# darshangm/dynamics-aware-diffusion

Measured on AMD Instinct MI355X. Metric: trajectory plans/sec (H=32, T=100), higher is better.
Workload: dtype f32; 1 GPU; PointMaze umaze-v2 guided policy, H=32 dim=128 mults(1,2,4) T=100 batch=256/GPU; arch=pointmaze, batch_per_gpu=256, global_batch=256, horizon=32, denoise_steps=100, rng=in-kernel philox, conv_arithmetic=fp32 (exact fp32 MFMA), hipgraph=False, loops_in_flight=1

## Files before the change

dynamics_aware_diffusion_amd/_engine.py:

```python
from __future__ import annotations

import ctypes as C
import math
import os
from typing import Dict, Mapping, Optional, Sequence

import torch

_HERE = os.path.dirname(os.path.abspath(__file__))
LIB_PATH = os.environ.get("DAD_LIB") or os.path.join(_HERE, "libdad_hip.so")

DAD_MAX_LEVELS = 8


class DadCfg(C.Structure):
    _fields_ = [
        ("transition_dim", C.c_int32), ("dim", C.c_int32), ("time_dim", C.c_int32),
        ("n_levels", C.c_int32), ("channels", C.c_int32 * DAD_MAX_LEVELS),
        ("kernel_size", C.c_int32), ("horizon", C.c_int32), ("n_timesteps", C.c_int32),
        ("predict_epsilon", C.c_int32), ("clip_denoised", C.c_int32),
    ]


class DadStepArgs(C.Structure):
    _fields_ = [
        ("noise", C.c_void_p), ("seed", C.c_uint64), ("row_offset", C.c_uint64),
        ("draw", C.c_uint64), ("cond0", C.c_void_p), ("cond_per_row", C.c_int32),
        ("guide_grad", C.c_void_p), ("guide_weight", C.c_float),
        ("mean_out", C.c_void_p), ("eps_out", C.c_void_p),
    ]


class DadProjectArgs(C.Structure):
    _fields_ = [
        ("P", C.c_void_p), ("obs_mean", C.c_void_p), ("obs_std", C.c_void_p),
        ("act_mean", C.c_void_p), ("act_std", C.c_void_p),
        ("state_dim", C.c_int32), ("observation_dim", C.c_int32), ("action_dim", C.c_int32),
        ("scratch", C.c_void_p), ("scratch_bytes", C.c_size_t),
    ]


class DadOptimTensor(C.Structure):
    _fields_ = [
        ("param", C.c_void_p), ("grad", C.c_void_p), ("exp_avg", C.c_void_p), ("exp_avg_sq", C.c_void_p),
        ("ema", C.c_void_p), ("numel", C.c_int64), ("group", C.c_int32),
    ]


class DadOptimGroup(C.Structure):
    _fields_ = [
        ("lr", C.c_float), ("beta1", C.c_float), ("beta2", C.c_float), ("eps", C.c_float),
        ("weight_decay", C.c_float), ("step_size", C.c_float), ("bc2_sqrt", C.c_float),
        ("decoupled", C.c_int32), ("one_minus_beta1", C.c_float), ("one_minus_beta2", C.c_float),
    ]


class DadOptimArgs(C.Structure):
    _fields_ = [
        ("groups", C.POINTER(DadOptimGroup)), ("n_groups", C.c_int32), ("max_grad_norm", C.c_float),
        ("ema_decay", C.c_float), ("grad_norm_out", C.c_void_p),
    ]


OPTIM_MAX_GROUPS = 8
OS_HEADER = ("chunk", "chunks", "grid", "partials", "record_ints")
OS_REC_FIELDS = ("tensor", "first", "first_hi", "count", "block")


ABI = {
    "dad_last_error": (C.c_char_p, []),
    "dad_version": (C.c_char_p, []),
    "dad_model_create": (C.c_int, [C.POINTER(DadCfg), C.POINTER(C.c_void_p)]),
    "dad_model_destroy": (None, [C.c_void_p]),
    "dad_model_load_weight": (C.c_int, [C.c_void_p, C.c_char_p, C.c_void_p,
                                        C.POINTER(C.c_int64), C.c_int32]),
    "dad_model_load_schedule": (C.c_int, [C.c_void_p] + [C.c_void_p] * 5),
    "dad_model_load_time_embedding": (C.c_int, [C.c_void_p, C.c_void_p, C.c_int32, C.c_int32]),
    "dad_model_set_precision": (C.c_int, [C.c_void_p, C.c_int32]),
    "dad_model_set_group_channels": (C.c_int, [C.c_void_p, C.POINTER(C.c_int32), C.c_int32]),
    "dad_model_set_horizon": (C.c_int, [C.c_void_p, C.c_int32]),
    "dad_model_finalize": (C.c_int, [C.c_void_p, C.c_void_p]),
    "dad_workspace_bytes": (C.c_int, [C.c_void_p, C.c_int32, C.POINTER(C.c_size_t)]),
    "dad_unet_forward": (C.c_int, [C.c_void_p, C.c_void_p, C.c_int32, C.c_void_p, C.c_int32,
                                   C.c_void_p, C.c_size_t, C.c_void_p]),
    "dad_unet_forward_rows": (C.c_int, [C.c_void_p, C.c_void_p, C.c_void_p, C.c_void_p, C.c_int32,
                                        C.c_void_p, C.c_size_t, C.c_void_p]),
    "dad_projection_violation": (C.c_int, [C.POINTER(DadProjectArgs), C.c_void_p, C.c_void_p, C.c_int32,
                                           C.c_int32, C.c_void_p]),
    "dad_denoise_step": (C.c_int, [C.c_void_p, C.c_void_p, C.c_int32, C.c_int32,
                                   C.POINTER(DadStepArgs), C.c_int32, C.c_void_p, C.c_size_t,
                                   C.c_void_p]),
    "dad_sample_loop": (C.c_int, [C.c_void_p, C.c_void_p, C.c_int32, C.c_int32, C.c_void_p,
                                  C.c_uint64, C.c_uint64, C.c_void_p, C.c_int32,
                                  C.POINTER(DadProjectArgs), C.c_void_p, C.c_int32, C.c_void_p,
                                  C.c_size_t, C.c_void_p]),
    "dad_project": (C.c_int, [C.POINTER(DadProjectArgs), C.c_float, C.c_void_p, C.c_int32,
                              C.c_int32, C.c_void_p]),
    "dad_fill_normal": (C.c_int, [C.c_void_p, C.c_int32, C.c_int32, C.c_uint64, C.c_uint64,
                                  C.c_uint64, C.c_void_p]),
    "dad_debug_set_tile": (C.c_int, [C.c_void_p, C.c_int32]),
    "dad_debug_set_option": (C.c_int, [C.c_void_p, C.c_char_p, C.c_int32]),
    "dad_debug_read_table": (C.c_int, [C.c_void_p, C.c_int32, C.c_int32, C.c_void_p, C.c_int32,
                                       C.POINTER(C.c_int32)]),
    "dad_debug_mish": (C.c_int, [C.c_void_p, C.c_void_p, C.c_int64, C.c_void_p]),
    "dad_debug_kernel_table_consistent": (C.c_int, []),
    "dad_debug_small_batch_plan": (C.c_int, [C.c_void_p, C.c_int32, C.POINTER(C.c_int32),
                                             C.POINTER(C.c_int32)]),
    "dad_debug_backward_plan": (C.c_int, [C.c_void_p, C.c_int32, C.POINTER(C.c_int32), C.c_int32,
                                          C.POINTER(C.c_int32)]),
    "dad_debug_backward_steps": (C.c_int, [C.c_void_p, C.c_int32, C.POINTER(C.c_int32), C.c_int32,
                                           C.POINTER(C.c_int32)]),
    "dad_debug_wgrad_kernel_exists": (C.c_int, [C.c_int32] * 3),
    "dad_model_set_training": (C.c_int, [C.c_void_p, C.c_int32]),
    "dad_model_refresh_weights": (C.c_int, [C.c_void_p, C.c_int32, C.POINTER(C.c_char_p), C.POINTER(C.c_void_p),
                                            C.c_void_p]),
    "dad_train_grad_count": (C.c_int, [C.c_void_p, C.POINTER(C.c_int32), C.POINTER(C.c_int64)]),
    "dad_train_grad_info": (C.c_int, [C.c_void_p, C.c_int32, C.POINTER(C.c_char_p), C.POINTER(C.c_int64),
                                      C.POINTER(C.c_int64)]),
    "dad_train_workspace_bytes": (C.c_int, [C.c_void_p, C.c_int32, C.POINTER(C.c_size_t),
                                            C.POINTER(C.c_size_t)]),
    "dad_unet_forward_train": (C.c_int, [C.c_void_p, C.c_void_p, C.c_void_p, C.c_void_p, C.c_void_p,
                                         C.c_int32, C.c_void_p, C.c_size_t, C.c_void_p]),
    "dad_unet_backward": (C.c_int, [C.c_void_p, C.c_void_p, C.c_void_p, C.c_void_p, C.c_void_p,
                                    C.POINTER(C.c_void_p), C.c_int32,
                                    C.c_int32, C.c_void_p, C.c_size_t, C.c_void_p, C.c_size_t, C.c_void_p]),
    "dad_model_load_train_schedule": (C.c_int, [C.c_void_p, C.c_void_p, C.c_void_p, C.c_int32]),
    "dad_train_time_grad_count": (C.c_int, [C.c_void_p, C.POINTER(C.c_int32), C.POINTER(C.c_int64)]),
    "dad_train_time_grad_info": (C.c_int, [C.c_void_p, C.c_int32, C.POINTER(C.c_char_p), C.POINTER(C.c_int64),
                                           C.POINTER(C.c_int64)]),
    "dad_train_objective_workspace_bytes": (C.c_int, [C.c_void_p, C.c_int32, C.POINTER(C.c_size_t),
                                                      C.POINTER(C.c_size_t)]),
    "dad_train_objective_forward": (C.c_int, [C.c_void_p, C.c_void_p, C.c_void_p, C.c_void_p, C.c_void_p, C.c_int32,
                                              C.c_void_p, C.c_int32, C.c_void_p, C.c_size_t, C.c_void_p]),
    "dad_train_objective_backward": (C.c_int, [C.c_void_p, C.c_void_p, C.c_void_p, C.c_void_p, C.c_int32, C.c_void_p,
                                               C.POINTER(C.c_void_p), C.c_int32, C.POINTER(C.c_void_p), C.c_int32,
                                               C.c_int32, C.c_void_p, C.c_size_t, C.c_void_p, C.c_size_t, C.c_void_p]),
    "dad_debug_objective_offsets": (C.c_int, [C.c_void_p, C.c_int32, C.POINTER(C.c_size_t), C.POINTER(C.c_size_t)]),
    "dad_debug_objective_plan": (C.c_int, [C.c_void_p, C.c_int32, C.POINTER(C.c_int32), C.c_int32,
                                           C.POINTER(C.c_int32)]),
    "dad_debug_forward_plan": (C.c_int, [C.c_void_p, C.c_int32, C.c_int32, C.POINTER(C.c_int32), C.c_int32,
                                         C.POINTER(C.c_int32)]),
    "dad_debug_project_plan": (C.c_int, [C.c_int32] * 5 + [C.c_size_t, C.c_int32, C.POINTER(C.c_int32)]),
    "dad_debug_kernel_registered": (C.c_int, [C.c_int32] * 4),
    "dad_debug_small_kernel_exists": (C.c_int, [C.c_int32] * 8),
    "dad_optim_create": (C.c_int, [C.POINTER(C.c_void_p)]),
    "dad_optim_destroy": (None, [C.c_void_p]),
    "dad_optim_step": (C.c_int, [C.c_void_p, C.POINTER(DadOptimTensor), C.c_int32, C.POINTER(DadOptimArgs), C.c_void_p]),
    "dad_debug_optim_plan": (C.c_int, [C.POINTER(C.c_int64), C.c_int32, C.POINTER(C.c_int32), C.c_int32,
                                       C.POINTER(C.c_int32)]),
    "dad_profile_enable": (C.c_int, [C.c_void_p, C.c_int32]),
    "dad_profile_read": (C.c_int, [C.c_void_p, C.POINTER(C.c_double), C.POINTER(C.c_int64),
                                   C.POINTER(C.c_double)]),
}

_lib = None


def load_library() -> C.CDLL:
    global _lib
    if _lib is not None:
        return _lib
    if not os.path.exists(LIB_PATH):
        raise RuntimeError(
            f"{LIB_PATH} not found: build it with dynamics_aware_diffusion_amd/csrc/build.sh "
            "(or __graft_entry__.build()).  There is no CPU fallback.")
    lib = C.CDLL(LIB_PATH)
    for name, (restype, argtypes) in ABI.items():
        if os.environ.get("DAD_LIB") and not hasattr(lib, name):
            continue
        fn = getattr(lib, name)
        fn.restype = restype
        fn.argtypes = argtypes
    _lib = lib
    return lib


class DadError(RuntimeError):
    def __init__(self, code: int, message: str):
        super().__init__(f"libdad_hip error {code}: {message}")
        self.code = code


def _check(lib, rc: int) -> None:
    if rc != 0:
        raise DadError(rc, lib.dad_last_error().decode("utf-8", "replace"))


def _ptr(t: Optional[torch.Tensor]) -> Optional[int]:
    return None if t is None else t.data_ptr()


def _require_device(t: torch.Tensor, name: str) -> None:
    if not t.is_cuda:
        raise RuntimeError(f"{name} must live on a ROCm device (got {t.device}); the HIP engine "
                           "has no CPU path")
    if t.dtype != torch.float32 or not t.is_contiguous():
        raise RuntimeError(f"{name} must be contiguous float32 (got {t.dtype}, "
                           f"contiguous={t.is_contiguous()})")


PRECISIONS = {"fp32": 0, "f16x3": 1}
LOSS_TYPES = {"l1": 1, "l2": 2}
TABLES = {"sinusoid": 0, "time_mlp": 1, "blocks": 2}
TIME_GEMM_MODES = ("FWD_H1", "FWD_TEMB", "FWD_ROWS", "BWD_DWK", "BWD_DACT", "BWD_DW3", "BWD_DH1", "BWD_DW1", "DTEMB")


FP_REC_FIELDS = ("conv", "sub", "cfg", "taps", "stride", "flags", "kc", "kslices", "gn_npt", "ntiles_n", "mtiles", "part_tile",
                 "family")
FP_FAMILIES = ("gemm", "halo8")
FP_CC_FIELDS = ("conv", "taps", "stride", "wide", "ride", "big", "ride_in", "tile_rows", "windowed", "slice_ch", "kslices",
                "ntiles", "res_kind")
FP_FINAL_KERNELS = (None, "final_posterior_kernel", "final_cc_kernel")
FP_FLAGS = ("x3", "bdir", "ragged", "res", "padded", "windowed")
PP_FIELDS = ("form", "rows_per_block", "gx", "gy", "lds_bytes", "refused")
PP_FORMS = ("row1", "row4", "gemm")


def registered_kernels():
    lib = load_library()
    gemm = {("gemm", cfg, taps, stride, f) for cfg in range(10) for taps in range(1, 8) for stride in (1, 2) for f in range(64)
            if lib.dad_debug_kernel_registered(cfg, taps, stride, f)}
    cc, ccw = set(), set()
    for taps in range(1, 8):
        for stride in (1, 2):
            for ride in (0, 1):
                for rows in (8, 16, 32, 64):
                    for a in (0, 1):
                        for win in (0, 1):
                            if lib.dad_debug_small_kernel_exists(taps, stride, ride, 0, a, 0, rows, win):
                                cc.add(("cc", taps, stride, ride, a, rows, win))
                        if lib.dad_debug_small_kernel_exists(taps, stride, ride, 1, 0, a, rows, 0):
                            ccw.add(("ccw", taps, stride, ride, a, rows))
    return gemm, cc, ccw


BS_KINDS = ("bias", "wgrad", "dgrad", "gn", "resid", "cols")
BS_FIELDS = {
    "bias": ("rows", "C"),
    "wgrad": ("taps", "tile", "windowed", "M", "C0", "C1", "stride", "pad", "Lg", "Lz", "gx", "gy", "ragged", "concat_inside",
              "edge_m", "edge_c", "swapped", "ksplit", "slab_n4", "samples", "spc", "sps", "chunks", "last_chunks"),
    "dgrad": ("conv", "sub", "write"),
    "gn": ("nv", "cpg", "L", "lreal", "cpg_real", "dtemb", "short_pair", "C"),
    "resid": ("write", "n", "to_x"),
    "cols": ("C", "off", "ld", "rows", "write"),
}
BS_WRITES = ("set", "add", "stage")


def wgrad_kernels():
    lib = load_library()
    return {(taps, tile, win) for taps in range(1, 9) for tile in range(4) for win in (0, 1)
            if lib.dad_debug_wgrad_kernel_exists(taps, tile, win)}


def projection_plan(state_dim: int, observation_dim: int, action_dim: int, batch: int, horizon: int, *,
                    scratch_bytes: int = 0, violation: bool = False) -> dict:
    lib = load_library()
    out = (C.c_int32 * len(PP_FIELDS))()
    _check(lib, lib.dad_debug_project_plan(int(state_dim), int(observation_dim), int(action_dim), int(batch), int(horizon),
                                           int(scratch_bytes), int(bool(violation)), out))
    q = dict(zip(PP_FIELDS, out))
    q["form"], q["refused"] = PP_FORMS[q["form"]], bool(q["refused"])
    q["grid"] = (q.pop("gx"), q.pop("gy"))
    return q


def optim_plan(numel: Sequence[int]) -> dict:
    lib = load_library()
    n = len(numel)
    sizes = (C.c_int64 * max(n, 1))(*[int(v) for v in numel])
    needed = C.c_int32()
    _check(lib, lib.dad_debug_optim_plan(sizes, n, None, 0, C.byref(needed)))
    out = (C.c_int32 * needed.value)()
    _check(lib, lib.dad_debug_optim_plan(sizes, n, out, needed.value, C.byref(needed)))
    head = dict(zip(OS_HEADER, out[:len(OS_HEADER)]))
    k = head.pop("record_ints")
    assert k == len(OS_REC_FIELDS)
    recs = []
    for i in range(head["chunks"]):
        r = dict(zip(OS_REC_FIELDS, out[len(OS_HEADER) + i * k:len(OS_HEADER) + (i + 1) * k]))
        r["first"] += r.pop("first_hi") << 31
        recs.append(r)
    head["records"] = recs
    return head


def sinusoid_table(n_timesteps: int, dim: int) -> torch.Tensor:
    half = dim // 2
    scale = math.log(10000) / (half - 1)
    freqs = torch.exp(torch.arange(half) * -scale)
    arg = torch.arange(n_timesteps)[:, None] * freqs[None, :]
    return torch.cat((arg.sin(), arg.cos()), dim=-1).contiguous()

SCHEDULE_KEYS = ("sqrt_recip_alphas_cumprod", "sqrt_recipm1_alphas_cumprod",
                 "posterior_mean_coef1", "posterior_mean_coef2",
                 "posterior_log_variance_clipped")


class HipEngine:

    def __init__(self, *, transition_dim: int, dim: int, channels: Sequence[int], horizon: int,
                 n_timesteps: int, time_dim: Optional[int] = None, kernel_size: int = 5,
                 predict_epsilon: bool = True, clip_denoised: bool = True,
                 device: torch.device | str = "cuda", precision: str = "fp32", training: bool = False):
        if precision not in PRECISIONS:
            raise ValueError(f"precision must be one of {sorted(PRECISIONS)}, got {precision!r}")
        self.precision = precision
        self.lib = load_library()
        self.device = torch.device(device)
        if self.device.type != "cuda":
            raise RuntimeError("HipEngine needs a ROCm device; there is no CPU path")
        from .utils import padding
        self.real_dim, self.real_channels = int(dim), [int(c) for c in channels]
        padded = [padding.padded_width(c) for c in self.real_channels]
        self.padded = padded != self.real_channels
        if self.padded:
            if self.real_channels[0] != self.real_dim:
                raise NotImplementedError("zero-padded widths need dim_mults[0] == 1")
            if transition_dim == self.real_dim:
                raise NotImplementedError(
                    f"transition_dim == dim == {dim} makes the first block's residual the trajectory itself; "
                    "with zero-padded GroupNorm groups that identity has no kernel")
        horizon = int(horizon)
        levels = len(self.real_channels)
        self.padded_horizon = max(1 << max(horizon - 1, 0).bit_length(), 4 << (levels - 1))
        self.rows_padded = self.padded_horizon != horizon
        if self.rows_padded:
            if horizon % (1 << (levels - 1)) != 0:
                raise ValueError(f"horizon {horizon} cannot be halved {levels - 1} times (the reference's U-Net needs "
                                 f"H % 2^(levels-1) == 0, temporal_unet.py:35-54)")
            if transition_dim == self.real_dim:
                raise NotImplementedError("transition_dim == dim with a zero-padded horizon has no kernel")
        self.padded = self.padded or self.rows_padded
        cfg = DadCfg()
        cfg.transition_dim = transition_dim
        cfg.dim = padded[0] if padded != self.real_channels else dim
        cfg.time_dim = time_dim or dim
        cfg.n_levels = len(channels)
        for i, ch in enumerate(padded):
            cfg.channels[i] = int(ch)
        cfg.kernel_size = kernel_size
        cfg.horizon = self.padded_horizon
        cfg.n_timesteps = n_timesteps
        cfg.predict_epsilon = int(predict_epsilon)
        cfg.clip_denoised = int(clip_denoised)
        self.cfg = cfg
        self.horizon = horizon
        self.transition_dim = transition_dim
        self.n_timesteps = n_timesteps
        handle = C.c_void_p()
        _check(self.lib, self.lib.dad_model_create(C.byref(cfg), C.byref(handle)))
        self._h = handle
        _check(self.lib, self.lib.dad_model_set_precision(self._h, PRECISIONS[precision]))
        self.widths_padded = padded != self.real_channels
        if self.widths_padded:
            real = (C.c_int32 * len(self.real_channels))(*self.real_channels)
            _check(self.lib, self.lib.dad_model_set_group_channels(self._h, real, len(self.real_channels)))
        if self.rows_padded:
            _check(self.lib, self.lib.dad_model_set_horizon(self._h, horizon))
        self.training = bool(training)
        if self.training:
            _check(self.lib, self.lib.dad_model_set_training(self._h, 1))
        self._ws: Dict[int, torch.Tensor] = {}
        self._pinned: Dict[tuple, torch.Tensor] = {}
        self.ready = False

    def __del__(self):
        h = getattr(self, "_h", None)
# ... 229 lines not shown
        rows = torch.arange(B, dtype=torch.int32, device=self.device)
        out = torch.empty_like(x)
        with torch.cuda.device(self.device):
            _check(self.lib, self.lib.dad_unet_forward_train(
                self._h, x.data_ptr(), rows.data_ptr(), temb_rows.data_ptr(), out.data_ptr(), B,
                saved.data_ptr(), saved.numel() * 4, self._stream()))
        return out, saved

    def train_backward(self, x: torch.Tensor, d_out: torch.Tensor, saved: torch.Tensor, temb_width: int, shapes):
        B = self._traj(x)
        if self._traj(d_out, "d_out") != B:
            raise RuntimeError("d_out batch mismatch")
        sv, sc = C.c_size_t(), C.c_size_t()
        _check(self.lib, self.lib.dad_train_workspace_bytes(self._h, B, C.byref(sv), C.byref(sc)))
        scratch = torch.empty(max(sc.value, 4) // 4 + 4, dtype=torch.float32, device=self.device)
        layout, total = self.grad_layout()
        if len(shapes) != len(layout):
            raise RuntimeError(f"{len(shapes)} parameter shapes for {len(layout)} gradient tensors")
        real = None
        if self.widths_padded:
            real = self.flat_padding([k for k, _, _ in layout], shapes, [o for _, o, _ in layout], total)
            shapes = real.padded_shapes
            for (key, _, numel), n in zip(layout, real.sizes):
                if n != numel:
                    raise RuntimeError(f"{key}: {n} padded elements, the library expects {numel}")
        flat = torch.empty(total, dtype=torch.float32, device=self.device)
        base = flat.data_ptr()
        spans = [layout[i + 1][1] - layout[i][1] for i in range(len(layout) - 1)] + [total - layout[-1][1]]
        pieces = flat.split_with_sizes(spans)
        grads = [(pc if pc.numel() == numel else pc[:numel]).view(tuple(shape))
                 for pc, (_, _, numel), shape in zip(pieces, layout, shapes)]
        ptrs = (C.c_void_p * len(grads))(*[base + 4 * offset for _, offset, _ in layout])
        d_x = torch.empty_like(x)
        d_temb = torch.empty(B, temb_width, dtype=torch.float32, device=self.device)
        with torch.cuda.device(self.device):
            _check(self.lib, self.lib.dad_unet_backward(
                self._h, x.data_ptr(), d_out.data_ptr(), d_x.data_ptr(), d_temb.data_ptr(), ptrs, len(grads), B,
                saved.data_ptr(), saved.numel() * 4, scratch.data_ptr(), scratch.numel() * 4, self._stream()))
        if real is not None:
            grads = real.gather(flat)
        return d_x, d_temb, grads

    def bind_train_schedule(self, sqrt_ac: torch.Tensor, sqrt_1m_ac: torch.Tensor) -> None:
        sig = (sqrt_ac.data_ptr(), sqrt_ac._version, sqrt_1m_ac.data_ptr(), sqrt_1m_ac._version)
        if getattr(self, "_train_sched_sig", None) == sig:
            return
        a = sqrt_ac.detach().to("cpu", torch.float32).contiguous()
        b = sqrt_1m_ac.detach().to("cpu", torch.float32).contiguous()
        if a.numel() != self.n_timesteps or b.numel() != self.n_timesteps:
            raise ValueError(f"training schedule has {a.numel()} / {b.numel()} entries, expected {self.n_timesteps}")
        with torch.cuda.device(self.device):
            _check(self.lib, self.lib.dad_model_load_train_schedule(self._h, a.data_ptr(), b.data_ptr(), self.n_timesteps))
        self._train_sched_sig = sig

    def time_grad_layout(self):
        cached = getattr(self, "_time_grad_layout", None)
        if cached is not None:
            return cached
        n, total = C.c_int32(), C.c_int64()
        _check(self.lib, self.lib.dad_train_time_grad_count(self._h, C.byref(n), C.byref(total)))
        out = []
        for i in range(n.value):
            key, off, numel = C.c_char_p(), C.c_int64(), C.c_int64()
            _check(self.lib, self.lib.dad_train_time_grad_info(self._h, i, C.byref(key), C.byref(off), C.byref(numel)))
            out.append((key.value.decode(), off.value, numel.value))
        self._time_grad_layout = (out, total.value)
        return self._time_grad_layout

    def _objective_bytes(self, batch: int):
        cache = self.__dict__.setdefault("_objective_sizes", {})
        if batch not in cache:
            sv, sc = C.c_size_t(), C.c_size_t()
            _check(self.lib, self.lib.dad_train_objective_workspace_bytes(self._h, batch, C.byref(sv), C.byref(sc)))
            cache[batch] = (sv.value, sc.value)
        return cache[batch]

    def objective_forward(self, x0: torch.Tensor, t32: torch.Tensor, noise: torch.Tensor,
                          weights: Optional[torch.Tensor], loss_type: int):
        B = self._traj(x0, "x_start")
        for name, ten in (("noise", noise), ("weights", weights)):
            if ten is not None and self._traj(ten, name) != B:
                raise RuntimeError(f"{name} batch mismatch")
        if t32.dtype != torch.int32 or t32.numel() != B or t32.device != x0.device or not t32.is_contiguous():
            raise RuntimeError("t must be (B) contiguous int32 on the trajectory's device")
        sv, _ = self._objective_bytes(B)
        saved = torch.empty(max(sv, 4) // 4 + 4, dtype=torch.float32, device=self.device)
        loss = torch.empty((), dtype=torch.float32, device=self.device)
        with torch.cuda.device(self.device):
            _check(self.lib, self.lib.dad_train_objective_forward(
                self._h, x0.data_ptr(), t32.data_ptr(), noise.data_ptr(), _ptr(weights), int(loss_type),
                loss.data_ptr(), B, saved.data_ptr(), saved.numel() * 4, self._stream()))
        return loss, saved

    def objective_backward(self, x0: torch.Tensor, noise: torch.Tensor, weights: Optional[torch.Tensor],
                           loss_type: int, d_loss: torch.Tensor, saved: torch.Tensor, shapes):
        B = self._traj(x0, "x_start")
        _require_device(d_loss, "d_loss")
        _, sc = self._objective_bytes(B)
        scratch = torch.empty(max(sc, 4) // 4 + 4, dtype=torch.float32, device=self.device)
        conv, conv_total = self.grad_layout()
        time, time_total = self.time_grad_layout()
        layout = list(conv) + [(k, conv_total + o, n) for k, o, n in time]
        total = conv_total + time_total
        if len(shapes) != len(layout):
            raise RuntimeError(f"{len(shapes)} parameter shapes for {len(layout)} gradient tensors")
        real = None
        if self.widths_padded:
            real = self.flat_padding([k for k, _, _ in layout], shapes, [o for _, o, _ in layout], total)
            shapes = real.padded_shapes
            for (key, _, numel), n in zip(layout, real.sizes):
                if n != numel:
                    raise RuntimeError(f"{key}: {n} padded elements, the library expects {numel}")
        flat = torch.empty(total, dtype=torch.float32, device=self.device)
        base = flat.data_ptr()
        ptrs = (C.c_void_p * len(conv))(*[base + 4 * o for _, o, _ in layout[:len(conv)]])
        tptrs = (C.c_void_p * len(time))(*[base + 4 * o for _, o, _ in layout[len(conv):]])
        with torch.cuda.device(self.device):
            _check(self.lib, self.lib.dad_train_objective_backward(
                self._h, x0.data_ptr(), noise.data_ptr(), _ptr(weights), int(loss_type), d_loss.data_ptr(),
                ptrs, len(conv), tptrs, len(time), B, saved.data_ptr(), saved.numel() * 4,
                scratch.data_ptr(), scratch.numel() * 4, self._stream()))
        if real is not None:
            return real.gather(flat)
        spans = [layout[i + 1][1] - layout[i][1] for i in range(len(layout) - 1)] + [total - layout[-1][1]]
        pieces = flat.split_with_sizes(spans)
        return [(pc if pc.numel() == numel else pc[:numel]).view(tuple(shape))
                for pc, (_, _, numel), shape in zip(pieces, layout, shapes)]

    def objective_saved_views(self, saved: torch.Tensor, batch: int):
        a, b = C.c_size_t(), C.c_size_t()
        _check(self.lib, self.lib.dad_debug_objective_offsets(self._h, int(batch), C.byref(a), C.byref(b)))
        n = batch * self.horizon * self.transition_dim
        shape = (batch, self.horizon, self.transition_dim)
        return saved[a.value // 4:a.value // 4 + n].view(shape), saved[b.value // 4:b.value // 4 + n].view(shape)

    def debug_set_tile(self, cfg: int) -> None:
        self.__dict__.pop("_objective_sizes", None)
        with torch.cuda.device(self.device):
            _check(self.lib, self.lib.dad_debug_set_tile(self._h, int(cfg)))

    def debug_set_option(self, name: str, value: int) -> None:
        self.__dict__.pop("_objective_sizes", None)
        with torch.cuda.device(self.device):
            _check(self.lib, self.lib.dad_debug_set_option(self._h, name.encode(), int(value)))

    def read_table(self, which: str, t: int) -> torch.Tensor:
        out = torch.empty(1 << 16, dtype=torch.float32)
        width = C.c_int32()
        with torch.cuda.device(self.device):
            _check(self.lib, self.lib.dad_debug_read_table(self._h, TABLES[which], int(t),
                                                           out.data_ptr(), out.numel(), C.byref(width)))
        return out[:width.value].clone()

    def small_batch_plan(self, batch: int):
        n, w = C.c_int32(), C.c_int32()
        _check(self.lib, self.lib.dad_debug_small_batch_plan(self._h, int(batch), C.byref(n), C.byref(w)))
        return n.value, w.value

    def backward_plan(self, batch: int) -> dict:
        need = C.c_int32()
        _check(self.lib, self.lib.dad_debug_backward_plan(self._h, int(batch), None, 0, C.byref(need)))
        buf = (C.c_int32 * need.value)()
        _check(self.lib, self.lib.dad_debug_backward_plan(self._h, int(batch), buf, need.value, C.byref(need)))
        r = list(buf)
        fields = ("taps", "tile", "windowed", "samples", "spc", "sps", "ksplit", "chunks", "last_chunks")
        assert r[71] == len(fields) and (len(r) - 72) == r[0] * r[71]
        hist = lambda at: {(cfg, bool(s)): r[at + 2 * cfg + s] for cfg in range(10) for s in (0, 1) if r[at + 2 * cfg + s]}
        return {
            "wgrads": r[0], "multi": r[1], "max_chunks": r[2], "max_ksplit": r[3], "part": r[4], "part_multi": r[5],
            "windowed": r[6], "tile": r[7:11],
            "taps_tile": {(taps, tile): r[11 + 4 * i + tile] for i, taps in enumerate((1, 3, 4, 5, 7)) for tile in range(4)
                          if r[11 + 4 * i + tile]},
            "fwd": hist(31), "dgrad": hist(51),
            "launches": [dict(zip(fields, r[at:at + len(fields)])) for at in range(72, len(r), len(fields))],
        }

    def backward_steps(self, batch: int) -> dict:
        need = C.c_int32()
        _check(self.lib, self.lib.dad_debug_backward_steps(self._h, int(batch), None, 0, C.byref(need)))
        buf = (C.c_int32 * need.value)()
        _check(self.lib, self.lib.dad_debug_backward_steps(self._h, int(batch), buf, need.value, C.byref(need)))
        r = list(buf)
        ints = r[1]
        assert ints == 25 and len(r) - 12 == r[0] * ints
        steps = []
        for at in range(12, len(r), ints):
            kind = BS_KINDS[r[at]]
            q = dict(zip(BS_FIELDS[kind], r[at + 1:at + ints]), kind=kind)
            if "write" in q:
                q["write"] = BS_WRITES[q["write"]]
            steps.append(q)
        return {"batch": r[2], "colsums": (r[3], r[4], r[5]), "padcopy": bool(r[6]), "horizon": r[7], "real_horizon": r[8],
                "dx": bool(r[9]), "steps": steps}

    def objective_plan(self, batch: int) -> dict:
        need = C.c_int32()
        _check(self.lib, self.lib.dad_debug_objective_plan(self._h, int(batch), None, 0, C.byref(need)))
        buf = (C.c_int32 * need.value)()
        _check(self.lib, self.lib.dad_debug_objective_plan(self._h, int(batch), buf, need.value, C.byref(need)))
        r = list(buf)
        fields = ("mode", "M", "N", "K", "gx", "gy", "gz", "chunks", "last_chunks", "ktail", "kslice")
        assert r[6] == len(fields) and (len(r) - 8) == r[7] * r[6]
        launches = []
        for at in range(8, len(r), len(fields)):
            q = dict(zip(fields, r[at:at + len(fields)]))
            q["mode"] = TIME_GEMM_MODES[q["mode"]]
            q["grid"] = (q.pop("gx"), q.pop("gy"), q.pop("gz"))
            launches.append(q)
        return {"loss_blocks": r[0], "kslices": r[1], "kslice": r[2], "temb_width": r[3], "blocks": r[4], "n": r[5],
                "launches": launches}

    def forward_plan(self, batch: int, mode: int = 0) -> dict:
        need = C.c_int32()
        _check(self.lib, self.lib.dad_debug_forward_plan(self._h, int(batch), int(mode), None, 0, C.byref(need)))
        buf = (C.c_int32 * need.value)()
        _check(self.lib, self.lib.dad_debug_forward_plan(self._h, int(batch), int(mode), buf, need.value, C.byref(need)))
        r = list(buf)
        small = bool(r[2])
        fields = FP_CC_FIELDS if small else FP_REC_FIELDS
        assert r[4] == len(fields) and len(r) - 8 == r[3] * r[4]
        launches = []
        for at in range(8, len(r), len(fields)):
            q = dict(zip(fields, r[at:at + len(fields)]))
            if not small and FP_FAMILIES[q["family"]] == "halo8":
                q["key"] = ("halo8", q["cfg"], (q["flags"] >> 3) & 1)
            elif not small:
                q["key"] = ("gemm", q["cfg"], q["taps"], q["stride"], q["flags"])
            elif q["wide"]:
                q["key"] = ("ccw", q["taps"], q["stride"], q["ride"], q["ride_in"], q["tile_rows"])
            else:
                q["key"] = ("cc", q["taps"], q["stride"], q["ride"], q["big"], q["tile_rows"], q["windowed"])
            launches.append(q)
        return {"mode": r[0], "batch": r[1], "small": small, "final": (r[5], r[6], FP_FINAL_KERNELS[r[7]]), "launches": launches}

    def mish(self, x: torch.Tensor) -> torch.Tensor:
        _require_device(x, "x")
        out = torch.empty_like(x)
        with torch.cuda.device(self.device):
            _check(self.lib, self.lib.dad_debug_mish(x.data_ptr(), out.data_ptr(), x.numel(),
                                                     self._stream()))
        return out

    def profile_enable(self, on: bool) -> None:
        _check(self.lib, self.lib.dad_profile_enable(self._h, int(on)))

    def profile_read(self):
        ms, n, fl = C.c_double(), C.c_int64(), C.c_double()
        _check(self.lib, self.lib.dad_profile_read(self._h, C.byref(ms), C.byref(n), C.byref(fl)))
        return ms.value, n.value, fl.value


class ProjectionState:

    def __init__(self, P: torch.Tensor, obs_mean, obs_std, act_mean, act_std, state_dim: int,
                 observation_dim: int, action_dim: int, device):
        dev = torch.device(device)
        if dev.type != "cuda":
            raise RuntimeError("projection kernel needs a ROCm device; there is no CPU path")

        def put(v):
            return torch.as_tensor(v, dtype=torch.float32).contiguous().to(dev)

        self.P = put(P)
        self.obs_mean, self.obs_std = put(obs_mean), put(obs_std)
        self.act_mean, self.act_std = put(act_mean), put(act_std)
        a = DadProjectArgs()
        a.P = self.P.data_ptr()
        a.obs_mean, a.obs_std = self.obs_mean.data_ptr(), self.obs_std.data_ptr()
        a.act_mean, a.act_std = self.act_mean.data_ptr(), self.act_std.data_ptr()
        a.state_dim, a.observation_dim, a.action_dim = state_dim, observation_dim, action_dim
        self.args = a
        self.device = dev
        self._scratch = None
        self.gemm = True
        self.D = int(self.P.shape[0])
        if self.P.dim() != 2 or self.P.shape[1] != self.D:
            raise ValueError(f"projection matrix must be square, got {tuple(self.P.shape)}")
        if self.obs_mean.numel() != observation_dim or self.obs_std.numel() != observation_dim \
                or self.act_mean.numel() != action_dim or self.act_std.numel() != action_dim:
            raise ValueError("normaliser statistics do not match observation_dim / action_dim")

    @classmethod
    def host(cls, state_dim: int, observation_dim: int, action_dim: int, gemm: bool = True) -> "ProjectionState":
        self = cls.__new__(cls)
        self.args = DadProjectArgs()
        self.args.state_dim, self.args.observation_dim, self.args.action_dim = state_dim, observation_dim, action_dim
        self.device, self._scratch, self.gemm, self.D = None, None, gemm, None
        return self

    def _check_x(self, x: torch.Tensor) -> None:
        _require_device(x, "x")
        a = self.args
        if x.dim() != 3 or x.shape[2] != a.observation_dim + a.action_dim:
            raise RuntimeError(f"x must be (B, H, {a.observation_dim + a.action_dim}), got {tuple(x.shape)}")
        D = (int(x.shape[1]) + 1) * a.state_dim + int(x.shape[1]) * a.action_dim
        if D != self.D:
            raise RuntimeError(f"mat1 and mat2 shapes cannot be multiplied ({x.shape[0]}x{D} and "
                               f"{self.D}x{self.D}): the projector was built for another horizon")
        if x.device != self.P.device:
            raise RuntimeError(f"x is on {x.device}, the projector on {self.P.device}")
        if self.gemm and (self._scratch is None or self._scratch.numel() < x.numel()):
            self._scratch = torch.empty(x.numel(), dtype=torch.float32, device=self.device)
            self.args.scratch = self._scratch.data_ptr()
            self.args.scratch_bytes = self._scratch.numel() * 4

    def plan(self, batch: int, horizon: int, violation: bool = False) -> dict:
# ... 26 lines not shown
```

dynamics_aware_diffusion_amd/csrc/conv_shapes.hpp:

```cpp
#pragma once
#include <stddef.h>

#if defined(__HIPCC__)
#define DAD_HD __host__ __device__
#else
#define DAD_HD
#endif

namespace dad {

constexpr int kXSwzPad = 64;
constexpr size_t kLdsBytes = 160 * 1024;

DAD_HD inline int conv_xrows(int BN, int Lin, int Lout, int taps) {
    return Lout > BN ? BN * (Lin / Lout) + 2 * (taps / 2) : (BN / Lout) * (Lin + 2 * (taps / 2));
}
DAD_HD inline size_t conv_lds_floats(int BM, int BN, int KC, int taps, int Lin, int Lout, int SK,
                                     bool bdir = false, int wtaps = 0) {
    const size_t kp = KC + 4;
    const size_t wt = wtaps ? wtaps : taps;
    const size_t stage = (size_t)conv_xrows(BN, Lin, Lout, taps) * kp + kXSwzPad +
                         (bdir ? 0 : wt * BM * kp);
    const size_t epi = (size_t)SK * BN * (BM + 4) + 64;
    const size_t k = 2 * stage;
    return k > epi ? k : epi;
}

DAD_HD inline int halo8_sample(int i) { return ((i >> 1) & 1) * 4 + (i >> 2); }
DAD_HD inline int halo8_pos(int i, int q) { return 2 * q + (i & 1); }
DAD_HD inline int halo8_block(int tn, int nb) { return tn ? 3 - nb : nb; }
DAD_HD inline int halo8_tap(int tn, int t) { return tn ? 4 - t : t; }

constexpr int WG_THREADS = 512;
constexpr int WG_ROWS = 64;
constexpr int WG_MAX_GROWS = 128, WG_MAX_ZROWS = 160;

constexpr int COLS_MAX = 120;

DAD_HD inline int wgrad_segz(int Lz, int taps, int pad) { return Lz + pad + (taps - 1 - pad); }
DAD_HD inline int wgrad_round64(int v) { return (v + 63) / 64 * 64; }
DAD_HD inline size_t wgrad_lds_floats(int spc, int Lg, int Lz, int taps, int pad, int tm, int tn) {
    const size_t stage = 2 * ((size_t)wgrad_round64(spc * Lg * 8 * tm) * 4 + (size_t)wgrad_round64(spc * wgrad_segz(Lz, taps, pad) * 8 * tn) * 4);
    const size_t red = (size_t)4 * taps * 16 * 64;
    return stage > red ? stage : red;
}

DAD_HD inline int cc_xrows(int taps, int Lin, int Lout, int nr) {
    return Lout > nr ? nr + 2 * (taps / 2) : (nr / Lout) * (Lin + 2 * (taps / 2));
}

constexpr int CC_THREADS = 512;
constexpr int CC_MAX_SLABS = 8;
DAD_HD inline size_t cc_lds_floats(int slice_ch, int taps, int wtaps, int Lin, int Lout, int nr) {
    const size_t xs = slice_ch + 4;
    const size_t k = (size_t)cc_xrows(taps, Lin, Lout, nr) * xs + (size_t)wtaps * 32 * xs;
    const size_t e = (size_t)2 * 8 * nr * 36;
    return k > e ? k : e;
}
DAD_HD inline size_t final_cc_lds_floats(int td, int dim, int H) {
    return (size_t)td * dim + ((td + 3) & ~3) + (size_t)H * (dim + 4);
}

constexpr int FINAL_COLS = 32;
DAD_HD inline int final_rows_local(int td, int gy) {
    constexpr int JG = 256 / FINAL_COLS;
    const int col_groups = (td + JG - 1) / JG;
    return (col_groups + gy - 1) / gy * JG;
}
DAD_HD inline size_t final_lds_floats(int td, int dim, int gy) {
    return (size_t)final_rows_local(td, gy) * dim + ((td + 3) & ~3) + (size_t)FINAL_COLS * (dim + 4);
}

constexpr int GNP_THREADS = 256;
constexpr int kGnPassMaxNpt = 32;

constexpr int kCcwMaxPairs = 64;
DAD_HD inline size_t ccw_lds_floats(int slice_ch, int taps, int Lin, int Lout, int nr) {
    const int spt = nr / Lout;
    const size_t xs = slice_ch + 4;
    const size_t k = (size_t)spt * (Lin + 2 * (taps / 2)) * xs + (size_t)spt * Lin * xs + 2 * (size_t)slice_ch +
                     2 * kCcwMaxPairs;
    const size_t e = (size_t)2 * 8 * nr * 36;
    return k > e ? k : e;
}

constexpr int PROJ_KP = 16;
DAD_HD inline size_t project_row_lds_bytes(int D) { return (size_t)(1 + PROJ_KP) * D * sizeof(float); }
constexpr int PG_THREADS = 256;
constexpr int PG_KC = 64;
constexpr int PG_AS = 33;
DAD_HD inline size_t project_gemm_lds_floats() { return (size_t)4 * PG_KC * PG_AS + 64; }

}
```

dynamics_aware_diffusion_amd/csrc/dad_lib.hip:

```cpp
#include <hip/hip_runtime.h>

#include <algorithm>
#include <cmath>
#include <cstdarg>
#include <cstdio>
#include <cstring>
#include <cstdlib>
#include <functional>
#include <map>
#include <memory>
#include <string>
#include <vector>

#include <mutex>
#include <set>
#include <tuple>
#include <utility>

#include "../../include/dad.h"
#include "host_plan.hpp"
#include "conv_gemm.hpp"
#include "conv_halo8.hpp"
#include "conv_gn_pass.hpp"
#include "pointwise.hpp"
#include "conv_cc.hpp"
#include "conv_ccw.hpp"
#include "train_bwd.hpp"
#include "train_objective.hpp"
#include "optim_step.hpp"

using namespace dadhost;

namespace {

#ifdef DAD_STAMPS
unsigned long long* g_stamps = nullptr;
#endif

#define HIP_TRY(expr)                                                                   \
    do {                                                                                \
        hipError_t e_ = (expr);                                                         \
        if (e_ != hipSuccess)                                                           \
            return fail(DAD_E_HIP, "%s failed: %s (%s:%d)", #expr, hipGetErrorString(e_), \
                        __FILE__, __LINE__);                                            \
    } while (0)

struct GraphKey {
    const void* x; const void* noise; const void* cond; const void* ws;
    const void* P; const void* obs_mean; const void* obs_std; const void* act_mean; const void* act_std;
    const void* proj_scratch;
    int n_steps, batch, cond_per_row, state_dim, observation_dim, action_dim;
    int force_tile, flags;
    uint64_t row_offset;
    uint64_t alpha_hash;
    bool operator<(const GraphKey& o) const {
        return std::memcmp(this, &o, sizeof(GraphKey)) < 0;
    }
};

}

struct dad_model : HostModel {
    bool finalized = false;
    int device = -1;
    std::vector<float> sched[5];
    bool have_sched = false;
    std::vector<float> emb_override;
    float* d_emb = nullptr;
    float* d_temb = nullptr;
    float* d_temb_table = nullptr;
    float* d_final_w = nullptr;
    float* d_final_b = nullptr;
    uint64_t* d_rng = nullptr;
    unsigned* d_counters = nullptr;
    float* d_zero = nullptr;
    std::map<std::string, float*> d_time;
    std::vector<WeightEntry> weights;
    float* d_h1 = nullptr;
    std::vector<float> train_sched[2];
    float* d_train_sched = nullptr;
    std::vector<void*> owned;
    void* d_repack = nullptr;
    size_t repack_cap = 0;
    std::vector<char> repack_host;
    bool tables_stale = false;
    char* arena = nullptr;
    size_t arena_cap = 0, arena_used = 0;
    bool profile = false;
    std::vector<std::pair<hipEvent_t, hipEvent_t>> ev_pool;
    size_t ev_used = 0;
    double prof_flops = 0;
    int64_t prof_launches = 0;
    std::map<GraphKey, hipGraphExec_t> graphs;
    hipStream_t cap_stream = nullptr;
};

namespace {

using dad::ConvParams;

int arena_alloc(dad_model* m, size_t bytes, void** out) {
    const size_t aligned = (bytes + 255) / 256 * 256;
    if (m->arena_used + aligned > m->arena_cap)
        return fail(DAD_E_STATE, "parameter arena exhausted (%zu + %zu > %zu)", m->arena_used, aligned,
                    m->arena_cap);
    *out = m->arena + m->arena_used;
    m->arena_used += aligned;
    return DAD_OK;
}

int upload(dad_model* m, const std::vector<float>& host, float** dev) {
    void* p = nullptr;
    const int rc = arena_alloc(m, std::max<size_t>(host.size(), 1) * sizeof(float), &p);
    if (rc != DAD_OK) return rc;
    HIP_TRY(hipMemcpy(p, host.data(), host.size() * sizeof(float), hipMemcpyHostToDevice));
    *dev = (float*)p;
    return DAD_OK;
}

float*& weight_ptr(dad_model* m, const WeightEntry& e) {
    switch (e.to) {
        case WT_W: return m->plan.convs[e.conv].d_w;
        case WT_BIAS: return m->plan.convs[e.conv].d_bias;
        case WT_RBIAS: return m->plan.convs[e.conv].d_rbias;
        case WT_GAMMA: return m->plan.convs[e.conv].d_gamma;
        case WT_BETA: return m->plan.convs[e.conv].d_beta;
        case WT_BWD_W: return m->bconvs[e.conv].op[e.sub].d_w;
        case WT_BFINAL_W: return m->bfinal.d_w;
        case WT_FINAL_W: return m->d_final_w;
        case WT_FINAL_B: return m->d_final_b;
        case WT_TIME: break;
    }
    return m->d_time[e.key];
}

void free_device(dad_model* m) {
    for (auto& kv : m->graphs) (void)hipGraphExecDestroy(kv.second);
    m->graphs.clear();
    for (void* p : m->owned) (void)hipFree(p);
    m->owned.clear();
    m->d_repack = nullptr; m->repack_cap = 0; m->repack_host.clear(); m->tables_stale = false;
    m->arena = nullptr;
    m->arena_cap = m->arena_used = 0;
    m->d_emb = m->d_temb = m->d_temb_table = nullptr;
    m->d_final_w = m->d_final_b = nullptr;
    m->d_rng = nullptr;
    m->d_counters = nullptr;
    m->d_zero = nullptr;
    m->d_train_sched = nullptr;
    m->weights.clear(); m->d_time.clear();
    for (Plan* plan : {&m->plan, &m->tplan})
        for (auto& op : plan->convs) op.d_w = op.d_bias = op.d_gamma = op.d_beta = op.d_rbias = nullptr;
    for (auto& b : m->bconvs) for (int k = 0; k < b.n; ++k) b.op[k].d_w = b.op[k].d_bias = nullptr;
    m->bfinal.d_w = m->bfinal.d_bias = nullptr;
}

using KernFn = void (*)(const ConvParams);
using KernKey = std::tuple<int, int, int, bool, bool, bool, bool, bool, bool>;
using KernTable = std::map<KernKey, KernFn>;

template <int CFG, int TAPS, int STRIDE, int F>
void reg_kernel(KernTable& t) {
    if constexpr (kernel_registered_f(CFG, TAPS, STRIDE, F)) {
        constexpr TileCfg T = kTiles[CFG];
        constexpr bool X3 = F & 1, BDIR = F & 2, RAGGED = F & 4, RES = F & 8, PADDED = F & 16, WIN = F & 32;
        t[KernKey(CFG, TAPS, STRIDE, X3, BDIR, RAGGED, RES, PADDED, WIN)] =
            dad::conv_gemm_f32<T.BM, T.BN, T.SK, tile_kc(CFG, TAPS, X3, BDIR), TAPS, STRIDE, RAGGED, X3, BDIR, RES, PADDED, WIN>;
    }
}
template <int CFG, int TAPS, size_t... F>
void reg_flags(KernTable& t, std::index_sequence<F...>) {
    (reg_kernel<CFG, TAPS, 1, (int)F>(t), ...);
    (reg_kernel<CFG, TAPS, 2, (int)F>(t), ...);
}
template <int CFG, size_t... TAPS>
void reg_taps(KernTable& t, std::index_sequence<TAPS...>) {
    (reg_flags<CFG, (int)TAPS + 1>(t, std::make_index_sequence<(1 << kRegFlags)>()), ...);
}
template <size_t... CFG>
void reg_tiles(KernTable& t, std::index_sequence<CFG...>) {
    (reg_taps<(int)CFG>(t, std::make_index_sequence<kRegMaxTaps>()), ...);
}
const KernTable& kernel_table() {
    static const KernTable table = [] {
        KernTable t;
        reg_tiles(t, std::make_index_sequence<kNumTiles>());
        return t;
    }();
    return table;
}

struct FamilyKernel { int key[5]; const void* fn; };
using FamilyList = std::vector<FamilyKernel>;
const void* find_kernel(const FamilyList& list, int k0, int k1, int k2, int k3 = 0, int k4 = 0) {
    for (const FamilyKernel& k : list)
        if (k.key[0] == k0 && k.key[1] == k1 && k.key[2] == k2 && k.key[3] == k3 && k.key[4] == k4) return k.fn;
    return nullptr;
}

template <bool BIG, int NR>
void add_cc(FamilyList& v) {
    v.push_back({{5, 0, BIG, NR, 0}, (const void*)dad::conv_cc<5, 1, false, BIG, NR>});
    v.push_back({{5, 1, BIG, NR, 0}, (const void*)dad::conv_cc<5, 1, true, BIG, NR>});
    v.push_back({{3, 0, BIG, NR, 0}, (const void*)dad::conv_cc<3, 2, false, BIG, NR>});
    v.push_back({{2, 0, BIG, NR, 0}, (const void*)dad::conv_cc<2, 1, false, BIG, NR>});
}
const FamilyList& cc_kernels() {
    static const FamilyList list = [] {
        FamilyList v;
        add_cc<false, 16>(v); add_cc<false, 32>(v); add_cc<true, 16>(v); add_cc<true, 32>(v);
        v.push_back({{5, 0, 0, 32, 1}, (const void*)dad::conv_cc<5, 1, false, false, 32, 6, true>});
        v.push_back({{5, 1, 0, 32, 1}, (const void*)dad::conv_cc<5, 1, true, false, 32, 6, true>});
        return v;
    }();
    return list;
}
const void* cc_kernel(int taps, bool ride, bool big, int rows, bool windowed) {
    return find_kernel(cc_kernels(), taps, ride, big, rows, windowed);
}

template <bool RIDE, int NR>
void add_ccw(FamilyList& v) {
    v.push_back({{5, 0, RIDE, NR}, (const void*)dad::conv_ccw<5, 1, false, RIDE, NR>});
    v.push_back({{5, 1, RIDE, NR}, (const void*)dad::conv_ccw<5, 1, true, RIDE, NR>});
    v.push_back({{3, 0, RIDE, NR}, (const void*)dad::conv_ccw<3, 2, false, RIDE, NR>});
    v.push_back({{2, 0, RIDE, NR}, (const void*)dad::conv_ccw<2, 1, false, RIDE, NR>});
    v.push_back({{1, 0, RIDE, NR}, (const void*)dad::conv_ccw<1, 1, false, RIDE, NR>});
}
const FamilyList& ccw_kernels() {
    static const FamilyList list = [] {
        FamilyList v;
        add_ccw<false, 16>(v); add_ccw<false, 32>(v); add_ccw<true, 16>(v); add_ccw<true, 32>(v);
        return v;
    }();
    return list;
}
const void* ccw_kernel(int taps, bool res, bool ride_in, int rows) {
    return find_kernel(ccw_kernels(), taps, res, ride_in, rows);
}

const FamilyList& halo8_kernels() {
    static const FamilyList list = [] {
        FamilyList v;
        static_assert(kTiles[0].BM == 32 && kTiles[0].SK == 4 && kTiles[1].BM == 64 && kTiles[1].SK == 2 && halo8_kernel_exists(0) &&
                      halo8_kernel_exists(1) && !halo8_kernel_exists(2), "conv_halo8_f32 covers tiles 0 and 1");
        v.push_back({{0, 0}, (const void*)dad::conv_halo8_f32<32, 4, false>});
        v.push_back({{0, 1}, (const void*)dad::conv_halo8_f32<32, 4, true>});
        v.push_back({{1, 0}, (const void*)dad::conv_halo8_f32<64, 2, false>});
        v.push_back({{1, 1}, (const void*)dad::conv_halo8_f32<64, 2, true>});
        return v;
    }();
    return list;
}
const void* halo8_kernel(int cfg, bool res) { return find_kernel(halo8_kernels(), cfg, res, 0); }

template <int TAPS, bool WIN>
void add_wgrad(FamilyList& v) {
    v.push_back({{TAPS, 0, WIN}, (const void*)dad::conv_wgrad<TAPS, 2, 2, true, WIN>});
    v.push_back({{TAPS, 1, WIN}, (const void*)dad::conv_wgrad<TAPS, 2, 1, true, WIN>});
    v.push_back({{TAPS, 2, WIN}, (const void*)dad::conv_wgrad<TAPS, 1, 1, true, WIN>});
    v.push_back({{TAPS, 3, WIN}, (const void*)dad::conv_wgrad<TAPS, 1, 1, false, WIN>});
}
template <size_t... I>
void add_wgrad_taps(FamilyList& v, std::index_sequence<I...>) {
    ((add_wgrad<kWgradTaps[I], false>(v), add_wgrad<kWgradTaps[I], true>(v)), ...);
}
const FamilyList& wgrad_kernels() {
    static const FamilyList list = [] {
        FamilyList v;
        add_wgrad_taps(v, std::make_index_sequence<std::size(kWgradTaps)>());
        return v;
    }();
    return list;
}
const void* wgrad_kernel(int taps, int tile, bool win) { return find_kernel(wgrad_kernels(), taps, tile, win); }

int configure_kernels() {
    static std::mutex lock;
    static std::set<int> done;
    int dev = -1;
    HIP_TRY(hipGetDevice(&dev));
    std::lock_guard<std::mutex> hold(lock);
    if (done.count(dev)) return DAD_OK;
    std::vector<const void*> fns = {(const void*)dad::final_posterior_kernel, (const void*)dad::final_cc_kernel,
                                    (const void*)dad::project_kernel<4, 16>, (const void*)dad::project_kernel<1, 16>};
    for (const auto& kv : kernel_table()) fns.push_back((const void*)kv.second);
    for (const FamilyList* list : {&cc_kernels(), &ccw_kernels(), &wgrad_kernels(), &halo8_kernels()})
        for (const FamilyKernel& k : *list) fns.push_back(k.fn);
    for (const void* fn : fns)
        HIP_TRY(hipFuncSetAttribute(fn, hipFuncAttributeMaxDynamicSharedMemorySize, (int)dad::kLdsBytes));
    done.insert(dev);
    return DAD_OK;
}

struct ConvIO {
    const float* src0 = nullptr; const float* src1 = nullptr;
    float* dst = nullptr; const float* res = nullptr; float* rdst = nullptr;
    const float* temb = nullptr; const int32_t* trow = nullptr;
    float* pre = nullptr; float* stats = nullptr;
    float* slab = nullptr;
};
int launch_conv(dad_model* m, const ConvOp& op, const LaunchGeom& g, int batch, const ConvIO& io, hipStream_t st);

int run_conv(dad_model* m, const FwdPlan& f, const FwdLaunch& l, const float* xext, float* ws, int t, hipStream_t st,
             const int32_t* trow, const float* temb_rows) {
    const Plan& plan = f.train ? m->tplan : m->plan;
    const ConvOp& op = plan.convs[l.conv];
    const int batch = f.batch;
    auto buf = [&](int id) -> float* {
        return id >= 0 ? ws + plan.bufs[id].offset * (long)batch : nullptr;
    };
    if (op.cat0 >= 0) {
        const long rows = (long)batch * op.Lout;
        const long n4 = rows * ((op.cat_c0 + op.cat_c1) / 4);
        hipLaunchKernelGGL(dad::concat_rows_kernel, dim3((unsigned)((n4 + 255) / 256)), dim3(256), 0, st,
                           buf(op.res), buf(op.cat0), buf(op.cat1), rows, op.cat_c0, op.cat_c1);
        HIP_TRY(hipGetLastError());
    }
    ConvIO io;
    io.src0 = op.src0 == -2 ? xext : buf(op.src0);
    io.src1 = buf(op.src1);
    if (op.temb_off >= 0)
        io.temb = temb_rows != nullptr ? temb_rows + op.temb_off
                                       : m->d_temb_table + (trow ? 0L : (long)t * m->plan.temb_width) + op.temb_off;
    io.trow = io.temb != nullptr ? trow : nullptr;
    io.res = op.res == -2 ? xext : buf(op.res);
    io.dst = buf(op.dst);
    io.rdst = buf(op.rdst);
    io.pre = buf(op.pre); io.stats = buf(op.stats);
    io.slab = ws + plan.floats_per_sample * (long)batch;
    return launch_conv(m, op, l.g, batch, io, st);
}

int launch_gn_pass(dad_model* m, const ConvOp& op, int npt, int batch, const ConvIO& io, hipStream_t st) {
    dad::GnPassParams q{};
    q.src = io.pre != nullptr ? io.pre : io.dst;
    q.dst = io.dst;
    q.gamma = op.d_gamma; q.beta = op.d_beta;
    q.temb = io.temb; q.trow = io.trow; q.temb_stride = m->plan.temb_width;
    q.res = io.res; q.stats = io.stats;
    q.C = op.cout; q.L = op.Lout; q.cpg = op.cout / 8; q.lreal = op.lreal; q.cpg_real = op.gn_real;
    const dim3 grid(8, (unsigned)batch), block(dad::GNP_THREADS);
    static_assert(dad::kGnPassMaxNpt == 32, "one case per power of two up to kGnPassMaxNpt");
    switch (npt) {
        case 1: hipLaunchKernelGGL(dad::gn_pass_kernel<1>, grid, block, 0, st, q); break;
        case 2: hipLaunchKernelGGL(dad::gn_pass_kernel<2>, grid, block, 0, st, q); break;
        case 4: hipLaunchKernelGGL(dad::gn_pass_kernel<4>, grid, block, 0, st, q); break;
        case 8: hipLaunchKernelGGL(dad::gn_pass_kernel<8>, grid, block, 0, st, q); break;
        case 16: hipLaunchKernelGGL(dad::gn_pass_kernel<16>, grid, block, 0, st, q); break;
        default: hipLaunchKernelGGL(dad::gn_pass_kernel<32>, grid, block, 0, st, q);
    }
    HIP_TRY(hipGetLastError());
    return DAD_OK;
}

int launch_conv(dad_model* m, const ConvOp& op, const LaunchGeom& g, int batch, const ConvIO& io, hipStream_t st) {
    const bool gn_pass = g.gn_npt > 0;
    ConvParams p{};
    p.src0 = io.src0;
    p.src1 = io.src1;
    p.w = op.d_w; p.bias = op.d_bias; p.gamma = op.d_gamma; p.beta = op.d_beta;
    p.temb = io.temb;
    p.trow = io.trow; p.temb_stride = m->plan.temb_width;
    p.res = io.res;
    p.dst = io.dst;
    p.pre = io.pre; p.stats = io.stats;
    if (gn_pass) {
        p.gamma = p.beta = p.temb = p.res = nullptr;
        p.trow = nullptr;
        p.pre = nullptr; p.stats = nullptr;
        if (io.pre != nullptr) p.dst = io.pre;
    }
    p.cin0 = op.cin0; p.cin1 = op.cin1; p.cin_pad = op.cin_pad;
    p.M = op.M; p.cpg = op.norm.empty() ? 0 : op.cout / 8; p.cpg_real = op.gn_real;
    p.lreal = op.lreal; p.src_len = op.src_len;
    p.B = batch; p.Lin = op.Lin; p.Lout = op.Lout; p.lshift = ilog2(op.Lout);
    p.lshift_in = ilog2(op.Lin);
    p.interleave = op.kind == CONV_UP;
    p.ntiles_n = g.ntiles_n;
    p.xcd_gn = g.xcd_gn; p.xcd_mts = g.xcd_mts; p.xcd_ntn = g.xcd_ntn;
    p.kslices = g.split.kslices;
    p.chunks_per_slice = g.split.chunks_per_slice;
    p.slab = io.slab;
    p.counters = m->d_counters;
    p.c1 = op.c1; p.c2 = op.c2;
    p.xswz = g.xswz;
    p.wtaps = op.wtaps();
    p.rbias = g.fused ? op.d_rbias : nullptr;
    p.rdst = g.fused ? io.rdst : nullptr;
    if (g.split.kslices > 1 && io.slab == nullptr)
        return fail(DAD_E_WORKSPACE, "%s: split-K launch without scratch", op.name.c_str());
    static const bool trace = getenv("DAD_TRACE_TILES") != nullptr;
    if (trace)
        fprintf(stderr, "[dad] %-34s B=%d M=%d K=%dx%d L=%d tile=%d (%dx%d SK%d) kslices=%d%s\n", op.name.c_str(),
                batch, op.M, op.taps, op.cin0 + op.cin1, op.Lout, g.cfg, kTiles[g.cfg].BM, kTiles[g.cfg].BN,
                kTiles[g.cfg].SK, g.split.kslices, g.fused ? " +res1x1" : "");
#ifdef DAD_STAMPS
    p.stamps = (g_stamps && &op >= &m->plan.convs[0] && &op < &m->plan.convs[0] + m->plan.convs.size())
                   ? g_stamps + (size_t)(&op - &m->plan.convs[0]) * 4096 * 8 : nullptr;
#endif
    if (g.halo8) {
        const void* fn = halo8_kernel(g.cfg, g.fused);
        if (fn == nullptr || gn_pass || p.pre != nullptr || p.stats != nullptr || p.kslices != 1)
            return fail(DAD_E_INVALID, "no halo-skipping kernel for %s (tile %d res=%d)", op.name.c_str(), g.cfg, (int)g.fused);
        p.xswz = g.xswz8;
        void* hargs[] = {&p};
        HIP_TRY(hipLaunchKernel(fn, dim3(g.gx, g.gy, g.gz), dim3(g.threads), hargs, g.lds_bytes, st));
        return DAD_OK;
    }
    const auto& table = kernel_table();
    const auto it = table.find(KernKey(g.cfg, op.taps, op.stride, op.x3, op.bdir, g.ragged, g.fused, g.padded, g.windowed));
    if (it == table.end())
        return fail(DAD_E_INVALID, "no kernel for %s (tile %d taps=%d stride=%d x3=%d bdir=%d ragged=%d res=%d)",
                    op.name.c_str(), g.cfg, op.taps, op.stride, (int)op.x3, (int)op.bdir, (int)g.ragged, (int)g.fused);
    void* args[] = {&p};
    HIP_TRY(hipLaunchKernel((const void*)it->second, dim3(g.gx, g.gy, g.gz), dim3(g.threads), args,
                            g.lds_bytes, st));
    if (gn_pass) return launch_gn_pass(m, op, g.gn_npt, batch, io, st);
    return DAD_OK;
}

int build_time_tables(dad_model* m, hipStream_t st);
int upload_train_schedule(dad_model* m) {
    const size_t T = m->train_sched[0].size();
    if (m->d_train_sched != nullptr) HIP_TRY(hipDeviceSynchronize());
    if (m->d_train_sched == nullptr) {
        void* a = nullptr;
        HIP_TRY(hipMalloc(&a, 2 * T * sizeof(float)));
        m->owned.push_back(a);
        m->d_train_sched = (float*)a;
    }
    HIP_TRY(hipMemcpy(m->d_train_sched, m->train_sched[0].data(), T * sizeof(float), hipMemcpyHostToDevice));
    HIP_TRY(hipMemcpy(m->d_train_sched + T, m->train_sched[1].data(), T * sizeof(float), hipMemcpyHostToDevice));
    return DAD_OK;
}
int ensure_tables(dad_model* m, hipStream_t st) {
    if (!m->tables_stale) return DAD_OK;
    const int rc = build_time_tables(m, st);
    if (rc == DAD_OK) m->tables_stale = false;
    return rc;
}

int check_ready(const dad_model* m, int batch, int t, size_t ws_bytes, bool small_ok, FwdPlan& f) {
    if (!m) return fail(DAD_E_INVALID, "null model");
    if (!m->finalized) return fail(DAD_E_STATE, "dad_model_finalize has not been called");
    if (batch <= 0) return fail(DAD_E_INVALID, "batch must be positive (got %d)", batch);
    if (t < 0 || t >= m->cfg.n_timesteps)
        return fail(DAD_E_RANGE, "index %d is out of bounds for the schedule of size %d", t,
                    m->cfg.n_timesteps);
    const int rc = plan_forward(*m, false, batch, small_ok, f);
    if (ws_bytes < f.bytes)
        return fail(DAD_E_WORKSPACE, "workspace has %zu bytes, batch %d needs %zu", ws_bytes, batch,
                    f.bytes);
    return rc;
}

dad::CcSrc cc_source(dad_model* m, const CcPlan& cc, const CcInput& in, int channels, const float* xext,
                     float* ws, int batch, int t) {
    dad::CcSrc s{};
    auto buf = [&](int id) -> float* { return ws + m->plan.bufs[id].offset * (long)batch; };
    float* slabs = ws + m->plan.floats_per_sample * (long)batch;
    s.C = channels;
    if (in.kind == 1) { s.data = xext; s.rows = batch * m->cfg.horizon; return s; }
    if (in.kind == 2) { s.data = buf(in.buf); return s; }
    const ConvOp& q = m->plan.convs[in.producer];
    const CcOp& qo = cc.ops[in.producer];
    s.data = slabs + qo.oslab;
    s.nsl = qo.kslices;
    s.C = qo.out_cols;
    s.rows = qo.out_rows;
    s.bias = q.d_bias;
    if (!q.norm.empty()) { s.gamma = q.d_gamma; s.beta = q.d_beta; s.cpg = q.cout / 8; }
    if (q.temb_off >= 0) s.temb = m->d_temb_table + (long)t * m->plan.temb_width + q.temb_off;
    if (qo.res_kind == 1) s.res = xext;
    else if (qo.res_kind == 2) s.res = buf(qo.res_buf);
    else if (qo.res_kind == 3) {
        const CcOp& r = cc.ops[qo.res_ride];
        s.rslab = slabs + r.orslab; s.nrs = r.kslices; s.rbias = m->plan.convs[qo.res_ride].d_rbias;
    } else if (qo.res_kind == 4) {
        const CcOp& r = cc.ops[qo.res_ride];
        s.rslab = slabs + r.oslab; s.nrs = r.kslices; s.rbias = m->plan.convs[qo.res_ride].d_bias;
    }
    s.mat = buf(in.buf);
    return s;
}

int run_conv_cc(dad_model* m, const CcPlan& cc, int i, const float* xext, float* ws, int batch, int t,
                hipStream_t st) {
    const ConvOp& op = m->plan.convs[i];
    const CcOp& o = cc.ops[i];
    dad::CcParams p{};
    p.src0 = cc_source(m, cc, o.in0, op.cin0, xext, ws, batch, t);
    if (o.in1.kind != 0) p.src1 = cc_source(m, cc, o.in1, op.cin1, xext, ws, batch, t);
    p.w = op.d_w; p.wtaps = op.wtaps();
    p.cin0 = op.cin0; p.cin1 = op.cin1; p.M = op.M;
    p.B = batch; p.Lin = op.Lin; p.Lout = op.Lout;
    p.lshift = ilog2(op.Lout); p.lshift_in = ilog2(op.Lin);
    p.interleave = op.kind == CONV_UP;
    p.slice_ch = o.slice_ch;
    float* slabs = ws + m->plan.floats_per_sample * (long)batch;
    p.oslab = slabs + o.oslab;
    p.orslab = o.orslab >= 0 ? slabs + o.orslab : nullptr;
    p.out_rows = o.out_rows;
    const void* kern = o.wide ? ccw_kernel(op.taps, op.ride, o.ride_in, o.tile_rows)
                              : cc_kernel(op.taps, op.ride, o.big, o.tile_rows, op.Lout > 32);
    if (!kern) return fail(DAD_E_INVALID, "no small-batch kernel for %s (taps=%d stride=%d)", op.name.c_str(), op.taps, op.stride);
    static const bool trace = getenv("DAD_TRACE_TILES") != nullptr;
    if (trace)
        fprintf(stderr, "[dad] %-34s B=%d M=%d K=%dx%d L=%d cc slice=%d kslices=%d ntiles=%d%s\n", op.name.c_str(), batch,
                op.M, op.taps, op.cin0 + op.cin1, op.Lout, o.slice_ch, o.kslices, o.ntiles, op.ride ? " +res1x1" : "");
    if (trace && o.wide) fprintf(stderr, "[dad]   (wide: %d-row tiles, %zu B LDS)\n", o.tile_rows, o.lds_bytes);
#ifdef DAD_STAMPS
    p.stamps = g_stamps ? g_stamps + (size_t)i * 16 : nullptr;
#endif
    void* args[] = {&p};
    HIP_TRY(hipLaunchKernel(kern, dim3(o.kslices, op.M / 32, o.ntiles), dim3(dad::CC_THREADS), args, o.lds_bytes, st));
    return DAD_OK;
}

int run_unet(dad_model* m, const FwdPlan& f, const float* x, int t, float* ws, hipStream_t st,
             const int32_t* trow = nullptr, const float* temb_rows = nullptr) {
    hipEvent_t e0 = nullptr, e1 = nullptr;
    if (m->profile) {
        if (m->ev_used == m->ev_pool.size()) {
            hipEvent_t a, b;
            HIP_TRY(hipEventCreate(&a));
            HIP_TRY(hipEventCreate(&b));
            m->ev_pool.push_back({a, b});
        }
        e0 = m->ev_pool[m->ev_used].first;
        e1 = m->ev_pool[m->ev_used].second;
        ++m->ev_used;
        HIP_TRY(hipEventRecord(e0, st));
    }
    for (size_t i = 0; f.cc.ok && i < f.cc.ops.size(); ++i) {
        if (!f.cc.ops[i].launched) continue;
        const int rc = run_conv_cc(m, f.cc, (int)i, x, ws, f.batch, t, st);
        if (rc != DAD_OK) return rc;
    }
    for (const FwdLaunch& l : f.launches) {
        const int rc = run_conv(m, f, l, x, ws, t, st, trow, temb_rows);
        if (rc != DAD_OK) return rc;
    }
    if (m->profile) {
        for (const ConvOp& op : m->plan.convs) m->prof_flops += op.flops_per_sample * f.batch;
        for (const CcOp& o : f.cc.ops) m->prof_launches += o.launched;
        m->prof_launches += (int64_t)f.launches.size();
        HIP_TRY(hipEventRecord(e1, st));
    }
    return DAD_OK;
}

int run_final(dad_model* m, const FwdPlan& f, float* x, const float* x_ro, int t, const dad_step_args* a,
              int x_out_disabled, float* eps_only, float* ws, hipStream_t st, bool seed_from_device = false) {
    const dad_cfg& c = m->cfg;
    const int batch = f.batch;
    dad::FinalParams p{};
    const Plan& plan = f.train ? m->tplan : m->plan;
    p.act = ws + plan.bufs[plan.final_act].offset * (long)batch;
    p.w = m->d_final_w; p.bias = m->d_final_b;
    p.dim = c.dim; p.td = c.transition_dim; p.B = batch; p.H = traj_horizon(*m); p.Hact = c.horizon;
    p.predict_epsilon = c.predict_epsilon; p.clip_denoised = c.clip_denoised;
    if (eps_only) {
        p.x = const_cast<float*>(x_ro);
        p.eps_out = eps_only;
        p.x_out_disabled = 1;
    } else {
        p.x = x;
        p.noise = a->noise; p.cond0 = a->cond0; p.cond_per_row = a->cond_per_row;
        p.guide = (a->guide_grad && a->guide_weight > 0.0f) ? a->guide_grad : nullptr;
        p.mean_out = a->mean_out; p.eps_out = a->eps_out;
        p.x_out_disabled = x_out_disabled;
        const float lv = m->sched[4][t];
        p.c_recip = m->sched[0][t]; p.c_recipm1 = m->sched[1][t];
        p.coef1 = m->sched[2][t]; p.coef2 = m->sched[3][t];
        p.sigma = t == 0 ? 0.0f : expf(0.5f * lv);
        p.guide_scale = a->guide_weight * expf(lv);
        p.seed = a->seed;
        p.elem_offset = a->row_offset * (uint64_t)traj_horizon(*m) * (uint64_t)c.transition_dim;
        p.draw = a->draw;
        p.seed_dev = seed_from_device ? (const unsigned long long*)m->d_rng : nullptr;
    }
    const dim3 grid(f.final_gx, f.final_gy);
    if (f.cc.ok) {
        dad::FinalCcParams fp{};
        CcInput in; in.kind = 3; in.producer = f.cc.final_producer; in.buf = m->plan.final_act;
        fp.src = cc_source(m, f.cc, in, c.dim, x_ro ? x_ro : x, ws, batch, t);
        fp.src.mat = nullptr;
        fp.f = p;
        hipLaunchKernelGGL(dad::final_cc_kernel, grid, dim3(dad::CC_THREADS), f.final_lds, st, fp);
    } else {
        hipLaunchKernelGGL(dad::final_posterior_kernel, grid, dim3(256), f.final_lds, st, p);
    }
    HIP_TRY(hipGetLastError());
    return DAD_OK;
}

int run_project(const dad_project_args* pa, float alpha, float* x, int batch, int horizon,
                hipStream_t st, float* violation = nullptr) {
    if (!pa || !pa->P) return fail(DAD_E_INVALID, "projection arguments missing");
    if (alpha <= 0.0f && !violation) return DAD_OK;
    {
        const int rc0 = configure_kernels();
        if (rc0 != DAD_OK) return rc0;
    }
    dad::ProjParams p{};
    p.P = pa->P; p.obs_mean = pa->obs_mean; p.obs_std = pa->obs_std;
    p.act_mean = pa->act_mean; p.act_std = pa->act_std;
    p.x = x; p.B = batch; p.H = horizon; p.n = pa->state_dim; p.od = pa->observation_dim;
    p.m = pa->action_dim;
    p.D = (horizon + 1) * p.n + horizon * p.m;
    p.alpha = alpha;
    p.one_minus_alpha = (float)(1.0 - (double)alpha);
    p.violation = violation;
    const size_t x_bytes = (size_t)batch * horizon * (pa->observation_dim + pa->action_dim) * sizeof(float);
    const ProjectPlan q = plan_project(p.D, batch, x_bytes, pa->scratch ? pa->scratch_bytes : 0, violation != nullptr);
    if (q.refused)
        return fail(DAD_E_INVALID, "projection dimension D=%d: one trajectory's partial sums exceed LDS; pass "
                    "dad_project_args.scratch and a batch of at least 32 for the GEMM form", p.D);
    const dim3 grid(q.gx, q.gy);
    if (q.form == DAD_PP_GEMM) {
        p.xout = pa->scratch;
        hipLaunchKernelGGL(dad::project_gemm_kernel, grid, dim3(dad::PG_THREADS), q.lds_bytes, st, p);
        HIP_TRY(hipGetLastError());
        HIP_TRY(hipMemcpyAsync(x, pa->scratch, x_bytes, hipMemcpyDeviceToDevice, st));
        return DAD_OK;
    }
    p.xout = x;
    if (q.form == DAD_PP_ROW1)
        hipLaunchKernelGGL((dad::project_kernel<1, dad::PROJ_KP>), grid, dim3(64 * dad::PROJ_KP), q.lds_bytes, st, p);
    else
        hipLaunchKernelGGL((dad::project_kernel<4, dad::PROJ_KP>), grid, dim3(64 * dad::PROJ_KP), q.lds_bytes, st, p);
    HIP_TRY(hipGetLastError());
    return DAD_OK;
}

int build_time_tables(dad_model* m, hipStream_t st) {
    const dad_cfg& c = m->cfg;
    const int T = c.n_timesteps, dim = c.dim, tdm = c.time_dim;
    auto linear = [&](const float* in, const std::string& key, float* out, int K, int M, int stride, int mish_in) -> int {
        auto w = m->d_time.find(key + ".weight"), b = m->d_time.find(key + ".bias");
        if (w == m->d_time.end() || b == m->d_time.end()) return fail(DAD_E_KEY, "missing key '%s'", key.c_str());
        const long total = (long)T * M;
        hipLaunchKernelGGL(dad::table_linear_kernel, dim3((unsigned)((total + 255) / 256)), dim3(256),
                           0, st, in, w->second, b->second, out, T, K, M, stride, mish_in);
        HIP_TRY(hipGetLastError());
        return DAD_OK;
    };
    int rc;
    if ((rc = linear(m->d_emb, "time_mlp.1", m->d_h1, dim, 4 * tdm, 4 * tdm, 0)) != DAD_OK) return rc;
    if ((rc = linear(m->d_h1, "time_mlp.3", m->d_temb, 4 * tdm, tdm, tdm, 1)) != DAD_OK) return rc;
    for (const ConvOp& op : m->plan.convs) {
        if (op.temb_off < 0) continue;
        std::string base = op.name.substr(0, op.name.size() - std::strlen(".blocks.0.block.0"));
        if ((rc = linear(m->d_temb, base + ".time_mlp.1", m->d_temb_table + op.temb_off, tdm, op.cout,
                         m->plan.temb_width, 1)) != DAD_OK) return rc;
    }
    return DAD_OK;
}

}

extern "C" {

const char* dad_last_error(void) { return g_err; }
const char* dad_version(void) { return "dad-hip 0.1 (gfx950, fp32 MFMA)"; }

int dad_model_create(const dad_cfg* cfg, dad_model** out) {
    if (!cfg || !out) return fail(DAD_E_INVALID, "null argument");
    int rc = check_cfg(cfg);
    if (rc != DAD_OK) return rc;
    std::unique_ptr<dad_model> m(new dad_model());
    m->cfg = *cfg;
    m->xswz_enabled = getenv("DAD_NO_XSWZ") == nullptr;
    m->xcd_order = getenv("DAD_NO_XCD_ORDER") == nullptr;
    m->fuse_residual = getenv("DAD_NO_FUSE_RES") == nullptr;
    if (const char* v = getenv("DAD_SPLIT_TARGET")) m->split_target = std::max(1, atoi(v));
    m->cc_enabled = getenv("DAD_NO_CC") == nullptr;
    if (const char* v = getenv("DAD_CC_MAX_ROWS")) m->cc_max_rows = std::max(0, atoi(v));
    if (const char* v = getenv("DAD_WGRAD_BLOCKS")) m->wgrad_blocks = std::max(1, atoi(v));
    if ((rc = build_plan(m.get())) != DAD_OK) return rc;
    *out = m.release();
    return DAD_OK;
}

void dad_model_destroy(dad_model* m) {
    if (!m) return;
    free_device(m);
    if (m->cap_stream) (void)hipStreamDestroy(m->cap_stream);
    for (auto& e : m->ev_pool) { (void)hipEventDestroy(e.first); (void)hipEventDestroy(e.second); }
    delete m;
}

int dad_model_load_weight(dad_model* m, const char* key, const float* data, const int64_t* shape,
                          int32_t ndim) {
    if (!m || !key || !data || !shape) return fail(DAD_E_INVALID, "null argument");
    auto it = m->expected.find(key);
    if (it == m->expected.end()) return fail(DAD_E_KEY, "unexpected key '%s'", key);
    if ((int)it->second.size() != ndim) return fail(DAD_E_KEY, "'%s': rank %d, expected %zu", key, ndim, it->second.size());
    size_t n = 1;
    for (int i = 0; i < ndim; ++i) {
        if (shape[i] != it->second[i])
            return fail(DAD_E_KEY, "'%s': size mismatch at dim %d (%lld vs %lld)", key, i,
                        (long long)shape[i], (long long)it->second[i]);
        n *= (size_t)shape[i];
    }
    HostTensor& t = m->raw[key];
    t.shape.assign(shape, shape + ndim);
    t.data.assign(data, data + n);
    m->finalized = false;
    return DAD_OK;
}

int dad_model_load_schedule(dad_model* m, const float* a, const float* b, const float* c1,
                            const float* c2, const float* lv) {
    if (!m || !a || !b || !c1 || !c2 || !lv) return fail(DAD_E_INVALID, "null argument");
    const float* src[5] = {a, b, c1, c2, lv};
    for (int i = 0; i < 5; ++i) m->sched[i].assign(src[i], src[i] + m->cfg.n_timesteps);
    m->have_sched = true;
    return DAD_OK;
}

int dad_model_load_train_schedule(dad_model* m, const float* sqrt_ac, const float* sqrt_1m_ac, int32_t n) {
    if (!m || !sqrt_ac || !sqrt_1m_ac) return fail(DAD_E_INVALID, "null argument");
    if (n != m->cfg.n_timesteps)
        return fail(DAD_E_INVALID, "training schedule has %d entries, the model %d timesteps", n, m->cfg.n_timesteps);
    m->train_sched[0].assign(sqrt_ac, sqrt_ac + n);
    m->train_sched[1].assign(sqrt_1m_ac, sqrt_1m_ac + n);
    return m->finalized ? upload_train_schedule(m) : DAD_OK;
}

int dad_model_load_time_embedding(dad_model* m, const float* emb, int32_t n_timesteps, int32_t dim) {
    if (!m || !emb) return fail(DAD_E_INVALID, "null argument");
    if (n_timesteps != m->cfg.n_timesteps || dim != m->cfg.dim)
// ... 39 lines not shown
    for (int i = 0; i < DAD_MAX_LEVELS; ++i) m->real_channels[i] = i < n_levels ? real_channels[i] : 0;
    const int rc = build_plan(m);
    if (rc != DAD_OK) return rc;
    m->finalized = false;
    if (m->training) if (const char* why = training_refusal(*m)) return fail(DAD_E_INVALID, "training: %s", why);
    return DAD_OK;
}

int dad_model_finalize(dad_model* m, dad_stream_t stream) {
    if (!m) return fail(DAD_E_INVALID, "null model");
    if (!m->have_sched) return fail(DAD_E_STATE, "schedule not loaded");
    for (auto& kv : m->expected)
        if (!m->raw.count(kv.first)) return fail(DAD_E_KEY, "missing key '%s'", kv.first.c_str());
    hipStream_t st = (hipStream_t)stream;
    HIP_TRY(hipStreamSynchronize(st));
    {
        const int rc0 = configure_kernels();
        if (rc0 != DAD_OK) return rc0;
    }
    free_device(m);
    const dad_cfg& c = m->cfg;
    if (m->training) if (const char* why = training_refusal(*m)) return fail(DAD_E_INVALID, "training: %s", why);
    m->weights = weight_table(*m);
    {
        void* a = nullptr;
        m->arena_cap = arena_bytes_needed(*m, m->weights);
        HIP_TRY(hipMalloc(&a, m->arena_cap));
        m->owned.push_back(a);
        m->arena = (char*)a;
        m->arena_used = 0;
    }

    HIP_TRY(hipGetDevice(&m->device));
    int rc;
    std::vector<float> host;
    for (WeightEntry& e : m->weights) {
        if ((rc = pack_entry(m, e, host)) != DAD_OK) return rc;
        if ((rc = upload(m, host, &e.dev)) != DAD_OK) return rc;
        weight_ptr(m, e) = e.dev;
    }
    for (size_t i = 0; i < m->plan.convs.size(); ++i) {
        const ConvOp& a = m->plan.convs[i];
        ConvOp& b = m->tplan.convs[i];
        b.d_w = a.d_w; b.d_bias = a.d_bias; b.d_gamma = a.d_gamma; b.d_beta = a.d_beta; b.d_rbias = a.d_rbias;
        b.c1 = a.c1; b.c2 = a.c2;
    }
    if (m->training) {
        std::vector<float> zeros((size_t)std::max(m->max_bwd_m, 2 * m->max_cout) + 64, 0.0f);
        if ((rc = upload(m, zeros, &m->d_zero)) != DAD_OK) return rc;
        for (HostModel::BwdConv& b : m->bconvs)
            for (int k = 0; k < b.n; ++k) b.op[k].d_bias = m->d_zero;
        m->bfinal.d_bias = m->d_zero;
    }

    const int T = c.n_timesteps, dim = c.dim, tdm = c.time_dim;
    const std::vector<float> emb = m->emb_override.size() == (size_t)T * dim ? m->emb_override
                                                                            : sinusoid_table(T, dim);
    float *d_emb, *d_h1, *d_temb;
    (void)c; (void)dim;
    if ((rc = upload(m, emb, &d_emb)) != DAD_OK) return rc;
    std::vector<float> zeros((size_t)T * 4 * tdm, 0.0f);
    if ((rc = upload(m, zeros, &d_h1)) != DAD_OK) return rc;
    zeros.resize((size_t)T * tdm);
    if ((rc = upload(m, zeros, &d_temb)) != DAD_OK) return rc;
    zeros.assign((size_t)T * std::max(1, m->plan.temb_width), 0.0f);
    if ((rc = upload(m, zeros, &m->d_temb_table)) != DAD_OK) return rc;
    m->d_emb = d_emb; m->d_temb = d_temb; m->d_h1 = d_h1;
    if ((rc = build_time_tables(m, st)) != DAD_OK) return rc;
    void* rng = nullptr;
    if ((rc = arena_alloc(m, 64, &rng)) != DAD_OK) return rc;
    m->d_rng = (uint64_t*)rng;
    void* cnt = nullptr;
    if ((rc = arena_alloc(m, kMaxSplitTiles * sizeof(unsigned), &cnt)) != DAD_OK) return rc;
    HIP_TRY(hipMemsetAsync(cnt, 0, kMaxSplitTiles * sizeof(unsigned), st));
    m->d_counters = (unsigned*)cnt;
    HIP_TRY(hipStreamSynchronize(st));
    if (!m->train_sched[0].empty() && (rc = upload_train_schedule(m)) != DAD_OK) return rc;
    m->raw.clear();
    m->finalized = true;
    return DAD_OK;
}

int dad_workspace_bytes(const dad_model* m, int32_t batch, size_t* bytes) {
    if (!m || !bytes || batch <= 0) return fail(DAD_E_INVALID, "bad argument");
    *bytes = workspace_bytes(*m, batch);
    return DAD_OK;
}

int dad_unet_forward(dad_model* m, const float* x, int32_t t, float* out, int32_t batch,
                     void* workspace, size_t workspace_bytes, dad_stream_t stream) {
    FwdPlan f;
    int rc = check_ready(m, batch, t, workspace_bytes, true, f);
    if (rc != DAD_OK) return rc;
    if (!x || !out || !workspace) return fail(DAD_E_INVALID, "null pointer");
    hipStream_t st = (hipStream_t)stream;
    if ((rc = ensure_tables(m, st)) != DAD_OK) return rc;
    if ((rc = run_unet(m, f, x, t, (float*)workspace, st)) != DAD_OK) return rc;
    return run_final(m, f, nullptr, x, t, nullptr, 1, out, (float*)workspace, st);
}

int dad_unet_forward_rows(dad_model* m, const float* x, const int32_t* t_rows, float* out, int32_t batch,
                          void* workspace, size_t workspace_bytes, dad_stream_t stream) {
    FwdPlan f;
    int rc = check_ready(m, batch, 0, workspace_bytes, false, f);
    if (rc != DAD_OK) return rc;
    if (!x || !out || !workspace || !t_rows) return fail(DAD_E_INVALID, "null pointer");
    hipStream_t st = (hipStream_t)stream;
    if ((rc = ensure_tables(m, st)) != DAD_OK) return rc;
    if ((rc = run_unet(m, f, x, 0, (float*)workspace, st, t_rows)) != DAD_OK) return rc;
    return run_final(m, f, nullptr, x, 0, nullptr, 1, out, (float*)workspace, st);
}

int dad_denoise_step(dad_model* m, float* x, int32_t t, int32_t batch, const dad_step_args* args,
                     int32_t x_out_disabled, void* workspace, size_t workspace_bytes,
                     dad_stream_t stream) {
    FwdPlan f;
    int rc = check_ready(m, batch, t, workspace_bytes, true, f);
    if (rc != DAD_OK) return rc;
    if (!x || !args || !workspace) return fail(DAD_E_INVALID, "null pointer");
    hipStream_t st = (hipStream_t)stream;
    if ((rc = ensure_tables(m, st)) != DAD_OK) return rc;
    if ((rc = run_unet(m, f, x, t, (float*)workspace, st)) != DAD_OK) return rc;
    return run_final(m, f, x, nullptr, t, args, x_out_disabled, nullptr, (float*)workspace, st);
}

int dad_project(const dad_project_args* p, float alpha, float* x, int32_t batch, int32_t horizon,
                dad_stream_t stream) {
    if (!x || batch <= 0 || horizon <= 0) return fail(DAD_E_INVALID, "bad argument");
    return run_project(p, alpha, x, batch, horizon, (hipStream_t)stream);
}

int dad_projection_violation(const dad_project_args* p, const float* x, float* violation, int32_t batch,
                             int32_t horizon, dad_stream_t stream) {
    if (!x || !violation || batch <= 0 || horizon <= 0) return fail(DAD_E_INVALID, "bad argument");
    return run_project(p, 1.0f, const_cast<float*>(x), batch, horizon, (hipStream_t)stream, violation);
}

int dad_sample_loop(dad_model* m, float* x, int32_t n_steps, int32_t batch,
                    const float* noise_stack, uint64_t seed, uint64_t row_offset,
                    const float* cond0, int32_t cond_per_row, const dad_project_args* proj,
                    const float* proj_alphas_host, int32_t use_graph, void* workspace,
                    size_t workspace_bytes, dad_stream_t stream) {
    if (n_steps < 1) return fail(DAD_E_INVALID, "n_steps must be positive");
    FwdPlan f;
    int rc = check_ready(m, batch, n_steps - 1, workspace_bytes, true, f);
    if (rc != DAD_OK) return rc;
    if (!x || !workspace) return fail(DAD_E_INVALID, "null pointer");
    if (proj && !proj_alphas_host) return fail(DAD_E_INVALID, "projection needs per-step alphas");
    hipStream_t st = (hipStream_t)stream;
    if ((rc = ensure_tables(m, st)) != DAD_OK) return rc;
    const long step_elems = (long)batch * traj_horizon(*m) * m->cfg.transition_dim;

    const bool seed_dev = use_graph && !m->profile && noise_stack == nullptr;
    auto enqueue_all = [&](hipStream_t st) -> int {
        for (int j = 0; j < n_steps; ++j) {
            const int t = n_steps - 1 - j;
            dad_step_args a{};
            a.noise = noise_stack ? noise_stack + (long)j * step_elems : nullptr;
            a.seed = seed; a.row_offset = row_offset; a.draw = (uint64_t)(j + 1);
            a.cond0 = cond0; a.cond_per_row = cond_per_row;
            int r = run_unet(m, f, x, t, (float*)workspace, st);
            if (r != DAD_OK) return r;
            if ((r = run_final(m, f, x, nullptr, t, &a, 0, nullptr, (float*)workspace, st, seed_dev)) != DAD_OK) return r;
            if (proj && (r = run_project(proj, proj_alphas_host[t], x, batch, traj_horizon(*m), st)) != DAD_OK)
                return r;
        }
        return DAD_OK;
    };

    if (!use_graph || m->profile) return enqueue_all(st);

    if (seed_dev) {
        hipLaunchKernelGGL(dad::set_u64_kernel, dim3(1), dim3(1), 0, st,
                           (unsigned long long*)m->d_rng, (unsigned long long)seed);
        HIP_TRY(hipGetLastError());
    }
    GraphKey key{};
    key.x = x; key.noise = noise_stack; key.cond = cond0; key.ws = workspace;
    if (proj) {
        key.P = proj->P; key.obs_mean = proj->obs_mean; key.obs_std = proj->obs_std;
        key.act_mean = proj->act_mean; key.act_std = proj->act_std;
        key.proj_scratch = proj->scratch;
        key.state_dim = proj->state_dim; key.observation_dim = proj->observation_dim;
        key.action_dim = proj->action_dim;
    }
    key.n_steps = n_steps; key.batch = batch; key.cond_per_row = cond_per_row;
    key.force_tile = m->force_tile;
    key.flags = (m->split_enabled ? 1 : 0) | (m->fuse_residual ? 2 : 0) | (m->xswz_enabled ? 4 : 0) |
                (m->xcd_order ? 8 : 0) | (f.cc.ok ? 16 : 0) | (m->split_target << 8);
    key.row_offset = row_offset;
    if (proj) {
        uint64_t hsh = 1469598103934665603ull;
        for (int i = 0; i < n_steps; ++i) {
            uint32_t bits;
            std::memcpy(&bits, &proj_alphas_host[i], 4);
            hsh = (hsh ^ bits) * 1099511628211ull;
        }
        key.alpha_hash = hsh;
    }
    auto it = m->graphs.find(key);
    if (it == m->graphs.end()) {
        if (m->graphs.size() >= 16) {
            HIP_TRY(hipDeviceSynchronize());
            for (auto& kv : m->graphs) (void)hipGraphExecDestroy(kv.second);
            m->graphs.clear();
        }
        if (!m->cap_stream) HIP_TRY(hipStreamCreateWithFlags(&m->cap_stream, hipStreamNonBlocking));
        hipGraph_t graph = nullptr;
        HIP_TRY(hipStreamBeginCapture(m->cap_stream, hipStreamCaptureModeRelaxed));
        rc = enqueue_all(m->cap_stream);
        hipError_t e = hipStreamEndCapture(m->cap_stream, &graph);
        if (rc != DAD_OK) { if (graph) (void)hipGraphDestroy(graph); return rc; }
        if (e != hipSuccess) return fail(DAD_E_HIP, "hipStreamEndCapture: %s", hipGetErrorString(e));
        hipGraphExec_t exec = nullptr;
        e = hipGraphInstantiate(&exec, graph, nullptr, nullptr, 0);
        (void)hipGraphDestroy(graph);
        if (e != hipSuccess) return fail(DAD_E_HIP, "hipGraphInstantiate: %s", hipGetErrorString(e));
        it = m->graphs.emplace(key, exec).first;
    }
    HIP_TRY(hipGraphLaunch(it->second, st));
    return DAD_OK;
}

int dad_model_set_training(dad_model* m, int32_t on) {
    if (!m) return fail(DAD_E_INVALID, "null model");
    if (on) if (const char* why = training_refusal(*m)) return fail(DAD_E_INVALID, "training: %s", why);
    if ((on != 0) != m->training) m->finalized = false;
    m->training = on != 0;
    return DAD_OK;
}

int dad_model_refresh_weights(dad_model* m, int32_t n, const char* const* keys, const float* const* tensors,
                              dad_stream_t stream) {
    if (!m || n < 0 || (n > 0 && (!keys || !tensors))) return fail(DAD_E_INVALID, "bad argument");
    if (!m->finalized) return fail(DAD_E_STATE, "dad_model_finalize has not been called");
    if (m->precision != DAD_PREC_FP32)
        return fail(DAD_E_STATE, "the split-f16 images are scaled per layer on the host: load the weights and finalize again");
    hipStream_t st = (hipStream_t)stream;
    std::vector<dad::ImageDesc> reps;
    std::vector<std::tuple<float*, const float*, size_t>> copies;
    std::map<std::string, const float*> given;
    for (int i = 0; i < n; ++i) {
        if (!keys[i] || !tensors[i]) return fail(DAD_E_INVALID, "null key or tensor at index %d", i);
        if (!m->expected.count(keys[i])) return fail(DAD_E_KEY, "unexpected key '%s'", keys[i]);
        given[keys[i]] = tensors[i];
    }
    auto has = [&](const std::string& k) -> const float* { auto it = given.find(k); return it == given.end() ? nullptr : it->second; };
    bool tables_dirty = false;
    for (const WeightEntry& e : m->weights) {
        const float* w = has(e.key);
        if (e.img.n == 0) {
            if (!w) continue;
            if ((size_t)e.floats >= (1u << 31)) return fail(DAD_E_INVALID, "refresh: a tensor of %zu floats", (size_t)e.floats);
            for (int r = 0; r < e.reps; ++r) copies.emplace_back(e.dev + r * e.floats, w, (size_t)e.floats);
            tables_dirty = tables_dirty || e.to == WT_TIME;
            continue;
        }
        const float* ride = e.key2.empty() ? nullptr : has(e.key2);
        if (!e.key2.empty() && (!w) != (!ride))
            return fail(DAD_E_KEY, "'%s' and '%s' share one packed image: refresh them together", e.key.c_str(), e.key2.c_str());
        if (!w) continue;
        dad::ImageDesc p = e.img;
        p.dst = e.dev; p.w = w; p.ride = ride;
        reps.push_back(p);
    }
    for (size_t at = 0; at < copies.size(); at += dad::COPY_MAX) {
        dad::CopyMany cm{};
        const int k = (int)std::min<size_t>(dad::COPY_MAX, copies.size() - at);
        size_t widest = 1;
        for (int i = 0; i < k; ++i) {
            cm.dst[i] = std::get<0>(copies[at + i]); cm.src[i] = std::get<1>(copies[at + i]);
            cm.n[i] = (int32_t)std::get<2>(copies[at + i]);
            widest = std::max(widest, std::get<2>(copies[at + i]));
        }
        const unsigned gx = (unsigned)std::min<size_t>(64, (widest + 1023) / 1024);
        hipLaunchKernelGGL(dad::copy_many_kernel, dim3(gx, (unsigned)k), dim3(256), 0, st, cm);
        HIP_TRY(hipGetLastError());
    }
    if (!reps.empty()) {
        std::vector<int> first(reps.size() + 1, 0);
        for (size_t i = 0; i < reps.size(); ++i) {
            const long blocks = (reps[i].n + 255) / 256;
            if (first[i] + blocks >= (1L << 31)) return fail(DAD_E_INVALID, "refresh: too many image elements for one launch");
            first[i + 1] = first[i] + (int)blocks;
        }
        const size_t desc_bytes = reps.size() * sizeof(dad::ImageDesc), first_bytes = first.size() * sizeof(int);
        const bool same = m->repack_host.size() == desc_bytes && std::memcmp(m->repack_host.data(), reps.data(), desc_bytes) == 0;
        if (!same) {
            if (m->repack_cap < desc_bytes + first_bytes) {
                void* a = nullptr;
                HIP_TRY(hipMalloc(&a, desc_bytes + first_bytes));
                m->owned.push_back(a);
                m->d_repack = a; m->repack_cap = desc_bytes + first_bytes;
            }
            HIP_TRY(hipStreamSynchronize(st));
            HIP_TRY(hipMemcpy(m->d_repack, reps.data(), desc_bytes, hipMemcpyHostToDevice));
            HIP_TRY(hipMemcpy((char*)m->d_repack + desc_bytes, first.data(), first_bytes, hipMemcpyHostToDevice));
            m->repack_host.assign((const char*)reps.data(), (const char*)reps.data() + desc_bytes);
        }
        hipLaunchKernelGGL(dad::repack_many_kernel, dim3((unsigned)first.back()), dim3(256), 0, st,
                           (const dad::ImageDesc*)m->d_repack, (const int*)((const char*)m->d_repack + desc_bytes), (int)reps.size());
        HIP_TRY(hipGetLastError());
    }
    if (tables_dirty) m->tables_stale = true;
    return DAD_OK;
}

int dad_train_grad_count(const dad_model* m, int32_t* count, int64_t* total_floats) {
    if (!m) return fail(DAD_E_INVALID, "null model");
    if (count) *count = (int32_t)m->grad_slots.size();
    if (total_floats) *total_floats = m->grad_numel;
    return DAD_OK;
}

int dad_train_grad_info(const dad_model* m, int32_t i, const char** key, int64_t* offset, int64_t* numel) {
    if (!m || i < 0 || i >= (int32_t)m->grad_slots.size()) return fail(DAD_E_INVALID, "gradient slot %d out of range", i);
    if (key) *key = m->grad_slots[i].key.c_str();
    if (offset) *offset = m->grad_slots[i].offset;
    if (numel) *numel = m->grad_slots[i].numel;
    return DAD_OK;
}

}

namespace {

int launch_wgrad(const dad_model* m, const BwdStep& s, const TrainScratch::Wgrad& w, const float* G, const float* Z0,
                 const float* Z1, float* out, float* wslab, hipStream_t st) {
    const WgradGeom& g = w.g;
    dad::WgradParams p{};
    p.G = G; p.ldg = s.M; p.M = s.M;
    p.Z0 = Z0; p.ldz0 = s.C0; p.C0 = s.C0; p.Z1 = Z1; p.ldz1 = s.C1; p.C1 = s.C1;
    p.out_numel = (long)s.M * (s.C0 + s.C1) * s.taps;
    p.out = g.ksplit > 1 ? wslab : out;
    p.B = w.sh.B; p.Lg = w.sh.Lg; p.Lz = w.sh.Lz; p.lg_shift = ilog2(w.sh.Lg); p.stride = s.stride; p.pad = s.pad;
    p.wshift = w.sh.wshift;
    p.ksplit = g.ksplit; p.samples_per_split = g.sps; p.spc = g.spc;
    p.zero = m->d_zero;
    void* args[] = {&p};
    HIP_TRY(hipLaunchKernel(wgrad_kernel(s.taps, g.tile, w.sh.wshift > 0), dim3(g.gx, g.gy, (unsigned)g.ksplit),
                            dim3(dad::WG_THREADS), args, g.lds, st));
    if (g.ksplit > 1) {
// ... 319 lines not shown
    if (rc != DAD_OK) return rc;
    if (saved_bytes < o.saved_bytes)
        return fail(DAD_E_WORKSPACE, "saved buffer has %zu bytes, the objective at batch %d needs %zu", saved_bytes, batch, o.saved_bytes);
    const dad_cfg& c = m->cfg;
    const int tdm = c.time_dim;
    const std::vector<TimeLaunch>& tl = plan.time;
    const float *w1 = time_tensor(m, "time_mlp.1.weight"), *b1 = time_tensor(m, "time_mlp.1.bias");
    const float *w3 = time_tensor(m, "time_mlp.3.weight"), *b3 = time_tensor(m, "time_mlp.3.bias");
    if (!w1 || !b1 || !w3 || !b3) return fail(DAD_E_KEY, "missing key 'time_mlp'");
    dad::TimeGemmParams g{};
    if ((rc = fill_time_blocks(m, g.tb, nullptr)) != DAD_OK) return rc;

    hipStream_t st = (hipStream_t)stream;
    float* const sv = (float*)((char*)saved + o.saved_base);
    dad::ObjectiveParams q = objective_params(m, o, sv, batch, loss_type, x0, noise, weights);
    q.t_in = t_rows; q.loss = loss_out;
    hipLaunchKernelGGL(dad::objective_xt_kernel, dim3((unsigned)((std::max<long>(q.n, batch) + 255) / 256)), dim3(dad::OBJ_THREADS), 0, st, q);
    HIP_TRY(hipGetLastError());
    g.emb = m->d_emb; g.t_rows = q.t_rows;
    g.w = w1; g.ldw = c.dim; g.bias = b1; g.out = sv + o.h1;
    if ((rc = launch_time_gemm<dad::TG_FWD_H1>(g, tl[0], st)) != DAD_OK) return rc;
    g.a = sv + o.h1; g.lda = 4 * tdm; g.w = w3; g.ldw = 4 * tdm; g.bias = b3; g.out = sv + o.temb; g.out2 = sv + o.act;
    if ((rc = launch_time_gemm<dad::TG_FWD_TEMB>(g, tl[1], st)) != DAD_OK) return rc;
    g.a = sv + o.act; g.lda = tdm; g.out = sv + o.rows; g.out2 = nullptr;
    if ((rc = launch_time_gemm<dad::TG_FWD_ROWS>(g, tl[2], st)) != DAD_OK) return rc;
    if ((rc = run_unet(m, f, q.xt, 0, (float*)saved, st, q.row_index, sv + o.rows)) != DAD_OK) return rc;
    if ((rc = run_final(m, f, nullptr, q.xt, 0, nullptr, 1, sv + o.out, (float*)saved, st)) != DAD_OK) return rc;
    hipLaunchKernelGGL(dad::objective_loss_partial_kernel, dim3((unsigned)q.nblocks), dim3(dad::OBJ_THREADS), 0, st, q);
    hipLaunchKernelGGL(dad::objective_loss_final_kernel, dim3(1), dim3(dad::OBJ_THREADS), 0, st, q);
    HIP_TRY(hipGetLastError());
    return DAD_OK;
}

int dad_train_objective_backward(dad_model* m, const float* x0, const float* noise, const float* weights, int32_t loss_type,
                                 const float* d_loss, float* const* grad_tensors, int32_t n_grad_tensors,
                                 float* const* time_grad_tensors, int32_t n_time_grad_tensors, int32_t batch, void* saved,
                                 size_t saved_bytes, void* scratch, size_t scratch_bytes, dad_stream_t stream) {
    if (!m) return fail(DAD_E_INVALID, "null model");
    if (!x0 || !noise || !d_loss || !grad_tensors || !time_grad_tensors || !saved || !scratch) return fail(DAD_E_INVALID, "null pointer");
    ObjectivePlan plan;
    int rc = check_objective(m, batch, loss_type, true, plan);
    const ObjectiveLayout& o = plan.o;
    if (rc != DAD_OK) return rc;
    if (n_grad_tensors != (int32_t)m->grad_slots.size())
        return fail(DAD_E_INVALID, "%d gradient tensors passed, the model has %zu (dad_train_grad_count)", n_grad_tensors, m->grad_slots.size());
    if (n_time_grad_tensors != (int32_t)m->time_grad_slots.size())
        return fail(DAD_E_INVALID, "%d time gradient tensors passed, the model has %zu (dad_train_time_grad_count)", n_time_grad_tensors,
                    m->time_grad_slots.size());
    for (int32_t i = 0; i < n_time_grad_tensors; ++i)
        if (!time_grad_tensors[i]) return fail(DAD_E_INVALID, "time gradient tensor %d ('%s') is null", i, m->time_grad_slots[i].key.c_str());
    if (saved_bytes < o.saved_bytes || scratch_bytes < o.scratch_bytes)
        return fail(DAD_E_WORKSPACE, "objective workspaces too small (saved %zu / %zu, scratch %zu / %zu bytes)", saved_bytes, o.saved_bytes,
                    scratch_bytes, o.scratch_bytes);
    float* const sv = (float*)((char*)saved + o.saved_base);
    float* const sc = (float*)((char*)scratch + o.scratch_base);
    const int tdm = m->cfg.time_dim, W = m->tplan.temb_width;
    const std::vector<TimeLaunch>& tl = plan.time;
    const float* w3 = time_tensor(m, "time_mlp.3.weight");
    if (!w3) return fail(DAD_E_KEY, "missing key 'time_mlp.3.weight'");
    dad::TimeGemmParams g{};
    if ((rc = fill_time_blocks(m, g.tb, time_grad_tensors)) != DAD_OK) return rc;

    hipStream_t st = (hipStream_t)stream;
    dad::ObjectiveParams q = objective_params(m, o, sv, batch, loss_type, x0, noise, weights);
    q.d_loss = d_loss; q.d_out = sc + o.d_out;
    const std::function<int()> head = [&]() -> int {
        hipLaunchKernelGGL(dad::objective_dout_kernel, dim3((unsigned)((q.n + 255) / 256)), dim3(dad::OBJ_THREADS), 0, st, q);
        HIP_TRY(hipGetLastError());
        return DAD_OK;
    };
    if ((rc = unet_backward(m, sv + o.xt, sc + o.d_out, nullptr, sc + o.d_rows, grad_tensors, n_grad_tensors, batch, saved, saved_bytes,
                            scratch, scratch_bytes, stream, &plan, &head)) != DAD_OK) return rc;
    g.emb = m->d_emb; g.t_rows = q.t_rows;
    g.a = sc + o.d_rows; g.lda = W; g.w = sv + o.act; g.ldw = tdm;
    if ((rc = launch_time_gemm<dad::TG_BWD_DWK>(g, tl[3], st)) != DAD_OK) return rc;
    g.out = sc + o.dact_slab;
    if ((rc = launch_time_gemm<dad::TG_BWD_DACT>(g, tl[4], st)) != DAD_OK) return rc;
    {
        const TimeLaunch& l = tl[5];
        if (l.mode != DAD_OP_TG_DTEMB) return fail(DAD_E_STATE, "time chain: launch %d planned where the slab sum runs", l.mode);
        hipLaunchKernelGGL(dad::time_dtemb_kernel, dim3(l.gx(), l.gy(), l.gz()), dim3(256), 0, st, sc + o.dtemb,
                           sc + o.dact_slab, sv + o.temb, (long)l.M * l.N, l.K);
        HIP_TRY(hipGetLastError());
    }
    g.a = sc + o.dtemb; g.lda = tdm; g.w = sv + o.h1; g.ldw = 4 * tdm; g.out = time_grad_tensors[2]; g.out2 = time_grad_tensors[3];
    if ((rc = launch_time_gemm<dad::TG_BWD_DW3>(g, tl[6], st)) != DAD_OK) return rc;
    g.w = w3; g.ldw = 4 * tdm; g.h1 = sv + o.h1; g.out = sc + o.dh1; g.out2 = nullptr;
    if ((rc = launch_time_gemm<dad::TG_BWD_DH1>(g, tl[7], st)) != DAD_OK) return rc;
    g.a = sc + o.dh1; g.lda = 4 * tdm; g.out = time_grad_tensors[0]; g.out2 = time_grad_tensors[1];
    return launch_time_gemm<dad::TG_BWD_DW1>(g, tl[8], st);
}

int dad_fill_normal(float* x, int32_t batch, int32_t row_elems, uint64_t seed, uint64_t row_offset,
                    uint64_t draw, dad_stream_t stream) {
    if (!x || batch <= 0 || row_elems <= 0) return fail(DAD_E_INVALID, "bad argument");
    const long n = (long)batch * row_elems;
    hipLaunchKernelGGL(dad::fill_normal_kernel, dim3((unsigned)((n + 255) / 256)), dim3(256), 0,
                       (hipStream_t)stream, x, n, row_offset * (uint64_t)row_elems, draw, seed);
    HIP_TRY(hipGetLastError());
    return DAD_OK;
}

#ifdef DAD_STAMPS
int dad_debug_stamps(void* buf) { g_stamps = (unsigned long long*)buf; return DAD_OK; }
#endif
int dad_debug_kernel_table_consistent(void) {
    const KernTable& t = kernel_table();
    size_t hits = 0;
    for (int cfg = 0; cfg < kNumTiles; ++cfg)
        for (int taps = 1; taps <= kRegMaxTaps; ++taps)
            for (int stride = 1; stride <= 2; ++stride)
                for (int f = 0; f < (1 << kRegFlags); ++f) {
                    const bool x3 = f & 1, bdir = f & 2, ragged = f & 4, res = f & 8, padded = f & 16, win = f & 32;
                    const bool have = t.count(KernKey(cfg, taps, stride, x3, bdir, ragged, res, padded, win)) != 0;
                    if (have != kernel_registered_f(cfg, taps, stride, f)) {
                        fail(DAD_E_INVALID, "kernel table mismatch at tile %d taps=%d stride=%d x3=%d bdir=%d ragged=%d res=%d padded=%d windowed=%d (registry %d)",
                             cfg, taps, stride, (int)x3, (int)bdir, (int)ragged, (int)res, (int)padded, (int)win, (int)have);
                        return 0;
                    }
                    hits += have;
                }
    return hits == t.size() ? 1 : 0;
}

#ifdef DAD_WG_STAMPS
extern "C" int dad_debug_wgrad_stamps(unsigned long long* host32) {
    HIP_TRY(hipDeviceSynchronize());
    HIP_TRY(hipMemcpyFromSymbol(host32, HIP_SYMBOL(dad::g_wg_stamps), 32 * sizeof(unsigned long long)));
    return DAD_OK;
}
#endif

int dad_debug_set_tile(dad_model* m, int32_t cfg) {
    if (!m) return fail(DAD_E_INVALID, "null model");
    m->split_enabled = cfg < 99;
    m->force_tile = cfg >= 99 ? cfg - 100 : cfg;
    return DAD_OK;
}

int dad_debug_set_option(dad_model* m, const char* name, int32_t value) {
    if (!m || !name) return fail(DAD_E_INVALID, "null argument");
    const std::string key(name);
    if (key == "fuse_residual") m->fuse_residual = value != 0;
    else if (key == "xswz") m->xswz_enabled = value != 0;
    else if (key == "xcd_order") m->xcd_order = value != 0;
    else if (key == "split_target") m->split_target = std::max(1, (int)value);
    else if (key == "cc") m->cc_enabled = value != 0;
    else if (key == "cc_max_rows") m->cc_max_rows = std::max(0, (int)value);
    else if (key == "ccw_max_rows") m->ccw_max_rows = std::max(0, (int)value);
    else if (key == "ccw_min_blocks") m->ccw_min_blocks = std::max(1, (int)value);
    else if (key == "ccw_prefer16") m->ccw_prefer16 = value != 0;
    else if (key == "wgrad_blocks") m->wgrad_blocks = std::max(1, (int)value);
    else if (key == "halo8") m->halo8_enabled = value != 0;
    else return fail(DAD_E_INVALID, "unknown option '%s'", name);
    if (!m->graphs.empty()) {
        HIP_TRY(hipDeviceSynchronize());
        for (auto& kv : m->graphs) (void)hipGraphExecDestroy(kv.second);
        m->graphs.clear();
    }
    return DAD_OK;
}

int dad_debug_read_table(dad_model* m, int32_t which, int32_t t, float* host_out, int32_t capacity,
                         int32_t* width_out) {
    if (!m || !host_out) return fail(DAD_E_INVALID, "null argument");
    if (!m->finalized) return fail(DAD_E_STATE, "dad_model_finalize has not been called");
    if (t < 0 || t >= m->cfg.n_timesteps)
        return fail(DAD_E_RANGE, "index %d is out of bounds for the schedule of size %d", t, m->cfg.n_timesteps);
    { const int rc = ensure_tables(m, nullptr); if (rc != DAD_OK) return rc; }
    const float* base = nullptr;
    int width = 0;
    switch (which) {
        case DAD_TABLE_SINUSOID: base = m->d_emb; width = m->cfg.dim; break;
        case DAD_TABLE_TIME_MLP: base = m->d_temb; width = m->cfg.time_dim; break;
        case DAD_TABLE_BLOCKS: base = m->d_temb_table; width = m->plan.temb_width; break;
        default: return fail(DAD_E_INVALID, "unknown table %d", which);
    }
    if (width_out) *width_out = width;
    if (capacity < width)
        return fail(DAD_E_INVALID, "table %d has rows of %d floats, the buffer holds %d", which, width, capacity);
    HIP_TRY(hipDeviceSynchronize());
    HIP_TRY(hipMemcpy(host_out, base + (size_t)t * width, (size_t)width * sizeof(float), hipMemcpyDeviceToHost));
    return DAD_OK;
}

int dad_debug_mish(const float* in, float* out, int64_t n, dad_stream_t stream) {
    if (!in || !out || n <= 0) return fail(DAD_E_INVALID, "bad argument");
    hipLaunchKernelGGL(dad::mish_probe_kernel, dim3((unsigned)((n + 255) / 256)), dim3(256), 0,
                       (hipStream_t)stream, in, out, (long)n);
    HIP_TRY(hipGetLastError());
    return DAD_OK;
}

int dad_debug_small_batch_plan(dad_model* m, int32_t batch, int32_t* launches_out, int32_t* wide_out) {
    if (!m || batch <= 0) return fail(DAD_E_INVALID, "bad argument");
    const CcPlan cc = cc_plan(*m, batch);
    int launches = 0, wide = 0;
    if (cc.ok)
        for (const CcOp& o : cc.ops) {
            launches += o.launched;
            wide += o.launched && o.wide;
        }
    static const bool trace = getenv("DAD_TRACE_TILES") != nullptr;
    if (trace && !cc.ok) fprintf(stderr, "[dad] batch %d: no small-batch plan (%s)\n", batch, cc.why.c_str());
    if (launches_out) *launches_out = launches;
    if (wide_out) *wide_out = wide;
    return DAD_OK;
}

int dad_debug_backward_plan(dad_model* m, int32_t batch, int32_t* out, int32_t capacity, int32_t* needed_out) {
    if (!m || batch <= 0 || capacity < 0 || (capacity > 0 && !out)) return fail(DAD_E_INVALID, "bad argument");
    if (!m->training) return fail(DAD_E_STATE, "dad_model_set_training(m, 1) has not been called");
    if (m->bwd_rc != DAD_OK) return fail(m->bwd_rc, "%s", m->bwd_err.c_str());
    std::vector<int32_t> r;
    const int rc = backward_plan_report(*m, batch, r);
    if (rc != DAD_OK) return rc;
    if (needed_out) *needed_out = (int32_t)r.size();
    std::copy(r.begin(), r.begin() + std::min<size_t>(r.size(), (size_t)capacity), out);
    return DAD_OK;
}

int dad_debug_backward_steps(dad_model* m, int32_t batch, int32_t* out, int32_t capacity, int32_t* needed_out) {
    if (!m || batch <= 0 || capacity < 0 || (capacity > 0 && !out)) return fail(DAD_E_INVALID, "bad argument");
    if (!m->training) return fail(DAD_E_STATE, "dad_model_set_training(m, 1) has not been called");
    if (m->bwd_rc != DAD_OK) return fail(m->bwd_rc, "%s", m->bwd_err.c_str());
    std::vector<int32_t> r;
    const int rc = backward_steps_report(*m, batch, r);
    if (rc != DAD_OK) return rc;
    if (needed_out) *needed_out = (int32_t)r.size();
    std::copy(r.begin(), r.begin() + std::min<size_t>(r.size(), (size_t)capacity), out);
    return DAD_OK;
}

int dad_debug_wgrad_kernel_exists(int32_t taps, int32_t tile, int32_t windowed) {
    return wgrad_kernel(taps, tile, windowed != 0) != nullptr ? 1 : 0;
}

int dad_debug_objective_plan(dad_model* m, int32_t batch, int32_t* out, int32_t capacity, int32_t* needed_out) {
    if (!m || batch <= 0 || capacity < 0 || (capacity > 0 && !out)) return fail(DAD_E_INVALID, "bad argument");
    if (!m->training) return fail(DAD_E_STATE, "dad_model_set_training(m, 1) has not been called");
    if (m->bwd_rc != DAD_OK) return fail(m->bwd_rc, "%s", m->bwd_err.c_str());
    std::vector<int32_t> r;
    const int rc = objective_plan_report(*m, batch, r);
    if (rc != DAD_OK) return rc;
    if (needed_out) *needed_out = (int32_t)r.size();
    std::copy(r.begin(), r.begin() + std::min<size_t>(r.size(), (size_t)capacity), out);
    return DAD_OK;
}

int dad_debug_forward_plan(dad_model* m, int32_t batch, int32_t mode, int32_t* out, int32_t capacity, int32_t* needed_out) {
    if (!m || batch <= 0 || mode < 0 || mode > 3 || capacity < 0 || (capacity > 0 && !out)) return fail(DAD_E_INVALID, "bad argument");
    if (mode >= 2 && !m->training) return fail(DAD_E_STATE, "dad_model_set_training(m, 1) has not been called");
    if (mode == 3 && m->bwd_rc != DAD_OK) return fail(m->bwd_rc, "%s", m->bwd_err.c_str());
    std::vector<int32_t> r;
    const int rc = forward_plan_report(*m, batch, mode, r);
    if (rc != DAD_OK) return rc;
    if (needed_out) *needed_out = (int32_t)r.size();
    std::copy(r.begin(), r.begin() + std::min<size_t>(r.size(), (size_t)capacity), out);
    return DAD_OK;
}

int dad_debug_project_plan(int32_t state_dim, int32_t observation_dim, int32_t action_dim, int32_t batch, int32_t horizon,
                           size_t scratch_bytes, int32_t violation, int32_t* out) {
    if (!out || state_dim <= 0 || observation_dim < state_dim || action_dim <= 0 || batch <= 0 || horizon <= 0)
        return fail(DAD_E_INVALID, "bad argument");
    const long D = (long)(horizon + 1) * state_dim + (long)horizon * action_dim;
    if (D > INT32_MAX / 64) return fail(DAD_E_INVALID, "projection dimension D=%ld too large", D);
    const size_t x_bytes = (size_t)batch * horizon * (observation_dim + action_dim) * sizeof(float);
    const ProjectPlan q = plan_project((int)D, batch, x_bytes, scratch_bytes, violation != 0);
    out[DAD_PP_FORM] = q.form;
    out[DAD_PP_ROWS_PER_BLOCK] = q.rows_per_block;
    out[DAD_PP_GX] = (int32_t)q.gx;
    out[DAD_PP_GY] = (int32_t)q.gy;
    out[DAD_PP_LDS_BYTES] = (int32_t)std::min<size_t>(q.lds_bytes, INT32_MAX);
    out[DAD_PP_REFUSED] = q.refused;
    return DAD_OK;
}

int dad_debug_kernel_registered(int32_t cfg, int32_t taps, int32_t stride, int32_t flags) {
    if (taps < 1 || taps > kRegMaxTaps || stride < 1 || stride > 2 || flags < 0 || flags >= (1 << kRegFlags)) return 0;
    return kernel_registered_f(cfg, taps, stride, flags) ? 1 : 0;
}

int dad_debug_small_kernel_exists(int32_t taps, int32_t stride, int32_t ride, int32_t wide, int32_t big, int32_t ride_in,
                                  int32_t rows, int32_t windowed) {
    return small_kernel_exists(taps, stride, ride != 0, wide != 0, big != 0, ride_in != 0, rows, windowed != 0) ? 1 : 0;
}

int dad_profile_enable(dad_model* m, int32_t on) {
    if (!m) return fail(DAD_E_INVALID, "null model");
    m->profile = on != 0;
    m->ev_used = 0;
    m->prof_flops = 0;
    m->prof_launches = 0;
    return DAD_OK;
}

int dad_profile_read(dad_model* m, double* conv_ms, int64_t* conv_launches, double* conv_flops) {
    if (!m) return fail(DAD_E_INVALID, "null model");
    double ms = 0;
    for (size_t i = 0; i < m->ev_used; ++i) {
        HIP_TRY(hipEventSynchronize(m->ev_pool[i].second));
        float d = 0;
        HIP_TRY(hipEventElapsedTime(&d, m->ev_pool[i].first, m->ev_pool[i].second));
        ms += d;
    }
    if (conv_ms) *conv_ms = ms;
    if (conv_launches) *conv_launches = m->prof_launches;
    if (conv_flops) *conv_flops = m->prof_flops;
    m->ev_used = 0;
    m->prof_flops = 0;
    m->prof_launches = 0;
    return DAD_OK;
}

}

struct dad_optim {
    struct Stage { void* host; size_t cap; hipEvent_t done; };
    std::vector<Stage> stages;
    std::vector<void*> owned;
    void* d_table = nullptr;
    size_t table_cap = 0;
    double* d_partials = nullptr;
    std::vector<char> image;
    std::vector<int64_t> numel;
    OptimPlan plan;
};

namespace {

int optim_upload(dad_optim* o, const std::vector<char>& image, hipStream_t st) {
    const size_t bytes = image.size();
    if (o->table_cap < bytes) {
        void* a = nullptr;
        HIP_TRY(hipMalloc(&a, bytes * 2));
        o->owned.push_back(a);
        o->d_table = a;
        o->table_cap = bytes * 2;
    }
    dad_optim::Stage* use = nullptr;
    for (auto& sg : o->stages) {
        if (sg.cap < bytes) continue;
        const hipError_t q = hipEventQuery(sg.done);
        if (q == hipSuccess) { use = &sg; break; }
        if (q != hipErrorNotReady) return fail(DAD_E_HIP, "hipEventQuery failed: %s", hipGetErrorString(q));
        (void)hipGetLastError();
    }
    if (!use) {
        dad_optim::Stage sg{nullptr, bytes * 2, nullptr};
        HIP_TRY(hipHostMalloc(&sg.host, sg.cap, hipHostMallocDefault));
        const hipError_t e = hipEventCreateWithFlags(&sg.done, hipEventDisableTiming);
        if (e != hipSuccess) {
            (void)hipHostFree(sg.host);
            return fail(DAD_E_HIP, "hipEventCreateWithFlags failed: %s", hipGetErrorString(e));
        }
        o->stages.push_back(sg);
        use = &o->stages.back();
    }
    std::memcpy(use->host, image.data(), bytes);
    HIP_TRY(hipMemcpyAsync(o->d_table, use->host, bytes, hipMemcpyHostToDevice, st));
    HIP_TRY(hipEventRecord(use->done, st));
    return DAD_OK;
}

}

extern "C" {

int dad_optim_create(dad_optim** out) {
    if (!out) return fail(DAD_E_INVALID, "null out");
    *out = new dad_optim();
    return DAD_OK;
}

void dad_optim_destroy(dad_optim* o) {
    if (!o) return;
    for (auto& sg : o->stages) { (void)hipEventDestroy(sg.done); (void)hipHostFree(sg.host); }
    for (void* p : o->owned) (void)hipFree(p);
    delete o;
}

int dad_optim_step(dad_optim* o, const dad_optim_tensor* tensors, int32_t n, const dad_optim_args* a, dad_stream_t s) {
    if (!o || !tensors || !a) return fail(DAD_E_INVALID, "optimiser step: null %s", !o ? "dad_optim" : !tensors ? "tensor list" : "arguments");
    if (n <= 0) return fail(DAD_E_INVALID, "optimiser step: n = %d tensors", n);
    if (!a->groups) return fail(DAD_E_INVALID, "optimiser step: null groups");
    if (a->n_groups <= 0 || a->n_groups > kOptimMaxGroups)
        return fail(DAD_E_INVALID, "optimiser step: %d groups (1 .. %d)", a->n_groups, kOptimMaxGroups);
    bool any_grad = false, same_numel = o->numel.size() == (size_t)n;
    for (int i = 0; i < n; ++i) {
        const dad_optim_tensor& t = tensors[i];
        if (!t.param) return fail(DAD_E_INVALID, "optimiser step: tensor %d has a null param", i);
        if (t.numel <= 0) return fail(DAD_E_INVALID, "optimiser step: tensor %d has numel %lld", i, (long long)t.numel);
        if (t.group < 0 || t.group >= a->n_groups)
            return fail(DAD_E_INVALID, "optimiser step: tensor %d is in group %d of %d", i, t.group, a->n_groups);
        if (t.grad && (!t.exp_avg || !t.exp_avg_sq))
            return fail(DAD_E_INVALID, "optimiser step: tensor %d has a grad but no %s", i, !t.exp_avg ? "exp_avg" : "exp_avg_sq");
        if (!t.grad && !t.ema) return fail(DAD_E_INVALID, "optimiser step: tensor %d has neither grad nor ema: nothing to do", i);
        any_grad = any_grad || t.grad;
        same_numel = same_numel && o->numel[(size_t)i] == t.numel;
    }
    if (!same_numel) {
        std::vector<int64_t> numel((size_t)n);
        for (int i = 0; i < n; ++i) numel[(size_t)i] = tensors[i].numel;
        OptimPlan p;
        const int rc = optim_plan(numel.data(), n, p);
        if (rc != DAD_OK) return rc;
        o->plan = std::move(p);
        o->numel = std::move(numel);
    }
    hipStream_t st = (hipStream_t)s;
    const size_t desc_bytes = (size_t)n * sizeof(dad::OptimDesc), first_bytes = o->plan.first.size() * sizeof(int32_t);
    std::vector<char> image(desc_bytes + first_bytes, 0);
    for (int i = 0; i < n; ++i) {
        const dad_optim_tensor& t = tensors[i];
        dad::OptimDesc d{};
        d.p = t.param; d.g = t.grad; d.m = t.exp_avg; d.v = t.exp_avg_sq; d.ema = t.ema;
        d.numel = t.numel; d.group = t.group;
        const uintptr_t bits = (uintptr_t)t.param | (uintptr_t)t.grad | (uintptr_t)t.exp_avg | (uintptr_t)t.exp_avg_sq | (uintptr_t)t.ema;
        d.vec = (bits & 15) == 0;
        std::memcpy(image.data() + (size_t)i * sizeof(dad::OptimDesc), &d, sizeof(d));
    }
    std::memcpy(image.data() + desc_bytes, o->plan.first.data(), first_bytes);
    if (image != o->image) {
        const int rc = optim_upload(o, image, st);
        if (rc != DAD_OK) { o->image.clear(); return rc; }
        o->image.swap(image);
    }
    if (!o->d_partials) {
        void* p = nullptr;
// ... 35 lines not shown
```

dynamics_aware_diffusion_amd/csrc/host_plan.hpp:

```cpp
#pragma once
#include <algorithm>
#include <array>
#include <cmath>
#include <cstdarg>
#include <cstdint>
#include <cstdio>
#include <cstdlib>
#include <cstring>
#include <functional>
#include <iterator>
#include <map>
#include <string>
#include <vector>

#include "../../include/dad.h"
#include "conv_shapes.hpp"
#include "weight_image.hpp"

namespace dadhost {

inline thread_local char g_err[1024] = "";

inline int fail(int code, const char* fmt, ...) {
    va_list ap;
    va_start(ap, fmt);
    vsnprintf(g_err, sizeof(g_err), fmt, ap);
    va_end(ap);
    return code;
}

struct HostTensor {
    std::vector<float> data;
    std::vector<int64_t> shape;
};

enum ConvKind { CONV_K5 = 0, CONV_1X1 = 1, CONV_DOWN = 2, CONV_UP = 3 };

struct ConvOp {
    std::string name;
    std::string norm;
    ConvKind kind;
    int taps, stride;
    int cin0, cin1, cin_pad;
    int cout;
    int M;
    int Lin, Lout;
    int src0, src1, dst, res;
    int temb_off;
    int kc = 16;
    bool x3 = false;
    bool bdir = false;
    int cat0 = -1, cat1 = -1, cat_c0 = 0, cat_c1 = 0;
    std::string rname;
    int rdst = -1;
    bool ride = false;
    int rider_of = -1;
    float c1 = 1.0f, c2 = 0.0f;
    int pre = -1, stats = -1;
    bool net_padded = false;
    int gn_real = 0;
    int lreal = 0;
    int src_len = 0;
    int real_in = 0, real_out = 0;
    float* d_w = nullptr;
    float* d_bias = nullptr;
    float* d_gamma = nullptr;
    float* d_beta = nullptr;
    float* d_rbias = nullptr;
    double flops_per_sample = 0;
    int wtaps() const { return taps + (ride ? 1 : 0); }
    bool padded() const { return gn_real > 0 || lreal > 0 || src_len > 0; }
};

struct Buf {
    long per_sample;
    long offset;
};

struct Plan {
    std::vector<ConvOp> convs;
    std::vector<Buf> bufs;
    long floats_per_sample = 0;
    int final_act = -1;
    int temb_width = 0;
};

constexpr int kMaxSplitTiles = 4096;
struct TileCfg { int BM, BN, SK, KC; };
constexpr int kNumTiles = 10;
constexpr TileCfg kTiles[kNumTiles] = {
    {32, 64, 4, 32},
    {64, 64, 2, 32},
    {128, 64, 1, 16},
    {256, 32, 1, 8},
    {64, 64, 1, 16},
    {32, 64, 2, 16},
    {32, 64, 1, 16},
    {64, 64, 2, 16},
    {32, 128, 2, 32},
    {64, 128, 1, 16},
};
constexpr int kMaxTileBN = 128;
constexpr bool kWinTiles[kNumTiles] = {true, true, true, false, false, false, false, false, false, false};
constexpr bool kPaddedTiles[kNumTiles] = {true, true, true, true, true, false, false, false, true, true};
constexpr int kGnPassMaxPair = dad::GNP_THREADS * 4 * dad::kGnPassMaxNpt;
inline bool windowed_layer(const ConvOp& op) { return op.Lout > kMaxTileBN; }
inline long tiles_n(const ConvOp& op, int BN, int batch) {
    if (op.Lout > BN) return (long)batch * (op.Lout / BN);
    const int spt = BN / op.Lout;
    return (batch + spt - 1) / spt;
}

constexpr int eff_kc(int cfg_kc, int bm, int taps, int sk = 1, bool x3 = false, bool bd = false, int bn = 64) {
    return bd                          ? 32
           : (taps == 1 && cfg_kc >= 16) ? (bn >= 128 ? 32 : bm >= 128 ? 64 : 128)
           : (x3 && cfg_kc < 16 * sk)  ? 16 * sk
                                       : cfg_kc;
}
constexpr int tile_kc(int cfg, int taps, bool x3, bool bdir) {
    return eff_kc(kTiles[cfg].KC, kTiles[cfg].BM, taps, kTiles[cfg].SK, x3, bdir, kTiles[cfg].BN);
}

enum BwdSpace : int8_t { BSP_NONE, BSP_ACT, BSP_GRAD, BSP_X, BSP_DOUT, BSP_DX };
struct BwdRef { BwdSpace sp = BSP_NONE; int buf = -1; };
enum BwdKind : int8_t {
    BK_BIAS,
    BK_WGRAD,
    BK_DGRAD,
    BK_GN,
    BK_RESID,
    BK_COLS,
};
enum BwdWrite : int8_t { BW_SET, BW_ADD, BW_STAGE };
struct BwdStep {
    BwdKind kind;
    BwdWrite write = BW_SET;
    int conv = -1;
    int sub = 0;
    BwdRef in, out;
    BwdRef z0, z1;
    int slot = -1;
    long part = 0;
    long n = 0;
    int rows = 0, C = 0;
    int off = 0, ld = 0;
    int M = 0, C0 = 0, C1 = 0, taps = 0, stride = 0, pad = 0, Lg = 0, Lz = 0;
    int nv = 0;
};
struct BwdSum { int slot; long part; int C; };

struct HostModel {
    dad_cfg cfg{};
    std::map<std::string, HostTensor> raw;
    std::map<std::string, std::vector<int64_t>> expected;
    Plan plan;
    Plan tplan;
    int precision = DAD_PREC_FP32;
    int force_tile = -1;
    bool split_enabled = true;
    bool fuse_residual = true;
    bool xswz_enabled = true;
    bool xcd_order = true;
    int split_target = 256;
    bool cc_enabled = true;
    int cc_max_rows = 512;
    int ccw_max_rows = 128;
    int ccw_min_blocks = 256;
    int real_channels[DAD_MAX_LEVELS] = {0};
    int real_horizon = 0;
    int wgrad_blocks = 256;
    bool ccw_prefer16 = true;
    mutable std::map<std::array<int, 5>, uint64_t> xswz_cache;
    bool halo8_enabled = true;
    mutable std::map<std::array<int, 3>, uint64_t> xswz8_cache;
    bool training = false;
    struct BwdConv {
        int n = 0;
        ConvOp op[2];
        int c_lo[2] = {0, 0};
        int c_n[2] = {0, 0};
    };
    std::vector<BwdConv> bconvs;
    ConvOp bfinal;
    struct GradSlot { std::string key; long offset, numel; };
    std::vector<GradSlot> grad_slots;
    long grad_numel = 0;
    std::vector<GradSlot> time_grad_slots;
    long time_grad_numel = 0;
    std::vector<BwdStep> bsteps;
    std::vector<BwdSum> bsums;
    long bpart = 0;
    bool bdx = false;
    int bwd_rc = DAD_OK;
    std::string bwd_err;
    int max_cout = 0;
    int max_bwd_m = 0;
};

inline int ilog2(int v) { int s = 0; while ((1 << s) < v) ++s; return s; }
inline bool is_pow2(int v) { return v > 0 && (v & (v - 1)) == 0; }

inline int check_cfg(const dad_cfg* cfg) {
    if (!cfg) return fail(DAD_E_INVALID, "null argument");
    if (cfg->kernel_size != 3 && cfg->kernel_size != 5 && cfg->kernel_size != 7)
        return fail(DAD_E_INVALID, "kernel_size %d unsupported (3, 5 or 7)", cfg->kernel_size);
    if (cfg->n_levels < 1 || cfg->n_levels > DAD_MAX_LEVELS)
        return fail(DAD_E_INVALID, "n_levels %d out of range", cfg->n_levels);
    if (cfg->transition_dim < 1 || cfg->dim < 4 || (cfg->dim & 1) || cfg->time_dim < 1)
        return fail(DAD_E_INVALID, "bad transition_dim/dim/time_dim");
    if (!is_pow2(cfg->horizon) || (cfg->horizon >> (cfg->n_levels - 1)) < 4)
        return fail(DAD_E_INVALID, "horizon %d must be a power of two with horizon / 2^(levels-1) >= 4",
                    cfg->horizon);
    if (cfg->n_timesteps < 1) return fail(DAD_E_INVALID, "n_timesteps must be positive");
    for (int i = 0; i < cfg->n_levels; ++i) {
        const int ch = cfg->channels[i];
        if (ch < 32 || ch % 32 != 0 || !is_pow2(ch / 8))
            return fail(DAD_E_INVALID, "level %d has %d channels: need a multiple of 32 with C/8 a power of two",
                        i, ch);
    }
    if (cfg->dim % 32 != 0) return fail(DAD_E_INVALID, "dim %d must be a multiple of 32", cfg->dim);
    return DAD_OK;
}

struct Allocator {
    std::vector<Buf>& bufs;
    std::vector<bool> in_use;
    bool retain;
    explicit Allocator(std::vector<Buf>& b, bool keep = false) : bufs(b), retain(keep) {}
    int get(long per_sample) {
        int best = -1;
        for (size_t i = 0; i < bufs.size() && !retain; ++i)
            if (!in_use[i] && bufs[i].per_sample >= per_sample &&
                (best < 0 || bufs[i].per_sample < bufs[best].per_sample))
                best = (int)i;
        if (best < 0) {
            bufs.push_back({per_sample, 0});
            in_use.push_back(false);
            best = (int)bufs.size() - 1;
        }
        in_use[best] = true;
        return best;
    }
    void put(int id) { if (id >= 0) in_use[id] = false; }
};

inline void expect(HostModel* m, const std::string& key, std::vector<int64_t> shape) {
    m->expected[key] = std::move(shape);
}

inline void decide_kernel_families(HostModel* m) {
    bool padded_net = m->real_horizon > 0 && m->real_horizon != m->cfg.horizon;
    for (int i = 0; i < m->cfg.n_levels; ++i) padded_net = padded_net || (m->real_channels[i] > 0 && m->real_channels[i] != m->cfg.channels[i]);
    for (Plan* plan : {&m->plan, &m->tplan})
    for (ConvOp& op : plan->convs) {
        const int cin_all = op.cin0 + op.cin1;
        op.bdir = op.kc == 8 && op.kind == CONV_K5 &&
                  (op.cin0 % 32) == 0 && (cin_all % 32) == 0 && op.cin_pad == cin_all;
        const bool win = windowed_layer(op);
        op.ride = !op.rname.empty() && !op.bdir && m->precision == DAD_PREC_FP32 && !padded_net && !win;
        op.x3 = !padded_net && !win && ((op.bdir && m->precision == DAD_PREC_F16X3) ||
                (m->precision == DAD_PREC_F16X3 && op.kc == 16 &&
                 ((op.kind == CONV_K5 && op.taps == 5) || op.kind == CONV_1X1 ||
                  ((op.kind == CONV_DOWN || op.kind == CONV_UP) && (op.cin0 & 63) == 0 && (cin_all & 63) == 0))));
        op.net_padded = padded_net;
    }
}

inline int build_plan_into(HostModel* m, Plan& P, bool retain) {
    const dad_cfg& c = m->cfg;
    P = Plan();
    Allocator A(P.bufs, retain);
    const int k = c.kernel_size;
    const int tdm = c.time_dim;
    int temb_off = 0;

    int level_now = 0;
    const bool rows_padded = m->real_horizon > 0 && m->real_horizon != c.horizon;
    int Lr_now = rows_padded ? m->real_horizon : c.horizon;
    auto conv = [&](const std::string& name, const std::string& norm, ConvKind kind, int src0,
                    int src1, int cin0, int cin1, int cout, int Lin, int dst, int res,
                    int toff) {
        ConvOp op;
        op.name = name; op.norm = norm; op.kind = kind;
        const int real = m->real_channels[level_now];
        if (!norm.empty() && real > 0 && real != cout) op.gn_real = real / 8;
        if (rows_padded) {
            const int lr_out = kind == CONV_DOWN ? Lr_now / 2 : Lr_now;
            const int lp_out = kind == CONV_DOWN ? Lin / 2 : Lin;
            if (lr_out != lp_out) op.lreal = lr_out;
            if (src0 == -2) op.src_len = Lr_now;
            op.real_in = Lr_now;
            op.real_out = kind == CONV_DOWN ? Lr_now / 2 : kind == CONV_UP ? 2 * Lr_now : Lr_now;
        }
        op.cin0 = cin0; op.cin1 = cin1;
        op.kc = (!norm.empty() && cout / 8 >= 256) ? 8 : 16;
        const int padto = op.kc == 8 ? 8 : (kind == CONV_1X1 ? 128 : 64);
        op.cin_pad = (cin0 + cin1 + padto - 1) / padto * padto;
        op.cout = cout; op.src0 = src0; op.src1 = src1; op.dst = dst; op.res = res;
        op.temb_off = toff; op.Lin = Lin;
        const int cin = cin0 + cin1;
        switch (kind) {
            case CONV_K5: op.taps = k; op.stride = 1; op.M = cout; op.Lout = Lin;
                expect(m, name + ".weight", {cout, cin, k});
                op.flops_per_sample = 2.0 * cout * cin * k * Lin; break;
            case CONV_1X1: op.taps = 1; op.stride = 1; op.M = cout; op.Lout = Lin;
                expect(m, name + ".weight", {cout, cin, 1});
                op.flops_per_sample = 2.0 * cout * cin * Lin; break;
            case CONV_DOWN: op.taps = 3; op.stride = 2; op.M = cout; op.Lout = Lin / 2;
                expect(m, name + ".weight", {cout, cin, 3});
                op.flops_per_sample = 2.0 * cout * cin * 3 * (Lin / 2); break;
            case CONV_UP: op.taps = 2; op.stride = 1; op.M = 2 * cout; op.Lout = Lin;
                expect(m, name + ".weight", {cin, cout, 4});
                op.flops_per_sample = 2.0 * cout * cin * 4 * Lin; break;
        }
        expect(m, name + ".bias", {cout});
        if (!norm.empty()) {
            expect(m, norm + ".weight", {cout});
            expect(m, norm + ".bias", {cout});
            if (retain) { op.pre = A.get((long)cout * op.Lout); op.stats = A.get(16); }
        }
        P.convs.push_back(op);
    };

    auto realw = [&](int level) { return m->real_channels[level] > 0 ? m->real_channels[level] : c.channels[level]; };
    bool padded_net = false;
    for (int i = 0; i < c.n_levels; ++i) padded_net = padded_net || realw(i) != c.channels[i];
    const char* plan_error = nullptr;
// ... 881 lines not shown
            if (slice % 32 != 0) return refuse(P, "K slice not a multiple of 32 channels");
            o.tile_rows = 32;
            if (op.Lout <= 16) {
                const int ks = (cin + slice - 1) / slice;
                const long blocks16 = (long)((batch + 16 / op.Lout - 1) / (16 / op.Lout)) * (op.M / 32) * ks;
                if (blocks16 <= 256) o.tile_rows = 16;
            }
        } else {
            if (op.src0 == -2 || (op.cin0 & 3) || (op.cin1 & 3) || max_slabs_in > kCcwMaxSlabs ||
                max_pair > kCcwMaxPair)
                return refuse(P, "wide layer: ragged channels, more than 8 slabs to add, or a GroupNorm pair above 8192 elements");
            auto try_rows = [&](int rows) -> int {
                auto fits = [&](int sl) {
                    return dad::ccw_lds_floats(sl, op.taps, op.Lin, op.Lout, rows) * sizeof(float) <= dad::kLdsBytes;
                };
                const int spt_r = rows / op.Lout;
                const long nt = (batch + spt_r - 1) / spt_r;
                int sl = need;
                while (sl % 32 != 0) sl += need;
                while ((cin + sl - 1) / sl > kCcwMaxSlabs) sl *= 2;
                while ((long)((cin + 2 * sl - 1) / (2 * sl)) * (op.M / 32) * nt >= m.ccw_min_blocks && 2 * sl <= cin && fits(2 * sl) &&
                       (op.cin1 == 0 || op.cin0 % (2 * sl) == 0))
                    sl *= 2;
                return fits(sl) ? sl : 0;
            };
            o.tile_rows = 32;
            if (op.Lout <= 16 && (batch + 16 / op.Lout - 1) / (16 / op.Lout) == (batch + 32 / op.Lout - 1) / (32 / op.Lout))
                o.tile_rows = 16;
            slice = try_rows(o.tile_rows);
            if (o.tile_rows == 32 && op.Lout <= 16 && m.ccw_prefer16) {
                const int s16 = try_rows(16);
                if (slice == 0 || s16 >= 2 * slice) { o.tile_rows = 16; slice = s16; }
            }
            if (slice == 0) return refuse(P, "wide layer: no K slice of at most 8 slabs fits LDS");
            const int spt_w = o.tile_rows / op.Lout;
            int min_cpg = slice;
            for (const CcInput* in : {&o.in0, &o.in1})
                if (in->kind == 3 && !convs[in->producer].norm.empty())
                    min_cpg = std::min(min_cpg, convs[in->producer].cout / 8);
            if ((long)spt_w * (slice / min_cpg) > kCcwMaxPairs) return refuse(P, "wide layer: more than 64 (sample, group) pairs per block");
        }
        if (op.cin1 > 0 && op.cin0 % slice != 0) return refuse(P, "a K slice would straddle the concat");
        o.slice_ch = slice;
        o.kslices = (cin + slice - 1) / slice;
        if ((long)o.kslices * slice > op.cin_pad) return refuse(P, "weight image too short for whole K slices");
        if (!op.norm.empty() && (long)(op.cout / 8) * op.Lout > kCcwMaxPair) return refuse(P, "GroupNorm pair above 8192 elements");
        const int spt = windowed ? 1 : o.tile_rows / op.Lout;
        o.ntiles = windowed ? batch * (op.Lout / 32) : (batch + spt - 1) / spt;
        o.out_rows = op.kind == CONV_UP ? batch * 2 * op.Lout : batch * op.Lout;
        o.out_cols = op.kind == CONV_UP ? op.M / 2 : op.M;
        o.oslab = off;
        off += (long)o.kslices * o.out_rows * o.out_cols;
        if (op.ride) { o.orslab = off; off += (long)o.kslices * o.out_rows * o.out_cols; }
        o.lds_bytes = (o.wide ? dad::ccw_lds_floats(slice, op.taps, op.Lin, op.Lout, o.tile_rows)
                              : dad::cc_lds_floats(slice, op.taps, op.wtaps(), op.Lin, op.Lout, o.tile_rows)) * sizeof(float);
        if (o.lds_bytes > dad::kLdsBytes) return refuse(P, "a launch does not fit LDS");
        o.big = max_slabs_in > dad::CC_MAX_SLABS;
        if (!cc_kernel_exists(op.taps, op.stride, op.ride, o.wide, o.big, o.tile_rows, windowed)) return refuse(P, "a launch no small-batch kernel exists for");
        if (op.res == -2) o.res_kind = 1;
        else if (op.res >= 0) {
            const int q = owner[op.res];
            if (q <= -2) { o.res_kind = 3; o.res_ride = -2 - q; }
            else if (q >= 0 && materialised[q]) { o.res_kind = 2; o.res_buf = op.res; }
            else if (q >= 0 && convs[q].kind == CONV_1X1 && convs[q].norm.empty() && P.ops[q].launched) {
                o.res_kind = 4; o.res_ride = q;
            } else return refuse(P, "residual tensor neither finished nor a 1x1 conv in pieces");
        }
        owner[op.dst] = (int)i;
    }
    P.final_producer = owner[m.plan.final_act];
    if (P.final_producer < 0 || materialised[P.final_producer]) return refuse(P, "final conv input already finished");
    for (const CcOp& o : P.ops)
        if (o.launched && o.wide && (long)batch * c.horizon > m.ccw_max_rows) return refuse(P, "wide layers and more than ccw_max_rows rows");
    {
        const ConvOp& f = convs[P.final_producer];
        if ((long)(f.cout / 8) * f.Lout > 1024) return refuse(P, "final conv: GroupNorm pair above 1024 elements");
        if (P.ops[P.final_producer].kslices > 8) return refuse(P, "final conv: more than 8 partial slabs");
    }
    P.slab_floats = off;
    P.ok = true;
    return P;
}

struct FirstRefusal {
    int rc = DAD_OK;
    std::string why;
    void note(int r) { if (r != DAD_OK && rc == DAD_OK) { rc = r; why = g_err; } }
    int done() const { return rc == DAD_OK ? DAD_OK : fail(rc, "%s", why.c_str()); }
};
inline int traj_horizon(const HostModel& m) { return m.real_horizon > 0 ? m.real_horizon : m.cfg.horizon; }

struct FwdLaunch {
    int conv;
    bool ok;
    LaunchGeom g;
};
struct FwdPlan {
    bool train = false;
    int batch = 0;
    CcPlan cc;
    std::vector<FwdLaunch> launches;
    unsigned final_gx = 1, final_gy = 1;
    size_t final_lds = 0;
    size_t bytes = 0;
};
inline int plan_forward(const HostModel& m, bool train, int batch, bool small_ok, FwdPlan& f) {
    const Plan& plan = train ? m.tplan : m.plan;
    const dad_cfg& c = m.cfg;
    FirstRefusal first;
    f = FwdPlan();
    f.train = train; f.batch = batch;
    long scratch = 0;
    if (!train) {
        CcPlan cc = cc_plan(m, batch);
        if (cc.ok) scratch = cc.slab_floats;
        if (cc.ok && small_ok) f.cc = std::move(cc);
    }
    std::vector<char> carries(plan.convs.size(), 0);
    for (size_t i = 0; i < plan.convs.size(); ++i) {
        const ConvOp& op = plan.convs[i];
        FwdLaunch l{(int)i, true, LaunchGeom()};
        const bool listed = !f.cc.ok && !(op.rider_of >= 0 && carries[op.rider_of]);
        if (listed) { const int rc = plan_launch(m, op, batch, l.g); l.ok = rc == DAD_OK; first.note(rc); }
        else choose_launch(m, op, batch, l.g);
        if (listed && l.ok && !train) choose_halo8(m, op, l.g);
        carries[i] = l.g.fused;
        scratch = std::max(scratch, l.g.split.slab_floats);
        if (listed) f.launches.push_back(l);
    }
    f.bytes = ((size_t)plan.floats_per_sample * (size_t)batch + (size_t)scratch) * sizeof(float);
    if (f.cc.ok) {
        const int want = (c.horizon * c.transition_dim + dad::CC_THREADS - 1) / dad::CC_THREADS;
        f.final_gx = (unsigned)batch;
        f.final_gy = (unsigned)std::max(1, std::min({want, c.transition_dim, 256 / std::max(batch, 1)}));
        f.final_lds = dad::final_cc_lds_floats(c.transition_dim, c.dim, c.horizon) * sizeof(float);
    } else {
        const long row_tiles = ((long)batch * traj_horizon(m) + dad::FINAL_COLS - 1) / dad::FINAL_COLS;
        const long col_groups = (c.transition_dim + 256 / dad::FINAL_COLS - 1) / (256 / dad::FINAL_COLS);
        long gy = std::max(1L, std::min(col_groups, 512 / row_tiles));
        while (gy < col_groups && dad::final_lds_floats(c.transition_dim, c.dim, (int)gy) * sizeof(float) > dad::kLdsBytes) ++gy;
        f.final_gx = (unsigned)row_tiles; f.final_gy = (unsigned)gy;
        f.final_lds = dad::final_lds_floats(c.transition_dim, c.dim, (int)gy) * sizeof(float);
    }
    if (f.final_lds > dad::kLdsBytes)
        first.note(fail(DAD_E_INVALID, "final 1x1 conv does not fit LDS (td=%d, dim=%d)", c.transition_dim, c.dim));
    return first.done();
}
inline size_t workspace_bytes(const HostModel& m, int batch) {
    FwdPlan f;
    plan_forward(m, false, batch, true, f);
    return f.bytes;
}

struct ProjectPlan {
    int form = DAD_PP_ROW1;
    int rows_per_block = 1;
    unsigned gx = 1, gy = 1;
    size_t lds_bytes = 0;
    bool refused = false;
};
inline ProjectPlan plan_project(int D, int batch, size_t x_bytes, size_t scratch_bytes, bool violation) {
    ProjectPlan q;
    const size_t row_lds = dad::project_row_lds_bytes(D);
    const bool gemm_pays = D >= 512 || row_lds > dad::kLdsBytes;
    if (!violation && gemm_pays && batch >= 32 && scratch_bytes > 0 && scratch_bytes >= x_bytes) {
        q.form = DAD_PP_GEMM;
        q.rows_per_block = 32;
        q.gx = (unsigned)((batch + 31) / 32); q.gy = (unsigned)((D + 31) / 32);
        q.lds_bytes = dad::project_gemm_lds_floats() * sizeof(float);
        return q;
    }
    const int rb = (batch > 512 && 4 * row_lds <= dad::kLdsBytes) ? 4 : 1;
    q.form = rb == 4 ? DAD_PP_ROW4 : DAD_PP_ROW1;
    q.rows_per_block = rb;
    q.gx = (unsigned)((batch + rb - 1) / rb);
    q.lds_bytes = rb * row_lds;
    q.refused = q.lds_bytes > dad::kLdsBytes;
    return q;
}

constexpr int kWgradTaps[] = {1, 3, 4, 5, 7};
struct WgradGeom { int spc, ksplit, sps, tile, tm, tn; unsigned gx, gy; size_t lds; };
constexpr int kWgradWindow = 64;
struct WgradShape { int B, Lg, Lz, wshift; };
inline WgradShape wgrad_shape(int B, int Lg, int Lz) {
    if (Lg <= 128 && Lz <= 128) return {B, Lg, Lz, 0};
    const int nw = Lg / kWgradWindow;
    return {B * nw, kWgradWindow, Lz / nw, ilog2(nw)};
}
inline WgradGeom wgrad_geom(int M, int Ctot, int B, int Lg, int Lz, int taps, int pad, int target, bool ragged) {
    WgradGeom g{};
    g.spc = std::max(1, dad::WG_ROWS / Lg);
    while (g.spc > 1 && g.spc * dad::wgrad_segz(Lz, taps, pad) > dad::WG_MAX_ZROWS) g.spc /= 2;
    static const int tms[3] = {2, 2, 1}, tns[3] = {2, 1, 1};
    long tiles = 0;
    for (g.tile = ragged ? 2 : 0; g.tile < 3; ++g.tile) {
        g.tm = tms[g.tile]; g.tn = tns[g.tile];
        g.gx = (unsigned)((M + 32 * g.tm - 1) / (32 * g.tm));
        g.gy = (unsigned)((Ctot + 32 * g.tn - 1) / (32 * g.tn));
        tiles = (long)g.gx * g.gy;
        const int kgroups = 8 / (g.tm * g.tn);
        if ((tiles >= 32 && (g.spc * Lg) % (4 * kgroups) == 0) || g.tile == 2) break;
    }
    const int chunks = (B + g.spc - 1) / g.spc;
    int want = (int)std::max(1L, target / tiles);
    want = std::min(want, chunks);
    g.sps = (chunks + want - 1) / want * g.spc;
    g.ksplit = (B + g.sps - 1) / g.sps;
    g.lds = dad::wgrad_lds_floats(g.spc, Lg, Lz, taps, pad, g.tm, g.tn) * sizeof(float);
    if (ragged) g.tile = 3;
    return g;
}

struct TrainScratch {
    long mirror = 0, part = 0, wslab = 0, dxpad = 0, tmp = 0, bslab = 0, total = 0;
    struct Wgrad { WgradShape sh; WgradGeom g; };
    struct Dgrad { bool ok; LaunchGeom g; };
    std::vector<Wgrad> wgrads;
    std::vector<Dgrad> dgrads;
};
inline const ConvOp& bwd_op(const HostModel& m, const BwdStep& s) { return s.conv < 0 ? m.bfinal : m.bconvs[s.conv].op[s.sub]; }
inline int train_scratch(const HostModel& m, int B, TrainScratch& t) {
    const int H = m.cfg.horizon, td = m.cfg.transition_dim;
    FirstRefusal first;
    t = TrainScratch();
    t.mirror = m.tplan.floats_per_sample * (long)B;
    for (const ConvOp& f : m.tplan.convs) t.part += (f.norm.empty() ? 1L : 3L) * B * round_up(f.cout, 4);
    t.part += (long)B * round_up(td, 4);
    for (const BwdStep& s : m.bsteps) {
        if (s.kind == BK_WGRAD) {
            const WgradShape sh = wgrad_shape(B, s.Lg, s.Lz);
            const bool ragged = ((s.M | s.C0 | s.C1) & 3) != 0;
            const WgradGeom g = wgrad_geom(s.M, s.C0 + s.C1, sh.B, sh.Lg, sh.Lz, s.taps, s.pad, m.wgrad_blocks, ragged);
            const long numel = (long)s.M * (s.C0 + s.C1) * s.taps;
            const int kgroups = 8 / (g.tm * g.tn);
            if (g.lds > dad::kLdsBytes || g.spc * sh.Lg > dad::WG_MAX_GROWS ||
                g.spc * dad::wgrad_segz(sh.Lz, s.taps, s.pad) > dad::WG_MAX_ZROWS || (g.spc * sh.Lg) % (4 * kgroups) != 0)
                first.note(fail(DAD_E_INVALID, "wgrad: a chunk of %d samples x %d rows does not fit the kernel's staging", g.spc, sh.Lz));
            if (std::find(std::begin(kWgradTaps), std::end(kWgradTaps), s.taps) == std::end(kWgradTaps))
                first.note(fail(DAD_E_INVALID, "wgrad: %d taps", s.taps));
            if (g.ksplit > 1 && numel % 4 != 0)
                first.note(fail(DAD_E_INVALID, "wgrad: %ld gradient elements (not a multiple of 4)", numel));
            if (g.ksplit > 1) t.wslab = std::max(t.wslab, (long)g.ksplit * numel);
            t.wgrads.push_back({sh, g});
        } else if (s.kind == BK_DGRAD) {
            const ConvOp& op = bwd_op(m, s);
            TrainScratch::Dgrad d{};
            const int rc = plan_launch(m, op, B, d.g);
            d.ok = rc == DAD_OK;
            first.note(rc);
            t.bslab = std::max(t.bslab, d.g.split.slab_floats);
            t.dgrads.push_back(d);
            if (op.kind == CONV_UP) t.tmp = std::max(t.tmp, (long)B * s.n);
        }
    }
    t.dxpad = (long)B * H * round_up(td, 32);
    if (m.real_horizon > 0 && m.real_horizon != H) t.dxpad += 2L * B * H * round_up(td, 4);
    auto al = [](long v) { return (v + 63) / 64 * 64; };
    t.mirror = al(t.mirror); t.part = al(t.part); t.wslab = al(t.wslab); t.dxpad = al(t.dxpad);
    t.tmp = al(t.tmp); t.bslab = al(t.bslab);
    t.total = t.mirror + t.part + t.wslab + t.dxpad + t.tmp + t.bslab;
    if (m.bpart * B > t.part)
        first.note(fail(DAD_E_WORKSPACE, "backward: partial sums overran their region (%ld > %ld floats)", m.bpart * B, t.part));
    return first.done();
}

struct ObjectiveLayout {
    long xt = 0, out = 0, t_rows = 0, row_index = 0, h1 = 0, temb = 0, act = 0, rows = 0, partial = 0, saved_floats = 0;
    long d_out = 0, d_rows = 0, dact_slab = 0, dtemb = 0, dh1 = 0, scratch_floats = 0;
    int loss_blocks = 1;
    int kslices = 1;
    int kslice = 0;
    size_t saved_base = 0, scratch_base = 0;
    size_t saved_bytes = 0, scratch_bytes = 0;
};
constexpr int kObjectiveMaxLossBlocks = 1024;
struct TimeLaunch {
    int mode, M, N, K, kslice, kslices;
    unsigned gx() const { return mode == DAD_OP_TG_DTEMB ? (unsigned)(((long)M * N + 255) / 256) : (unsigned)((M + 31) / 32); }
    unsigned gy() const { return mode == DAD_OP_TG_DTEMB ? 1u : (unsigned)((N + 31) / 32); }
    unsigned gz() const { return mode == DAD_OP_TG_DTEMB ? 1u : (unsigned)kslices; }
};
constexpr int kObjectiveForwardLaunches = 3, kObjectiveTimeLaunches = 9;
struct ObjectivePlan { ObjectiveLayout o; FwdPlan fwd; TrainScratch ts; std::vector<TimeLaunch> time; };
inline int objective_plan(const HostModel& m, int B, bool backward, ObjectivePlan& p) {
    ObjectiveLayout& o = p.o;
    FwdPlan& f = p.fwd;
    TrainScratch& ts = p.ts;
    o = ObjectiveLayout();
    FirstRefusal first;
    first.note(plan_forward(m, true, B, false, f));
    ts = TrainScratch();
    if (backward) first.note(train_scratch(m, B, ts));
    const long tdm = m.cfg.time_dim, W = std::max(1, m.tplan.temb_width);
    const long n = (long)B * traj_horizon(m) * m.cfg.transition_dim;
    auto al = [](long v) { return (v + 63) / 64 * 64; };
    o.loss_blocks = (int)std::max(1L, std::min((long)kObjectiveMaxLossBlocks, (n + 1023) / 1024));
    const long tiles = (long)((B + 31) / 32) * ((tdm + 31) / 32);
    const long want = std::max(1L, std::min(256 / tiles, (W + 127) / 128));
    o.kslice = (int)(((W + want - 1) / want + 127) / 128 * 128);
    o.kslices = (int)((W + o.kslice - 1) / o.kslice);
    long at = 0;
    auto take = [&](long floats) { const long q = at; at += al(floats); return q; };
    o.xt = take(n); o.out = take(n); o.t_rows = take(B); o.row_index = take(B);
    o.h1 = take(B * 4 * tdm); o.temb = take(B * tdm); o.act = take(B * tdm); o.rows = take(B * W);
    o.partial = take(o.loss_blocks);
// ... 309 lines not shown
```

include/dad.h:

```cpp
#ifndef DAD_H
#define DAD_H

#include <stddef.h>
#include <stdint.h>

#ifdef __cplusplus
extern "C" {
#endif

#define DAD_OK 0
#define DAD_E_INVALID (-1)
#define DAD_E_STATE (-2)
#define DAD_E_KEY (-3)
#define DAD_E_HIP (-4)
#define DAD_E_RANGE (-5)
#define DAD_E_WORKSPACE (-6)

#define DAD_MAX_LEVELS 8

#define DAD_PREC_FP32 0
#define DAD_PREC_F16X3 1

typedef struct dad_model dad_model;
typedef void* dad_stream_t;
// ... 160 lines not shown
#define DAD_BS_RECORD_INTS 1
#define DAD_BS_BATCH 2
#define DAD_BS_COLSUMS_LAUNCHES 3
#define DAD_BS_COLSUMS_ENTRIES 4
#define DAD_BS_COLSUMS_WIDEST 5
#define DAD_BS_PADCOPY 6
#define DAD_BS_HORIZON 7
#define DAD_BS_REAL_HORIZON 8
#define DAD_BS_DX 9
#define DAD_BS_HEADER 12
#define DAD_BS_K_BIAS 0
#define DAD_BS_K_WGRAD 1
#define DAD_BS_K_DGRAD 2
#define DAD_BS_K_GN 3
#define DAD_BS_K_RESID 4
#define DAD_BS_K_COLS 5
#define DAD_BS_KIND 0
#define DAD_BS_BIAS_ROWS 1
#define DAD_BS_BIAS_C 2
#define DAD_BS_WG_TAPS 1
#define DAD_BS_WG_TILE 2
#define DAD_BS_WG_WINDOWED 3
#define DAD_BS_WG_M 4
#define DAD_BS_WG_C0 5
#define DAD_BS_WG_C1 6
#define DAD_BS_WG_STRIDE 7
#define DAD_BS_WG_PAD 8
#define DAD_BS_WG_LG 9
#define DAD_BS_WG_LZ 10
#define DAD_BS_WG_GX 11
#define DAD_BS_WG_GY 12
#define DAD_BS_WG_RAGGED 13
#define DAD_BS_WG_CONCAT_INSIDE 14
#define DAD_BS_WG_EDGE_M 15
#define DAD_BS_WG_EDGE_C 16
#define DAD_BS_WG_SWAPPED 17
#define DAD_BS_WG_KSPLIT 18
#define DAD_BS_WG_SLAB_N4 19
#define DAD_BS_WG_SAMPLES 20
#define DAD_BS_WG_SPC 21
#define DAD_BS_WG_SPS 22
#define DAD_BS_WG_CHUNKS 23
#define DAD_BS_WG_LAST_CHUNKS 24
#define DAD_BS_DG_CONV 1
#define DAD_BS_DG_SUB 2
#define DAD_BS_DG_WRITE 3
#define DAD_BS_GN_NV 1
#define DAD_BS_GN_CPG 2
#define DAD_BS_GN_L 3
#define DAD_BS_GN_LREAL 4
#define DAD_BS_GN_CPG_REAL 5
#define DAD_BS_GN_DTEMB 6
#define DAD_BS_GN_SHORT_PAIR 7
#define DAD_BS_GN_C 8
#define DAD_BS_RS_WRITE 1
#define DAD_BS_RS_N 2
#define DAD_BS_RS_TO_X 3
#define DAD_BS_CL_C 1
#define DAD_BS_CL_OFF 2
#define DAD_BS_CL_LD 3
#define DAD_BS_CL_ROWS 4
#define DAD_BS_CL_WRITE 5
#define DAD_BS_REC_INTS 25
int dad_debug_backward_steps(dad_model* m, int32_t batch, int32_t* out, int32_t capacity, int32_t* needed_out);
int dad_debug_wgrad_kernel_exists(int32_t taps, int32_t tile, int32_t windowed);

#define DAD_OP_LOSS_BLOCKS 0
#define DAD_OP_KSLICES 1
#define DAD_OP_KSLICE 2
#define DAD_OP_TEMB_WIDTH 3
#define DAD_OP_BLOCKS 4
#define DAD_OP_N 5
#define DAD_OP_RECORD_INTS 6
#define DAD_OP_LAUNCHES 7
#define DAD_OP_HEADER 8
#define DAD_OP_REC_MODE 0
#define DAD_OP_REC_M 1
#define DAD_OP_REC_N 2
#define DAD_OP_REC_K 3
#define DAD_OP_REC_GRID_X 4
#define DAD_OP_REC_GRID_Y 5
#define DAD_OP_REC_GRID_Z 6
#define DAD_OP_REC_CHUNKS 7
#define DAD_OP_REC_LAST_CHUNKS 8
#define DAD_OP_REC_KTAIL 9
#define DAD_OP_REC_KSLICE 10
#define DAD_OP_REC_INTS 11
#define DAD_OP_TG_FWD_H1 0
#define DAD_OP_TG_FWD_TEMB 1
#define DAD_OP_TG_FWD_ROWS 2
#define DAD_OP_TG_BWD_DWK 3
#define DAD_OP_TG_BWD_DACT 4
#define DAD_OP_TG_BWD_DW3 5
#define DAD_OP_TG_BWD_DH1 6
#define DAD_OP_TG_BWD_DW1 7
#define DAD_OP_TG_DTEMB 8
int dad_debug_objective_plan(dad_model* m, int32_t batch, int32_t* out, int32_t capacity, int32_t* needed_out);

#define DAD_FP_MODE 0
#define DAD_FP_BATCH 1
#define DAD_FP_SMALL 2
#define DAD_FP_RECORDS 3
#define DAD_FP_RECORD_INTS 4
#define DAD_FP_FINAL_GX 5
#define DAD_FP_FINAL_GY 6
#define DAD_FP_FINAL_KERNEL 7
#define DAD_FP_HEADER 8
#define DAD_FP_FINAL_NONE 0
#define DAD_FP_FINAL_POSTERIOR 1
#define DAD_FP_FINAL_CC 2
#define DAD_FP_REC_CONV 0
#define DAD_FP_REC_SUB 1
#define DAD_FP_REC_CFG 2
#define DAD_FP_REC_TAPS 3
#define DAD_FP_REC_STRIDE 4
#define DAD_FP_REC_FLAGS 5
#define DAD_FP_REC_KC 6
#define DAD_FP_REC_KSLICES 7
#define DAD_FP_REC_GN_NPT 8
#define DAD_FP_REC_NTILES_N 9
#define DAD_FP_REC_MTILES 10
#define DAD_FP_REC_PART_TILE 11
#define DAD_FP_REC_FAMILY 12
#define DAD_FP_REC_INTS 13
#define DAD_FP_FAMILY_GEMM 0
#define DAD_FP_FAMILY_HALO8 1
#define DAD_FP_CC_CONV 0
#define DAD_FP_CC_TAPS 1
#define DAD_FP_CC_STRIDE 2
#define DAD_FP_CC_WIDE 3
#define DAD_FP_CC_RIDE 4
#define DAD_FP_CC_BIG 5
#define DAD_FP_CC_RIDE_IN 6
#define DAD_FP_CC_TILE_ROWS 7
#define DAD_FP_CC_WINDOWED 8
#define DAD_FP_CC_SLICE_CH 9
#define DAD_FP_CC_KSLICES 10
#define DAD_FP_CC_NTILES 11
#define DAD_FP_CC_RES_KIND 12
#define DAD_FP_CC_INTS 13
int dad_debug_forward_plan(dad_model* m, int32_t batch, int32_t mode, int32_t* out, int32_t capacity, int32_t* needed_out);
#define DAD_PP_FORM 0
#define DAD_PP_ROWS_PER_BLOCK 1
#define DAD_PP_GX 2
#define DAD_PP_GY 3
#define DAD_PP_LDS_BYTES 4
#define DAD_PP_REFUSED 5
#define DAD_PP_INTS 6
#define DAD_PP_ROW1 0
#define DAD_PP_ROW4 1
#define DAD_PP_GEMM 2
int dad_debug_project_plan(int32_t state_dim, int32_t observation_dim, int32_t action_dim, int32_t batch, int32_t horizon,
                           size_t scratch_bytes, int32_t violation, int32_t* out);
int dad_debug_kernel_registered(int32_t cfg, int32_t taps, int32_t stride, int32_t flags);
int dad_debug_small_kernel_exists(int32_t taps, int32_t stride, int32_t ride, int32_t wide, int32_t big, int32_t ride_in,
                                  int32_t rows, int32_t windowed);

typedef struct dad_optim dad_optim;
typedef struct dad_optim_tensor {
    float* param;
    const float* grad;
    float* exp_avg;
    float* exp_avg_sq;
    float* ema;
    int64_t numel;
    int32_t group;
} dad_optim_tensor;
typedef struct dad_optim_group {
    float lr, beta1, beta2, eps, weight_decay, step_size, bc2_sqrt;
    int32_t decoupled;
    float one_minus_beta1, one_minus_beta2;
} dad_optim_group;
typedef struct dad_optim_args {
    const dad_optim_group* groups;
    int32_t n_groups;
    float max_grad_norm;
    float ema_decay;
    float* grad_norm_out;
} dad_optim_args;
int dad_optim_create(dad_optim** out);
void dad_optim_destroy(dad_optim* o);
int dad_optim_step(dad_optim* o, const dad_optim_tensor* tensors, int32_t n, const dad_optim_args* a, dad_stream_t s);
#define DAD_OS_CHUNK 0
#define DAD_OS_CHUNKS 1
#define DAD_OS_GRID 2
#define DAD_OS_PARTIALS 3
#define DAD_OS_RECORD_INTS 4
#define DAD_OS_HEADER 5
#define DAD_OS_REC_TENSOR 0
#define DAD_OS_REC_FIRST 1
#define DAD_OS_REC_FIRST_HI 2
#define DAD_OS_REC_COUNT 3
#define DAD_OS_REC_BLOCK 4
#define DAD_OS_REC_INTS 5
int dad_debug_optim_plan(const int64_t* numel, int32_t n, int32_t* out, int32_t capacity, int32_t* needed_out);

#ifdef __cplusplus
}
#endif
#endif
```

Measured before the change: 3522 plans/s.

## Fuse final conv and posterior step into next step's first conv

Adds a seam kernel that runs the previous denoising step's final 1x1 conv, posterior update and noise sampling, then the next step's first 5-tap conv with GroupNorm, Mish and the riding residual conv, all in one launch. Intermediate x values stay in LDS instead of going through global memory, and one kernel launch per step is removed. It is on by default through a new step_seam option, gated by a planner with many eligibility checks. The cost is a larger, register-heavy kernel with a large LDS footprint, which may lower occupancy, plus extra code paths for correctness.

```diff
diff --git a/dynamics_aware_diffusion_amd/_engine.py b/dynamics_aware_diffusion_amd/_engine.py
--- a/dynamics_aware_diffusion_amd/_engine.py
+++ b/dynamics_aware_diffusion_amd/_engine.py
@@ -141,6 +141,8 @@
     "dad_debug_forward_plan": (C.c_int, [C.c_void_p, C.c_int32, C.c_int32, C.POINTER(C.c_int32), C.c_int32,
                                          C.POINTER(C.c_int32)]),
     "dad_debug_project_plan": (C.c_int, [C.c_int32] * 5 + [C.c_size_t, C.c_int32, C.POINTER(C.c_int32)]),
+    "dad_debug_seam_plan": (C.c_int, [C.c_void_p, C.c_int32, C.c_int32, C.POINTER(C.c_int32)]),
+    "dad_debug_seam_reason": (C.c_char_p, [C.c_int32]),
     "dad_debug_kernel_registered": (C.c_int, [C.c_int32] * 4),
     "dad_debug_small_kernel_exists": (C.c_int, [C.c_int32] * 8),
     "dad_optim_create": (C.c_int, [C.POINTER(C.c_void_p)]),
@@ -214,6 +216,7 @@
 FP_FLAGS = ("x3", "bdir", "ragged", "res", "padded", "windowed")
 PP_FIELDS = ("form", "rows_per_block", "gx", "gy", "lds_bytes", "refused")
 PP_FORMS = ("row1", "row4", "gemm")
+SEAM_FIELDS = ("taken", "reason", "grid", "threads", "lds_bytes", "tile", "units")
 
 
 def registered_kernels():
@@ -749,6 +752,14 @@
                                                            out.data_ptr(), out.numel(), C.byref(width)))
         return out[:width.value].clone()
 
+    def seam_plan(self, batch: int, *, projection: bool = False) -> dict:
+        out = (C.c_int32 * len(SEAM_FIELDS))()
+        _check(self.lib, self.lib.dad_debug_seam_plan(self._h, int(batch), int(bool(projection)), out))
+        q = dict(zip(SEAM_FIELDS, out))
+        q["taken"] = bool(q["taken"])
+        q["reason"] = self.lib.dad_debug_seam_reason(q["reason"]).decode()
+        return q
+
     def small_batch_plan(self, batch: int):
         n, w = C.c_int32(), C.c_int32()
         _check(self.lib, self.lib.dad_debug_small_batch_plan(self._h, int(batch), C.byref(n), C.byref(w)))
diff --git a/dynamics_aware_diffusion_amd/csrc/conv_seam.hpp b/dynamics_aware_diffusion_amd/csrc/conv_seam.hpp
--- /dev/null
+++ b/dynamics_aware_diffusion_amd/csrc/conv_seam.hpp
@@ -0,0 +1,326 @@
+#pragma once
+#include "pointwise.hpp"
+
+namespace dad {
+
+struct SeamParams {
+    FinalParams f;
+    ConvParams c;
+    int32_t units;
+    int32_t hshift;
+};
+
+__device__ __forceinline__ bool posterior_finish(const FinalParams& p, const float* bl, long n, int td, int b, int l, int j,
+                                                 float acc, float xv, float zpre, float& xn) {
+    const long idx = n * td + j;
+    const float out = acc + bl[j];
+    if (p.eps_out != nullptr) p.eps_out[idx] = out;
+    if (p.x_out_disabled && p.mean_out == nullptr) return false;
+    float x0 = out, mean;
+    {
+#pragma clang fp contract(off)
+        if (p.predict_epsilon) x0 = p.c_recip * xv - p.c_recipm1 * out;
+        if (p.clip_denoised) x0 = fminf(fmaxf(x0, -1.0f), 1.0f);
+        mean = p.coef1 * x0 + p.coef2 * xv;
+    }
+    if (p.guide != nullptr) mean = fmaf(p.guide_scale, p.guide[idx], mean);
+    if (p.mean_out != nullptr) p.mean_out[idx] = mean;
+    if (p.x_out_disabled) return false;
+    const float z = (p.noise != nullptr)
+                        ? zpre
+                        : philox_normal(p.elem_offset + (uint64_t)idx, p.draw,
+                                        p.seed_dev != nullptr ? (uint64_t)*p.seed_dev : p.seed);
+    xn = fmaf(p.sigma, z, mean);
+    if (l == 0 && p.cond0 != nullptr) xn = p.cond0[(p.cond_per_row ? (long)b * td : 0) + j];
+    p.x[idx] = xn;
+    return true;
+}
+
+__device__ __forceinline__ void seam_store_f4_sc1(float* p, const float4 v) {
+    typedef float __attribute__((ext_vector_type(4))) f4;
+    const f4 x = {v.x, v.y, v.z, v.w};
+    asm volatile("global_store_dwordx4 %0, %1, off sc1\n\ts_nop 7" ::"v"(p), "v"(x) : "memory");
+}
+
+template <int DIM, bool T0>
+__global__ __launch_bounds__(4 * DIM) void conv_seam_f32(const SeamParams q) {
+    constexpr int NT = seam_threads(DIM), TMW = DIM / 32, ES = DIM + 4, KP = SEAM_KP, TAPS = 5, PAD = TAPS / 2;
+    constexpr int JG = NT / 32;
+    constexpr int JB = 16 / JG;
+    constexpr int DQ = DIM / 4;
+    static_assert(DIM == 32 || DIM == 64 || DIM == 128, "dim");
+    static_assert(T0 || DIM >= 64, "tile 1 needs 64 output channels");
+
+    extern __shared__ __attribute__((aligned(16))) float smem[];
+    float4* const smem4 = reinterpret_cast<float4*>(smem);
+    const FinalParams& p = q.f;
+    const ConvParams& c = q.c;
+    const int td = p.td, H = p.H, hsh = q.hshift;
+    const int tid = threadIdx.x;
+    const int lane = tid & 63;
+    const int wave = __builtin_amdgcn_readfirstlane(tid >> 6);
+    const int l32 = lane & 31;
+    const int h = lane >> 5;
+    const int SPT = 32 >> hsh, SEG = H + 2 * PAD;
+    const int XF = seam_xf(H);
+    float* const tile = smem;
+    float* const wl = tile + 32 * ES;
+    float* const bl = wl + td * DIM;
+    float* const xs = bl + ((td + 3) & ~3);
+    float* const ER = xs + XF;
+    const int xs4 = (int)(xs - smem) >> 2;
+    const long N = (long)p.B * H;
+    const long n0 = (long)blockIdx.x * 32;
+    const int s0 = (int)blockIdx.x * SPT;
+    const int nvalid = min(SPT, p.B - s0);
+    const int M = c.M;
+
+    float4 areg[2];
+#pragma unroll
+    for (int i = 0; i < 2; ++i) {
+        const int e = tid + i * NT;
+        const int row = e / DQ, qd = e - row * DQ;
+        areg[i] = ldg4(p.act + min(n0 + row, N - 1) * DIM + qd * 4);
+    }
+    const float4 wreg = ldg4(p.w + (long)min(tid, td * DQ - 1) * 4);
+    const float breg = p.bias[min(tid, td - 1)];
+    const int col = tid & 31;
+    const int jg = tid >> 5;
+    const long n = n0 + col;
+    const long nc = min(n, N - 1);
+    const float* const zsrc = p.noise != nullptr ? p.noise : p.x;
+    float xv[JB], zv[JB];
+#pragma unroll
+    for (int k = 0; k < JB; ++k) {
+        const long at = nc * td + min(jg + k * JG, td - 1);
+        xv[k] = p.x[at];
+        zv[k] = zsrc[at];
+    }
+    const bool rider = wave >= TMW;
+    const int tm = rider ? wave - TMW : wave;
+    float4 wf[TAPS][2];
+    {
+        const float* const base = c.w + (long)(tm * 32 + l32) * 16 + 4 * h;
+#pragma unroll
+        for (int t = 0; t < TAPS; ++t)
+#pragma unroll
+            for (int g = 0; g < 2; ++g) {
+                const int slot = rider ? TAPS : t;
+                wf[t][g] = ldg4(base + (long)slot * M * 16 + g * 8);
+            }
+    }
+    constexpr int CPG = DIM / 8, CQ = CPG / 4;
+    constexpr int CQ_SH = CQ == 1 ? 0 : CQ == 2 ? 1 : 2;
+    const int cnt4 = H * CQ;
+    const int lpp = T0 ? cnt4 : cnt4 >> 1;
+    const int lpp_sh = 31 - __clz(lpp);
+    int erow[2], ecol[2], eoff[2];
+    float4 bias4[2], gam4[2], bet4[2], temb4[2], rb4[2];
+    const float* const tptr = c.temb != nullptr ? c.temb : c.bias;
+    const bool has_temb = c.temb != nullptr;
+#pragma unroll
+    for (int k = 0; k < 2; ++k) {
+        const int vt = T0 ? 2 * tid + k : tid;
+        const int pr = vt >> lpp_sh, lp = vt & (lpp - 1);
+        const int ps = pr >> 3, pg = pr & 7;
+        const int j = T0 ? lp : lp + k * lpp;
+        erow[k] = ps * H + (j >> CQ_SH);
+        ecol[k] = pg * CPG + (j & (CQ - 1)) * 4;
+        const int s = erow[k] >> hsh;
+        eoff[k] = ((s0 + s) * H + (erow[k] & (H - 1))) * M + ecol[k];
+        if (s >= nvalid) eoff[k] = -1;
+        bias4[k] = ldg4(c.bias + ecol[k]);
+        gam4[k] = ldg4(c.gamma + ecol[k]);
+        bet4[k] = ldg4(c.beta + ecol[k]);
+        temb4[k] = ldg4(tptr + ecol[k]);
+        rb4[k] = ldg4(c.rbias + ecol[k]);
+    }
+
+    for (int i = tid; i < (XF >> 2); i += NT) smem4[xs4 + i] = make_float4(0.f, 0.f, 0.f, 0.f);
+#pragma unroll
+    for (int i = 0; i < 2; ++i) {
+        const int e = tid + i * NT;
+        const int row = e / DQ, qd = e - row * DQ;
+        float4 v = areg[i];
+        if (n0 + row >= N) v = make_float4(0.f, 0.f, 0.f, 0.f);
+        *reinterpret_cast<float4*>(tile + row * ES + qd * 4) = v;
+    }
+    if (tid < td * DQ) *reinterpret_cast<float4*>(wl + tid * 4) = wreg;
+    if (tid < td) bl[tid] = breg;
+    __syncthreads();
+
+    if (n < N) {
+        const int s = col >> hsh, l = col & (H - 1);
+        const int b = s0 + s;
+        float* const xrow = xs + (s * SEG + PAD + l) * KP + (int)((c.xswz >> (4 * s)) & 15) * 4;
+#pragma unroll
+        for (int k = 0; k < JB; ++k) {
+            const int j = jg + k * JG;
+            if (j >= td) continue;
+            float acc;
+            final_dots<1>(wl + j * DIM, tile + col * ES, DIM, 0, &acc);
+            float xn;
+            if (posterior_finish(p, bl, n, td, b, l, j, acc, xv[k], zv[k], xn)) xrow[j] = xn;
+        }
+    }
+    __syncthreads();
+
+    {
+        const int arow4 = xs4 + ((((l32 >> hsh) * SEG + (l32 & (H - 1))) * KP + 4 * h) >> 2) + (int)((c.xswz >> (4 * (l32 >> hsh))) & 15);
+        auto frag_a = [&](int tap, int g) -> float4 { return smem4[arow4 + tap * (KP / 4) + g * 2]; };
+        const int units = q.units;
+        f32x16 tot;
+        if (!rider) {
+            f32x16 a1, a2, a3, a4;
+#pragma unroll
+            for (int r = 0; r < 16; ++r) { a1[r] = 0.0f; a2[r] = 0.0f; a3[r] = 0.0f; a4[r] = 0.0f; tot[r] = 0.0f; }
+#define DAD_SEAM_MAIN(T, G)                                                                      \
+    {                                                                                            \
+        const float4 a = frag_a(T, G), w = wf[T][G];                                             \
+        a1 = __builtin_amdgcn_mfma_f32_32x32x2f32(a.x, w.x, a1, 0, 0, 0);                        \
+        a2 = __builtin_amdgcn_mfma_f32_32x32x2f32(a.y, w.y, a2, 0, 0, 0);                        \
+        a3 = __builtin_amdgcn_mfma_f32_32x32x2f32(a.z, w.z, a3, 0, 0, 0);                        \
+        a4 = __builtin_amdgcn_mfma_f32_32x32x2f32(a.w, w.w, a4, 0, 0, 0);                        \
+    }
+            if constexpr (T0) {
+#pragma unroll
+                for (int t = 0; t < TAPS; ++t) DAD_SEAM_MAIN(t, 0)
+#pragma unroll
+                for (int r = 0; r < 16; ++r) tot[r] = (a1[r] + a2[r]) + (a3[r] + a4[r]);
+                if (units > 1) {
+#pragma unroll
+                    for (int r = 0; r < 16; ++r) { a1[r] = 0.0f; a2[r] = 0.0f; a3[r] = 0.0f; a4[r] = 0.0f; }
+#pragma unroll
+                    for (int t = 0; t < TAPS; ++t) DAD_SEAM_MAIN(t, 1)
+#pragma unroll
+                    for (int r = 0; r < 16; ++r) tot[r] += (a1[r] + a2[r]) + (a3[r] + a4[r]);
+                }
+            } else {
+                if (units > 1) {
+#pragma unroll
+                    for (int t = 0; t < TAPS; ++t) { DAD_SEAM_MAIN(t, 0) DAD_SEAM_MAIN(t, 1) }
+                } else {
+#pragma unroll
+                    for (int t = 0; t < TAPS; ++t) DAD_SEAM_MAIN(t, 0)
+                }
+#pragma unroll
+                for (int r = 0; r < 16; ++r) tot[r] = (a1[r] + a2[r]) + (a3[r] + a4[r]);
+            }
+#undef DAD_SEAM_MAIN
+        } else {
+            f32x16 r1, r2;
+#pragma unroll
+            for (int r = 0; r < 16; ++r) { r1[r] = 0.0f; r2[r] = 0.0f; tot[r] = 0.0f; }
+#define DAD_SEAM_RIDE(G)                                                                         \
+    {                                                                                            \
+        const float4 a = frag_a(PAD, G), w = wf[0][G];                                           \
+        r1 = __builtin_amdgcn_mfma_f32_32x32x2f32(a.x, w.x, r1, 0, 0, 0);                        \
+        r2 = __builtin_amdgcn_mfma_f32_32x32x2f32(a.y, w.y, r2, 0, 0, 0);                        \
+        r1 = __builtin_amdgcn_mfma_f32_32x32x2f32(a.z, w.z, r1, 0, 0, 0);                        \
+        r2 = __builtin_amdgcn_mfma_f32_32x32x2f32(a.w, w.w, r2, 0, 0, 0);                        \
+    }
+            DAD_SEAM_RIDE(0)
+            if constexpr (T0) {
+#pragma unroll
+                for (int r = 0; r < 16; ++r) tot[r] = r1[r] + r2[r];
+                if (units > 1) {
+#pragma unroll
+                    for (int r = 0; r < 16; ++r) { r1[r] = 0.0f; r2[r] = 0.0f; }
+                    DAD_SEAM_RIDE(1)
+#pragma unroll
+                    for (int r = 0; r < 16; ++r) tot[r] += r1[r] + r2[r];
+                }
+            } else {
+                if (units > 1) DAD_SEAM_RIDE(1)
+#pragma unroll
+                for (int r = 0; r < 16; ++r) tot[r] = r1[r] + r2[r];
+            }
+#undef DAD_SEAM_RIDE
+        }
+        float* const E = rider ? ER : tile;
+#pragma unroll
+        for (int r = 0; r < 16; ++r) E[((r & 3) + 8 * (r >> 2) + 4 * h) * ES + tm * 32 + l32] = tot[r];
+    }
+    __syncthreads();
+
+    float y[2][4];
+#pragma unroll
+    for (int k = 0; k < 2; ++k) {
+        const float4 r = *reinterpret_cast<const float4*>(ER + erow[k] * ES + ecol[k]);
+        if (eoff[k] >= 0)
+            seam_store_f4_sc1(c.rdst + eoff[k], make_float4(r.x + rb4[k].x, r.y + rb4[k].y, r.z + rb4[k].z, r.w + rb4[k].w));
+        const float4 v = *reinterpret_cast<const float4*>(tile + erow[k] * ES + ecol[k]);
+        y[k][0] = v.x; y[k][1] = v.y; y[k][2] = v.z; y[k][3] = v.w;
+    }
+#pragma unroll
+    for (int k = 0; k < 2; ++k) {
+        y[k][0] += bias4[k].x; y[k][1] += bias4[k].y; y[k][2] += bias4[k].z; y[k][3] += bias4[k].w;
+    }
+    {
+        const float inv_cnt = 1.0f / (float)(cnt4 * 4);
+        const int vwidth = lpp < 64 ? lpp : 64;
+        const int width = T0 ? vwidth >> 1 : vwidth;
+        auto pair_sum = [&](float v) -> float {
+            if (width >= 2) v += dpp_f32<0xB1>(v);
+            if (width >= 4) v += dpp_f32<0x4E>(v);
+            if (width >= 8) v += dpp_f32<0x141>(v);
+            if (width >= 16) v += dpp_f32<0x140>(v);
+            if (width >= 32) v = rows_sum(v, width, lane);
+            if (T0 && lpp > 64) {
+                const int iv = __builtin_bit_cast(int, v);
+                const float w0 = __builtin_bit_cast(float, __builtin_amdgcn_readlane(iv, 0));
+                const float w1 = __builtin_bit_cast(float, __builtin_amdgcn_readlane(iv, 32));
+                v = 0.0f;
+                v += w0;
+                v += w1;
+            }
+            return v;
+        };
+        float sum;
+        if constexpr (T0) {
+            float sa = 0.0f, sb = 0.0f;
+            sa += (y[0][0] + y[0][1]) + (y[0][2] + y[0][3]);
+            sb += (y[1][0] + y[1][1]) + (y[1][2] + y[1][3]);
+            sum = sa + sb;
+        } else {
+            sum = 0.0f;
+#pragma unroll
+            for (int k = 0; k < 2; ++k) sum += (y[k][0] + y[k][1]) + (y[k][2] + y[k][3]);
+        }
+        const float mean = pair_sum(sum) * inv_cnt;
+        float sq;
+        {
+#pragma clang fp contract(off)
+            float dd[2][4];
+#pragma unroll
+            for (int k = 0; k < 2; ++k)
+#pragma unroll
+                for (int cc = 0; cc < 4; ++cc) { const float d = y[k][cc] - mean; dd[k][cc] = d * d; }
+            const float qa = ((dd[0][0] + dd[0][1]) + dd[0][2]) + dd[0][3];
+            if constexpr (T0) {
+                const float qb = ((dd[1][0] + dd[1][1]) + dd[1][2]) + dd[1][3];
+                sq = qa + qb;
+            } else {
+                sq = (((qa + dd[1][0]) + dd[1][1]) + dd[1][2]) + dd[1][3];
+            }
+        }
+        const float rstd = 1.0f / sqrtf(pair_sum(sq) * inv_cnt + 1e-5f);
+#pragma unroll
+        for (int k = 0; k < 2; ++k) {
+            y[k][0] = mish_fast_f32((y[k][0] - mean) * rstd * gam4[k].x + bet4[k].x);
+            y[k][1] = mish_fast_f32((y[k][1] - mean) * rstd * gam4[k].y + bet4[k].y);
+            y[k][2] = mish_fast_f32((y[k][2] - mean) * rstd * gam4[k].z + bet4[k].z);
+            y[k][3] = mish_fast_f32((y[k][3] - mean) * rstd * gam4[k].w + bet4[k].w);
+        }
+    }
+#pragma unroll
+    for (int k = 0; k < 2; ++k) {
+        if (eoff[k] < 0) continue;
+        const float4 t4 = has_temb ? temb4[k] : make_float4(0.f, 0.f, 0.f, 0.f);
+        const float4 r4 = make_float4(0.f, 0.f, 0.f, 0.f);
+        seam_store_f4_sc1(c.dst + eoff[k], make_float4(y[k][0] + (t4.x + r4.x), y[k][1] + (t4.y + r4.y),
+                                                  y[k][2] + (t4.z + r4.z), y[k][3] + (t4.w + r4.w)));
+    }
+}
+
+}
diff --git a/dynamics_aware_diffusion_amd/csrc/conv_shapes.hpp b/dynamics_aware_diffusion_amd/csrc/conv_shapes.hpp
--- a/dynamics_aware_diffusion_amd/csrc/conv_shapes.hpp
+++ b/dynamics_aware_diffusion_amd/csrc/conv_shapes.hpp
@@ -71,6 +71,13 @@
     return (size_t)final_rows_local(td, gy) * dim + ((td + 3) & ~3) + (size_t)FINAL_COLS * (dim + 4);
 }
 
+constexpr int SEAM_KP = 20;
+DAD_HD constexpr int seam_threads(int dim) { return 4 * dim; }
+DAD_HD inline int seam_xf(int H) { return (32 / H) * (H + 4) * SEAM_KP + kXSwzPad; }
+DAD_HD inline size_t seam_lds_floats(int td, int dim, int H) {
+    return (size_t)2 * 32 * (dim + 4) + (size_t)td * dim + ((td + 3) & ~3) + (size_t)seam_xf(H);
+}
+
 constexpr int GNP_THREADS = 256;
 constexpr int kGnPassMaxNpt = 32;
 
diff --git a/dynamics_aware_diffusion_amd/csrc/dad_lib.hip b/dynamics_aware_diffusion_amd/csrc/dad_lib.hip
--- a/dynamics_aware_diffusion_amd/csrc/dad_lib.hip
+++ b/dynamics_aware_diffusion_amd/csrc/dad_lib.hip
@@ -23,6 +23,7 @@
 #include "conv_halo8.hpp"
 #include "conv_gn_pass.hpp"
 #include "pointwise.hpp"
+#include "conv_seam.hpp"
 #include "conv_cc.hpp"
 #include "conv_ccw.hpp"
 #include "train_bwd.hpp"
@@ -254,6 +255,20 @@
 }
 const void* halo8_kernel(int cfg, bool res) { return find_kernel(halo8_kernels(), cfg, res, 0); }
 
+const FamilyList& seam_kernels() {
+    static const FamilyList list = [] {
+        FamilyList v;
+        v.push_back({{32, 1}, (const void*)dad::conv_seam_f32<32, true>});
+        v.push_back({{64, 1}, (const void*)dad::conv_seam_f32<64, true>});
+        v.push_back({{64, 0}, (const void*)dad::conv_seam_f32<64, false>});
+        v.push_back({{128, 1}, (const void*)dad::conv_seam_f32<128, true>});
+        v.push_back({{128, 0}, (const void*)dad::conv_seam_f32<128, false>});
+        return v;
+    }();
+    return list;
+}
+const void* seam_kernel(int dim, bool tile0) { return find_kernel(seam_kernels(), dim, tile0, 0); }
+
 template <int TAPS, bool WIN>
 void add_wgrad(FamilyList& v) {
     v.push_back({{TAPS, 0, WIN}, (const void*)dad::conv_wgrad<TAPS, 2, 2, true, WIN>});
@@ -285,7 +300,7 @@
     std::vector<const void*> fns = {(const void*)dad::final_posterior_kernel, (const void*)dad::final_cc_kernel,
                                     (const void*)dad::project_kernel<4, 16>, (const void*)dad::project_kernel<1, 16>};
     for (const auto& kv : kernel_table()) fns.push_back((const void*)kv.second);
-    for (const FamilyList* list : {&cc_kernels(), &ccw_kernels(), &wgrad_kernels(), &halo8_kernels()})
+    for (const FamilyList* list : {&cc_kernels(), &ccw_kernels(), &wgrad_kernels(), &halo8_kernels(), &seam_kernels()})
         for (const FamilyKernel& k : *list) fns.push_back(k.fn);
     for (const void* fn : fns)
         HIP_TRY(hipFuncSetAttribute(fn, hipFuncAttributeMaxDynamicSharedMemorySize, (int)dad::kLdsBytes));
@@ -302,21 +317,14 @@
 };
 int launch_conv(dad_model* m, const ConvOp& op, const LaunchGeom& g, int batch, const ConvIO& io, hipStream_t st);
 
-int run_conv(dad_model* m, const FwdPlan& f, const FwdLaunch& l, const float* xext, float* ws, int t, hipStream_t st,
-             const int32_t* trow, const float* temb_rows) {
+ConvIO conv_io(dad_model* m, const FwdPlan& f, const FwdLaunch& l, const float* xext, float* ws, int t,
+               const int32_t* trow, const float* temb_rows) {
     const Plan& plan = f.train ? m->tplan : m->plan;
     const ConvOp& op = plan.convs[l.conv];
     const int batch = f.batch;
     auto buf = [&](int id) -> float* {
         return id >= 0 ? ws + plan.bufs[id].offset * (long)batch : nullptr;
     };
-    if (op.cat0 >= 0) {
-        const long rows = (long)batch * op.Lout;
-        const long n4 = rows * ((op.cat_c0 + op.cat_c1) / 4);
-        hipLaunchKernelGGL(dad::concat_rows_kernel, dim3((unsigned)((n4 + 255) / 256)), dim3(256), 0, st,
-                           buf(op.res), buf(op.cat0), buf(op.cat1), rows, op.cat_c0, op.cat_c1);
-        HIP_TRY(hipGetLastError());
-    }
     ConvIO io;
     io.src0 = op.src0 == -2 ? xext : buf(op.src0);
     io.src1 = buf(op.src1);
@@ -329,7 +337,22 @@
     io.rdst = buf(op.rdst);
     io.pre = buf(op.pre); io.stats = buf(op.stats);
     io.slab = ws + plan.floats_per_sample * (long)batch;
-    return launch_conv(m, op, l.g, batch, io, st);
+    return io;
+}
+int run_conv(dad_model* m, const FwdPlan& f, const FwdLaunch& l, const float* xext, float* ws, int t, hipStream_t st,
+             const int32_t* trow, const float* temb_rows) {
+    const Plan& plan = f.train ? m->tplan : m->plan;
+    const ConvOp& op = plan.convs[l.conv];
+    const int batch = f.batch;
+    if (op.cat0 >= 0) {
+        auto buf = [&](int id) -> float* { return ws + plan.bufs[id].offset * (long)batch; };
+        const long rows = (long)batch * op.Lout;
+        const long n4 = rows * ((op.cat_c0 + op.cat_c1) / 4);
+        hipLaunchKernelGGL(dad::concat_rows_kernel, dim3((unsigned)((n4 + 255) / 256)), dim3(256), 0, st,
+                           buf(op.res), buf(op.cat0), buf(op.cat1), rows, op.cat_c0, op.cat_c1);
+        HIP_TRY(hipGetLastError());
+    }
+    return launch_conv(m, op, l.g, batch, conv_io(m, f, l, xext, ws, t, trow, temb_rows), st);
 }
 
 int launch_gn_pass(dad_model* m, const ConvOp& op, int npt, int batch, const ConvIO& io, hipStream_t st) {
@@ -354,7 +377,7 @@
     return DAD_OK;
 }
 
-int launch_conv(dad_model* m, const ConvOp& op, const LaunchGeom& g, int batch, const ConvIO& io, hipStream_t st) {
+ConvParams conv_params(dad_model* m, const ConvOp& op, const LaunchGeom& g, int batch, const ConvIO& io) {
     const bool gn_pass = g.gn_npt > 0;
     ConvParams p{};
     p.src0 = io.src0;
@@ -388,6 +411,11 @@
     p.wtaps = op.wtaps();
     p.rbias = g.fused ? op.d_rbias : nullptr;
     p.rdst = g.fused ? io.rdst : nullptr;
+    return p;
+}
+int launch_conv(dad_model* m, const ConvOp& op, const LaunchGeom& g, int batch, const ConvIO& io, hipStream_t st) {
+    const bool gn_pass = g.gn_npt > 0;
+    ConvParams p = conv_params(m, op, g, batch, io);
     if (g.split.kslices > 1 && io.slab == nullptr)
         return fail(DAD_E_WORKSPACE, "%s: split-K launch without scratch", op.name.c_str());
     static const bool trace = getenv("DAD_TRACE_TILES") != nullptr;
@@ -518,8 +546,56 @@
     return DAD_OK;
 }
 
+void posterior_params(dad_model* m, const FwdPlan& f, float* x, int t, const dad_step_args* a, int x_out_disabled,
+                      bool seed_from_device, float* ws, dad::FinalParams& p) {
+    const dad_cfg& c = m->cfg;
+    const Plan& plan = f.train ? m->tplan : m->plan;
+    p.act = ws + plan.bufs[plan.final_act].offset * (long)f.batch;
+    p.w = m->d_final_w; p.bias = m->d_final_b;
+    p.dim = c.dim; p.td = c.transition_dim; p.B = f.batch; p.H = traj_horizon(*m); p.Hact = c.horizon;
+    p.predict_epsilon = c.predict_epsilon; p.clip_denoised = c.clip_denoised;
+    p.x = x;
+    p.noise = a->noise; p.cond0 = a->cond0; p.cond_per_row = a->cond_per_row;
+    p.guide = (a->guide_grad && a->guide_weight > 0.0f) ? a->guide_grad : nullptr;
+    p.mean_out = a->mean_out; p.eps_out = a->eps_out;
+    p.x_out_disabled = x_out_disabled;
+    const float lv = m->sched[4][t];
+    p.c_recip = m->sched[0][t]; p.c_recipm1 = m->sched[1][t];
+    p.coef1 = m->sched[2][t]; p.coef2 = m->sched[3][t];
+    p.sigma = t == 0 ? 0.0f : expf(0.5f * lv);
+    p.guide_scale = a->guide_weight * expf(lv);
+    p.seed = a->seed;
+    p.elem_offset = a->row_offset * (uint64_t)traj_horizon(*m) * (uint64_t)c.transition_dim;
+    p.draw = a->draw;
+    p.seed_dev = seed_from_device ? (const unsigned long long*)m->d_rng : nullptr;
+}
+
+struct SeamCall {
+    const SeamPlan* plan;
+    float* x;
+    int t;
+    const dad_step_args* a;
+    bool seed_from_device;
+};
+int launch_seam(dad_model* m, const FwdPlan& f, const SeamCall& sc, int t_conv, float* ws, hipStream_t st) {
+    const FwdLaunch& l = f.launches[0];
+    const ConvOp& op = m->plan.convs[l.conv];
+    dad::SeamParams q{};
+    posterior_params(m, f, sc.x, sc.t, sc.a, 0, sc.seed_from_device, ws, q.f);
+    q.c = conv_params(m, op, l.g, f.batch, conv_io(m, f, l, sc.x, ws, t_conv, nullptr, nullptr));
+    q.c.xswz = sc.plan->xswz;
+    q.units = sc.plan->units;
+    q.hshift = ilog2(m->cfg.horizon);
+    const void* fn = seam_kernel(m->cfg.dim, sc.plan->tile0);
+    if (fn == nullptr || q.c.rdst == nullptr || q.c.rbias == nullptr || q.c.gamma == nullptr)
+        return fail(DAD_E_INVALID, "no seam kernel for dim %d on tile %d", m->cfg.dim, sc.plan->cfg);
+    void* args[] = {&q};
+    HIP_TRY(hipLaunchKernel(fn, dim3(sc.plan->grid), dim3(sc.plan->threads), args, sc.plan->lds_bytes, st));
+    return DAD_OK;
+}
+
 int run_unet(dad_model* m, const FwdPlan& f, const float* x, int t, float* ws, hipStream_t st,
-             const int32_t* trow = nullptr, const float* temb_rows = nullptr) {
+             const int32_t* trow = nullptr, const float* temb_rows = nullptr, const SeamCall* seam = nullptr) {
     hipEvent_t e0 = nullptr, e1 = nullptr;
     if (m->profile) {
         if (m->ev_used == m->ev_pool.size()) {
@@ -539,7 +615,8 @@
         if (rc != DAD_OK) return rc;
     }
     for (const FwdLaunch& l : f.launches) {
-        const int rc = run_conv(m, f, l, x, ws, t, st, trow, temb_rows);
+        const int rc = (seam != nullptr && &l == &f.launches[0]) ? launch_seam(m, f, *seam, t, ws, st)
+                                                                 : run_conv(m, f, l, x, ws, t, st, trow, temb_rows);
         if (rc != DAD_OK) return rc;
     }
     if (m->profile) {
@@ -566,20 +643,7 @@
         p.eps_out = eps_only;
         p.x_out_disabled = 1;
     } else {
-        p.x = x;
-        p.noise = a->noise; p.cond0 = a->cond0; p.cond_per_row = a->cond_per_row;
-        p.guide = (a->guide_grad && a->guide_weight > 0.0f) ? a->guide_grad : nullptr;
-        p.mean_out = a->mean_out; p.eps_out = a->eps_out;
-        p.x_out_disabled = x_out_disabled;
-        const float lv = m->sched[4][t];
-        p.c_recip = m->sched[0][t]; p.c_recipm1 = m->sched[1][t];
-        p.coef1 = m->sched[2][t]; p.coef2 = m->sched[3][t];
-        p.sigma = t == 0 ? 0.0f : expf(0.5f * lv);
-        p.guide_scale = a->guide_weight * expf(lv);
-        p.seed = a->seed;
-        p.elem_offset = a->row_offset * (uint64_t)traj_horizon(*m) * (uint64_t)c.transition_dim;
-        p.draw = a->draw;
-        p.seed_dev = seed_from_device ? (const unsigned long long*)m->d_rng : nullptr;
+        posterior_params(m, f, x, t, a, x_out_disabled, seed_from_device, ws, p);
     }
     const dim3 grid(f.final_gx, f.final_gy);
     if (f.cc.ok) {
@@ -925,15 +989,21 @@
     const long step_elems = (long)batch * traj_horizon(*m) * m->cfg.transition_dim;
 
     const bool seed_dev = use_graph && !m->profile && noise_stack == nullptr;
+    const SeamPlan seam = plan_seam(*m, f, proj != nullptr);
+    const bool seamed = seam.taken() && n_steps > 1;
     auto enqueue_all = [&](hipStream_t st) -> int {
+        dad_step_args prev{};
         for (int j = 0; j < n_steps; ++j) {
             const int t = n_steps - 1 - j;
             dad_step_args a{};
             a.noise = noise_stack ? noise_stack + (long)j * step_elems : nullptr;
             a.seed = seed; a.row_offset = row_offset; a.draw = (uint64_t)(j + 1);
             a.cond0 = cond0; a.cond_per_row = cond_per_row;
-            int r = run_unet(m, f, x, t, (float*)workspace, st);
+            const SeamCall sc{&seam, x, t + 1, &prev, seed_dev};
+            int r = run_unet(m, f, x, t, (float*)workspace, st, nullptr, nullptr, seamed && j > 0 ? &sc : nullptr);
             if (r != DAD_OK) return r;
+            prev = a;
+            if (seamed && j + 1 < n_steps) continue;
             if ((r = run_final(m, f, x, nullptr, t, &a, 0, nullptr, (float*)workspace, st, seed_dev)) != DAD_OK) return r;
             if (proj && (r = run_project(proj, proj_alphas_host[t], x, batch, traj_horizon(*m), st)) != DAD_OK)
                 return r;
@@ -960,7 +1030,7 @@
     key.n_steps = n_steps; key.batch = batch; key.cond_per_row = cond_per_row;
     key.force_tile = m->force_tile;
     key.flags = (m->split_enabled ? 1 : 0) | (m->fuse_residual ? 2 : 0) | (m->xswz_enabled ? 4 : 0) |
-                (m->xcd_order ? 8 : 0) | (f.cc.ok ? 16 : 0) | (m->split_target << 8);
+                (m->xcd_order ? 8 : 0) | (f.cc.ok ? 16 : 0) | (m->step_seam ? 32 : 0) | (m->split_target << 8);
     key.row_offset = row_offset;
     if (proj) {
         uint64_t hsh = 1469598103934665603ull;
@@ -1586,6 +1656,7 @@
     else if (key == "ccw_prefer16") m->ccw_prefer16 = value != 0;
     else if (key == "wgrad_blocks") m->wgrad_blocks = std::max(1, (int)value);
     else if (key == "halo8") m->halo8_enabled = value != 0;
+    else if (key == "step_seam") m->step_seam = value != 0;
     else return fail(DAD_E_INVALID, "unknown option '%s'", name);
     if (!m->graphs.empty()) {
         HIP_TRY(hipDeviceSynchronize());
@@ -1710,6 +1781,24 @@
     out[DAD_PP_REFUSED] = q.refused;
     return DAD_OK;
 }
+
+int dad_debug_seam_plan(dad_model* m, int32_t batch, int32_t projection, int32_t* out) {
+    if (!m || !out || batch <= 0) return fail(DAD_E_INVALID, "bad argument");
+    FwdPlan f;
+    const int rc = plan_forward(*m, false, batch, true, f);
+    if (rc != DAD_OK) return rc;
+    const SeamPlan s = plan_seam(*m, f, projection != 0);
+    out[DAD_SEAM_TAKEN] = s.taken();
+    out[DAD_SEAM_REASON] = s.why;
+    out[DAD_SEAM_GRID] = s.taken() ? (int32_t)s.grid : 0;
+    out[DAD_SEAM_THREADS] = s.taken() ? s.threads : 0;
+    out[DAD_SEAM_LDS_BYTES] = s.taken() ? (int32_t)s.lds_bytes : 0;
+    out[DAD_SEAM_TILE] = s.taken() ? s.cfg : -1;
+    out[DAD_SEAM_UNITS] = s.taken() ? s.units : 0;
+    return DAD_OK;
+}
+
+const char* dad_debug_seam_reason(int32_t reason) { return seam_reason(reason); }
 
 int dad_debug_kernel_registered(int32_t cfg, int32_t taps, int32_t stride, int32_t flags) {
     if (taps < 1 || taps > kRegMaxTaps || stride < 1 || stride > 2 || flags < 0 || flags >= (1 << kRegFlags)) return 0;
diff --git a/dynamics_aware_diffusion_amd/csrc/host_plan.hpp b/dynamics_aware_diffusion_amd/csrc/host_plan.hpp
--- a/dynamics_aware_diffusion_amd/csrc/host_plan.hpp
+++ b/dynamics_aware_diffusion_amd/csrc/host_plan.hpp
@@ -173,6 +173,7 @@
     mutable std::map<std::array<int, 5>, uint64_t> xswz_cache;
     bool halo8_enabled = true;
     mutable std::map<std::array<int, 3>, uint64_t> xswz8_cache;
+    bool step_seam = true;
     bool training = false;
     struct BwdConv {
         int n = 0;
@@ -1360,6 +1361,93 @@
     return f.bytes;
 }
 
+enum SeamWhy {
+    SEAM_TAKEN = 0,
+    SEAM_OPTION,
+    SEAM_SMALL_BATCH,
+    SEAM_PRECISION,
+    SEAM_FORCED_TILE,
+    SEAM_PROJECTION,
+    SEAM_PADDED,
+    SEAM_HORIZON,
+    SEAM_TRANSITION_DIM,
+    SEAM_DIM,
+    SEAM_FIRST_CONV,
+    SEAM_NO_RIDE,
+    SEAM_TILE,
+    SEAM_LDS,
+    SEAM_BUFFERS,
+    SEAM_WHYS
+};
+inline const char* seam_reason(int why) {
+    static const char* const names[SEAM_WHYS] = {"taken", "option off", "small-batch kernels", "split-f16 arithmetic", "forced tile",
+                                                 "projection", "zero-padded net", "horizon", "transition_dim", "dim", "first conv",
+                                                 "no riding residual conv", "tile", "LDS", "buffers"};
+    return why >= 0 && why < SEAM_WHYS ? names[why] : "?";
+}
+struct SeamPlan {
+    int why = SEAM_OPTION;
+    bool tile0 = false;
+    int cfg = -1;
+    int units = 0;
+    unsigned grid = 0;
+    int threads = 0;
+    size_t lds_bytes = 0;
+    uint64_t xswz = 0;
+    bool taken() const { return why == SEAM_TAKEN; }
+};
+inline bool seam_buffers_ok(const Plan& plan, const ConvOp& op) {
+    const int n = (int)plan.bufs.size();
+    const int fa = plan.final_act;
+    if (fa < 0 || fa >= n || op.dst < 0 || op.dst >= n || op.rdst < 0 || op.rdst >= n || op.dst == op.rdst) return false;
+    const long rows = (long)op.Lout * op.M;
+    auto apart = [&](int a, int b) {
+        const long a0 = plan.bufs[a].offset, b0 = plan.bufs[b].offset;
+        return a0 + rows <= b0 || b0 + rows <= a0;
+    };
+    for (int id : {fa, op.dst, op.rdst})
+        if (plan.bufs[id].per_sample < rows) return false;
+    if (!apart(op.dst, op.rdst)) return false;
+    for (int id : {op.dst, op.rdst})
+        if (id != fa && !apart(fa, id)) return false;
+    return true;
+}
+inline SeamPlan plan_seam(const HostModel& m, const FwdPlan& f, bool projection) {
+    SeamPlan s;
+    const dad_cfg& c = m.cfg;
+    const int H = c.horizon, td = c.transition_dim, dim = c.dim;
+    auto no = [&](int why) { s.why = why; return s; };
+    if (!m.step_seam) return no(SEAM_OPTION);
+    if (f.train || f.cc.ok || f.launches.empty()) return no(SEAM_SMALL_BATCH);
+    if (m.precision != DAD_PREC_FP32) return no(SEAM_PRECISION);
+    if (m.force_tile >= 0 || !m.split_enabled) return no(SEAM_FORCED_TILE);
+    if (projection) return no(SEAM_PROJECTION);
+    const FwdLaunch& l = f.launches[0];
+    const ConvOp& op = m.plan.convs[l.conv];
+    if (traj_horizon(m) != H || op.net_padded || op.padded()) return no(SEAM_PADDED);
+    if (H != 8 && H != 16 && H != 32) return no(SEAM_HORIZON);
+    if (td > 16) return no(SEAM_TRANSITION_DIM);
+    if (dim != 32 && dim != 64 && dim != 128) return no(SEAM_DIM);
+    const LaunchGeom& g = l.g;
+    if (l.conv != 0 || !l.ok || op.kind != CONV_K5 || op.taps != 5 || op.stride != 1 || op.src0 != -2 || op.src1 >= 0 || op.cin0 != td ||
+        op.cin1 != 0 || op.cout != dim || op.M != dim || op.Lin != H || op.Lout != H || op.norm.empty() || op.res != -1 || op.cat0 >= 0 ||
+        op.x3 || op.bdir || op.kc != 16 || op.cin_pad < 16 || g.halo8 || g.padded || g.windowed || g.split.kslices != 1)
+        return no(SEAM_FIRST_CONV);
+    if (!g.fused || op.rdst < 0) return no(SEAM_NO_RIDE);
+    if ((g.cfg != 0 && g.cfg != 1) || g.kc != 32) return no(SEAM_TILE);
+    s.lds_bytes = dad::seam_lds_floats(td, dim, H) * sizeof(float);
+    if (s.lds_bytes > dad::kLdsBytes) return no(SEAM_LDS);
+    if (!seam_buffers_ok(m.plan, op)) return no(SEAM_BUFFERS);
+    s.cfg = g.cfg;
+    s.tile0 = g.cfg == 0;
+    s.units = td > 8 ? 2 : 1;
+    s.grid = (unsigned)(((long)f.batch * H + 31) / 32);
+    s.threads = dad::seam_threads(dim);
+    s.xswz = m.xswz_enabled ? find_xswz(m, H, 1, 2, dad::SEAM_KP / 4, 32) : 0;
+    s.why = SEAM_TAKEN;
+    return s;
+}
+
 struct ProjectPlan {
     int form = DAD_PP_ROW1;
     int rows_per_block = 1;
diff --git a/include/dad.h b/include/dad.h
--- a/include/dad.h
+++ b/include/dad.h
@@ -336,6 +336,16 @@
 #define DAD_PP_GEMM 2
 int dad_debug_project_plan(int32_t state_dim, int32_t observation_dim, int32_t action_dim, int32_t batch, int32_t horizon,
                            size_t scratch_bytes, int32_t violation, int32_t* out);
+#define DAD_SEAM_TAKEN 0
+#define DAD_SEAM_REASON 1
+#define DAD_SEAM_GRID 2
+#define DAD_SEAM_THREADS 3
+#define DAD_SEAM_LDS_BYTES 4
+#define DAD_SEAM_TILE 5
+#define DAD_SEAM_UNITS 6
+#define DAD_SEAM_INTS 7
+int dad_debug_seam_plan(dad_model* m, int32_t batch, int32_t projection, int32_t* out);
+const char* dad_debug_seam_reason(int32_t reason);
 int dad_debug_kernel_registered(int32_t cfg, int32_t taps, int32_t stride, int32_t flags);
 int dad_debug_small_kernel_exists(int32_t taps, int32_t stride, int32_t ride, int32_t wide, int32_t big, int32_t ride_in,
                                   int32_t rows, int32_t windowed);
```

New measurement: 3574 plans/s, median of 6. 1.01x the previous value.
